# aws/sagemaker-xgboost-container

Hardware: NVIDIA B200
Metric: boosting rounds/sec (higher is better)
Workload: dtype int64

## Files before the change

sagemaker-xgboost-container_b200/csrc/booster.cu:

```cuda
#include "booster.h"
#include <algorithm>
#include <atomic>
#include <cmath>
#include <cstring>
#include <functional>
#include "comm.h"

namespace b200 {

long long g_kernel_launches = 0;

namespace {
struct DeviceCtx {
  cudaStream_t stream = nullptr; int num_sms = 148; bool ok = false; std::string why;
  DeviceCtx() {
    int count = 0;
    cudaError_t e = cudaGetDeviceCount(&count);
    if (e != cudaSuccess || count == 0) { why = std::string("no CUDA device available (") + cudaGetErrorString(e) + ")"; cudaGetLastError(); return; }
    int dev = 0;
    if (const char* lr = getenv("LOCAL_RANK")) { dev = atoi(lr) % count; }
    if (const char* d = getenv("B200XGB_DEVICE")) { dev = atoi(d) % count; }
    if (cudaSetDevice(dev) != cudaSuccess) { why = "cudaSetDevice failed"; return; }
    if (cudaStreamCreateWithFlags(&stream, cudaStreamNonBlocking) != cudaSuccess) { why = "cudaStreamCreate failed"; return; }
    cudaDeviceGetAttribute(&num_sms, cudaDevAttrMultiProcessorCount, dev);
// ... 139 lines not shown

void DMatrix::ensure_binned(int max_bin) {
  if (binned && (binned_max_bin == max_bin || binned_max_bin == -1)) return;
  B200_CHECK(max_bin >= 2, "max_bin must be >= 2");
  cudaStream_t s = engine_stream();
  Comm& comm = Comm::get();
  if (!comm.distributed()) {
    compute_cuts_device(X.p, n, F, weights.empty() ? nullptr : d_weights.p, max_bin, has_missing, &cuts, s);
  } else {
    const int cap = 2048;
    int hm = has_missing ? 1 : 0;
    {
      DevBuf<unsigned> flag; flag.alloc(1); unsigned v = (unsigned)hm;
      CUDA_OK(cudaMemcpyAsync(flag.p, &v, 4, cudaMemcpyHostToDevice, s));
      comm.allreduce_max_u32(flag.p, 1, s);
      CUDA_OK(cudaMemcpyAsync(&v, flag.p, 4, cudaMemcpyDeviceToHost, s)); Comm::get().sync_stream(s);
      has_missing = v != 0;
    }
    std::vector<FeatureSummary> local;
    compute_summaries_device(X.p, n, F, weights.empty() ? nullptr : d_weights.p, cap, &local, s);
    const size_t per_feat = (size_t)(cap + 2);
    const size_t rec = per_feat * (sizeof(float) + sizeof(double)) + sizeof(double);
    std::vector<unsigned char> sendbuf((size_t)F * rec, 0);
    for (int f = 0; f < F; ++f) {
      unsigned char* p = sendbuf.data() + (size_t)f * rec;
      double cntd = (double)local[f].vals.size(); memcpy(p, &cntd, 8);
      memcpy(p + 8, local[f].vals.data(), sizeof(float) * local[f].vals.size());
      memcpy(p + 8 + per_feat * sizeof(float), local[f].weights.data(), sizeof(double) * local[f].weights.size());
    }
    const int W = comm.world();
    DevBuf<unsigned char> dsend, drecv; dsend.alloc(sendbuf.size()); drecv.alloc(sendbuf.size() * W);
    CUDA_OK(cudaMemcpyAsync(dsend.p, sendbuf.data(), sendbuf.size(), cudaMemcpyHostToDevice, s));
    comm.allgather_bytes(dsend.p, drecv.p, sendbuf.size(), s);
    std::vector<unsigned char> all(sendbuf.size() * W);
    CUDA_OK(cudaMemcpyAsync(all.data(), drecv.p, all.size(), cudaMemcpyDeviceToHost, s));
    Comm::get().sync_stream(s);
    std::vector<FeatureSummary> merged(F);
    for (int f = 0; f < F; ++f) {
      std::vector<std::pair<float, double>> pts;
      for (int r = 0; r < W; ++r) {
        const unsigned char* p = all.data() + (size_t)r * sendbuf.size() + (size_t)f * rec;
        double cntd; memcpy(&cntd, p, 8); size_t c = (size_t)cntd;
        const float* v = reinterpret_cast<const float*>(p + 8);
        std::vector<double> w(c); memcpy(w.data(), p + 8 + per_feat * sizeof(float), sizeof(double) * c);
        for (size_t i = 0; i < c; ++i) pts.emplace_back(v[i], w[i]);
      }
      std::stable_sort(pts.begin(), pts.end(), [](const std::pair<float, double>& a, const std::pair<float, double>& b) { return a.first < b.first; });
      for (auto& pw : pts) {
        if (!merged[f].vals.empty() && merged[f].vals.back() == pw.first) merged[f].weights.back() += pw.second;
        else { merged[f].vals.push_back(pw.first); merged[f].weights.push_back(pw.second); }
      }
    }
    cuts_from_summaries(merged, max_bin, has_missing, &cuts);
  }
  binned_max_bin = max_bin;
  bin_with_cuts();
}

__global__ void pack_tree_kernel(TreeArrays t, const int* n_nodes, DevNode* out, int cap) {
  const int nn = *n_nodes;
  for (int i = blockIdx.x * blockDim.x + threadIdx.x; i < cap; i += gridDim.x * blockDim.x) {
    DevNode d;
    if (i < nn) { d.cond = t.split_cond[i]; d.left = t.left[i]; d.right = t.right[i]; d.fidx_dl = (unsigned)t.split_index[i] | ((unsigned)t.default_left[i] << 31); }
    else { d.cond = 0.f; d.left = -1; d.right = -1; d.fidx_dl = 0; }
    out[i] = d;
  }
}

__global__ void snapshot_h_kernel(const GH64* slot, long long* cache, size_t entries) {
  for (size_t e = (size_t)blockIdx.x * blockDim.x + threadIdx.x; e < entries; e += (size_t)gridDim.x * blockDim.x) cache[e] = slot[e].h;
}
__global__ void slot_from_cache_kernel(GH64* slot, const long long* cache, size_t entries) {
  for (size_t e = (size_t)blockIdx.x * blockDim.x + threadIdx.x; e < entries; e += (size_t)gridDim.x * blockDim.x) { GH64 v; v.g = 0; v.h = cache[e]; slot[e] = v; }
}

struct PinnedPool {
  std::vector<std::pair<char*, size_t>> chunks; size_t cur = 0, off = 0;
  ~PinnedPool() { for (auto& c : chunks) cudaFreeHost(c.first); }
  void* take(size_t bytes) {
    bytes = (bytes + 255) & ~(size_t)255;
    while (cur < chunks.size() && off + bytes > chunks[cur].second) { ++cur; off = 0; }
    if (cur >= chunks.size()) { size_t sz = std::max<size_t>(bytes, 4u << 20); char* p = nullptr; CUDA_OK(cudaMallocHost(&p, sz)); chunks.emplace_back(p, sz); off = 0; }
    void* r = chunks[cur].first + off; off += bytes; return r;
  }
  void reset() { cur = 0; off = 0; }
};

struct TreeGraphKey { uint64_t uid, binned_version; const void *margin, *mask, *packed, *bins, *bins_col, *cuts, *mono, *ic_sets, *ic_allowed; int n_ic; int max_depth, max_leaves, lg_iters; float eta, lambda, alpha, gamma, mcw, mds, bynode; unsigned seed; int world, root_mode; int64_t n; };
struct TreeGraph {
  std::vector<cudaGraphExec_t> segs; std::vector<std::function<void()>> colls;
  TreeGraphKey key; long long launches = 0;
  TreeGraph() { memset(&key, 0, sizeof key); }
  void destroy() { for (auto e : segs) if (e) cudaGraphExecDestroy(e); segs.clear(); colls.clear(); }
};

struct GrowerImpl {
  int64_t n = 0; int ngroups = 0, tw = 0, max_depth = 0, max_nodes = 0, cap_nodes = 0, max_level_nodes = 0, region = 0;
  int lg_iters = 0;
  size_t slot_stride = 0;
  int64_t gp_stride = 0;
  int64_t global_n = 0;
  DevBuf<long long> root_h_cache; uint64_t root_h_uid = 0, root_h_version = 0; bool root_h_valid = false;
  GrowState gs{}; TreeArrays ta{};
  DevBuf<unsigned char> state_block;
  DevBuf<unsigned char> tree_block;
  size_t tree_block_bytes = 0;
  DevBuf<GH64> hist_pool; DevBuf<unsigned> ridx0, ridx1, scratch;
  DevBuf<float2> gpair, gp0, gp1; DevBuf<unsigned> tl0, tl1; DevBuf<int> err, tree_index_dev, monotone_dev; DevBuf<unsigned char> feat_mask, ic_path, ic_allowed, ic_sets;
  std::vector<unsigned char> ic_sets_host;
  std::vector<int> monotone_host;
  DevBuf<double> dsum;
  PinnedPool pinned; std::vector<cudaEvent_t> free_events;
  DevBuf<DevNode> packed; std::vector<TreeGraph> graphs; std::vector<char> eager_done;
  TreeGraph* capturing = nullptr;

  void ensure(int64_t n_, int ngroups_, int tw_, int max_depth_, int K, int lg_iters_ = 0) {
    const int64_t stride_ = (n_ + 63) & ~(int64_t)63;
    if (n == n_ && ngroups == ngroups_ && tw == tw_ && max_depth == max_depth_ && lg_iters == lg_iters_ && gpair.n >= (size_t)stride_ * K + 512) return;
    if (lg_iters_ == 0) B200_CHECK(max_depth_ >= 1 && max_depth_ <= kMaxDepth, "max_depth must be in [1, 16] for the B200 depth-wise hist builder");
    n = n_; ngroups = ngroups_; tw = tw_; max_depth = max_depth_; lg_iters = lg_iters_; gp_stride = stride_; root_h_valid = false;
    if (peer_reduce_active()) {
      peer_reduce_close();
      DevBuf<unsigned> bar; bar.alloc(1); bar.zero(engine_stream());
      Comm::get().allreduce_max_u32(bar.p, 1, engine_stream());
      Comm::get().sync_stream(engine_stream());
    }
    for (auto& tg : graphs) tg.destroy();
    size_t pool_slots;
    if (lg_iters > 0) {
      max_nodes = 2 * lg_iters + 1; max_level_nodes = 2; region = 0;
      pool_slots = (size_t)lg_iters + kLgFirstFreeSlot;
    } else {
      max_nodes = (1 << (max_depth + 1)) - 1; max_level_nodes = 1 << (max_depth - 1); region = max_level_nodes;
      pool_slots = 2 * (size_t)region;
    }
    cap_nodes = (max_nodes + 15) & ~15;
    slot_stride = hist_slot_entries(ngroups, tw);
    const size_t pool_bytes = pool_slots * slot_stride * sizeof(GH64);
    size_t free_b = 0, total_b = 0; cudaMemGetInfo(&free_b, &total_b);
    B200_CHECK(pool_bytes < free_b / 2 + hist_pool.n * sizeof(GH64), "histogram pool for this max_depth / max_leaves / feature count does not fit in device memory");
    hist_pool.alloc(pool_slots * slot_stride);
    ridx0.alloc(n); ridx1.alloc(n);
    gpair.alloc((size_t)gp_stride * K + 512); gpair.zero(engine_stream()); gp0.alloc(n); gp1.alloc(n); err.alloc(1); dsum.alloc(4);
    root_h_cache.alloc(slot_stride);
    tl0.alloc(tw == 4 ? n : 0); tl1.alloc(tw == 4 ? n : 0);
    const unsigned max_tiles = (unsigned)((n + kPartTile - 1) / kPartTile) + max_level_nodes + 1;
    scratch.alloc(3 * (size_t)max_level_nodes + 8);
    size_t off = 0; auto take = [&](size_t bytes) { size_t o = off; off += (bytes + 255) & ~(size_t)255; return o; };
    const size_t N = cap_nodes, L = max_level_nodes;
    size_t o_seg_begin = take(4 * N), o_seg_count = take(4 * N), o_slot = take(4 * N), o_sum = take(16 * N), o_rg = take(4 * N), o_w = take(4 * N);
    size_t o_best = take(sizeof(SplitCand) * N), o_bestg = take(sizeof(SplitCand) * N * (ngroups + (tw > 0 ? 1 : 0)));
    size_t o_lnodes = take(4 * (size_t)(kMaxDepth + 1) * L), o_lcount = take(4 * (kMaxDepth + 2));
    size_t o_bnid = take(4 * L), o_bsub = take(4 * L), o_bps = take(4 * L), o_bcount = take(4), o_bprefix = take(4 * (L + 1));
    size_t o_action = take(4 * L), o_tprefix = take(4 * (L + 1)), o_tleft = take(4 * (size_t)max_tiles), o_toff = take(4 * (size_t)max_tiles);
    size_t o_flags = take((size_t)n + 16), o_nleaves = take(4), o_scales = take(16), o_absmax = take(8);
    size_t o_depth = take(4 * N), o_open = take(N), o_nslots = take(4), o_lgdone = take(4), o_lower = take(4 * N), o_upper = take(4 * N);
    state_block.alloc(off); state_block.zero(engine_stream());
    unsigned char* b = state_block.p;
    gs.seg_begin = (unsigned*)(b + o_seg_begin); gs.seg_count = (unsigned*)(b + o_seg_count); gs.hist_slot = (int*)(b + o_slot);
    gs.node_sum = (GH64*)(b + o_sum); gs.root_gain = (float*)(b + o_rg); gs.weight = (float*)(b + o_w);
    gs.best = (SplitCand*)(b + o_best); gs.best_group = (SplitCand*)(b + o_bestg);
    gs.level_nodes = (int*)(b + o_lnodes); gs.level_count = (int*)(b + o_lcount);
    gs.build_nid = (int*)(b + o_bnid); gs.build_sub_nid = (int*)(b + o_bsub); gs.build_parent_slot = (int*)(b + o_bps);
    gs.build_count = (int*)(b + o_bcount); gs.build_prefix = (unsigned*)(b + o_bprefix);
    gs.part_action = (int*)(b + o_action); gs.tile_prefix = (unsigned*)(b + o_tprefix); gs.tile_left = (unsigned*)(b + o_tleft); gs.tile_off = (unsigned*)(b + o_toff);
    gs.lower = (float*)(b + o_lower); gs.upper = (float*)(b + o_upper);
    gs.depth = (int*)(b + o_depth); gs.open = b + o_open; gs.n_slots = (int*)(b + o_nslots); gs.lg_done = (int*)(b + o_lgdone);
    gs.flags = b + o_flags; gs.n_leaves = (int*)(b + o_nleaves); gs.scales = (float*)(b + o_scales); gs.absmax = (unsigned*)(b + o_absmax);
    tree_block_bytes = 64 + 9 * 4 * N + N;
    tree_block.alloc(tree_block_bytes);
    unsigned char* t = tree_block.p;
    gs.n_nodes = (int*)t;
    int* ip = (int*)(t + 64);
    ta.left = ip; ta.right = ip + N; ta.parent = ip + 2 * N; ta.split_index = ip + 3 * N; ta.split_bin = ip + 4 * N;
    float* fp = (float*)(ip + 5 * N);
    ta.split_cond = fp; ta.base_weight = fp + N; ta.loss_chg = fp + 2 * N; ta.sum_hess = fp + 3 * N;
    ta.default_left = (unsigned char*)(fp + 4 * N);
    hist_configure();
    global_n = n;
    if (Comm::get().distributed()) {
      peer_reduce_setup({{hist_pool.p, hist_pool.n * sizeof(GH64)}, {state_block.p, state_block.n}}, engine_stream());
      double v = (double)n;
      CUDA_OK(cudaMemcpyAsync(dsum.p, &v, sizeof v, cudaMemcpyHostToDevice, engine_stream()));
      Comm::get().allreduce_sum_f64(dsum.p, 1, engine_stream());
      CUDA_OK(cudaMemcpyAsync(&v, dsum.p, sizeof v, cudaMemcpyDeviceToHost, engine_stream()));
      Comm::get().sync_stream(engine_stream());
      global_n = (int64_t)v;
    }
  }
};

static int job_grad_bits(int64_t global_n) { return grad_bits_for(global_n); }
static int job_window_rows(int64_t global_n) { return window_rows_for(global_n); }

static int lossguide_iters(const TrainParam& p) {
  if (!p.lossguide) return 0;
  if (p.max_leaves > 0) return std::max(1, p.max_leaves - 1);
  return (1 << p.max_depth) - 1;
}

static TrainParamDev to_dev(const TrainParam& p) {
  TrainParamDev d; d.eta = p.eta; d.lambda = p.lambda; d.alpha = p.alpha; d.gamma = p.gamma; d.min_child_weight = p.min_child_weight;
  d.max_delta_step = p.max_delta_step; d.max_depth = p.max_depth; d.max_leaves = p.max_leaves; return d;
}

static inline uint64_t splitmix64(uint64_t x) {
  x += 0x9E3779B97F4A7C15ULL; x = (x ^ (x >> 30)) * 0xBF58476D1CE4E5B9ULL; x = (x ^ (x >> 27)) * 0x94D049BB133111EBULL; return x ^ (x >> 31);
}
static inline float rng_uniform(uint32_t seed, uint64_t stream, uint64_t idx) {
  uint64_t h = splitmix64(splitmix64(((uint64_t)seed << 32) ^ stream) ^ idx);
  return (float)(h >> 40) * (1.0f / 16777216.0f);
}
std::string subset_mask(const std::string& parent, float frac, unsigned seed, uint64_t stream) {
  if (frac >= 1.0f) return parent;
  const int F = (int)parent.size();
  int cnt = 0; for (int f = 0; f < F; ++f) cnt += parent[f] ? 1 : 0;
  const int keep = std::max(1, (int)std::floor(frac * (float)cnt));
  std::vector<float> u(F);
  for (int f = 0; f < F; ++f) u[f] = rng_uniform(seed, stream, (uint64_t)f);
  std::string m((size_t)F, (char)0);
  for (int f = 0; f < F; ++f) {
    if (!parent[f]) continue;
    int rank = 0;
    for (int g = 0; g < F; ++g) if (parent[g] && (u[g] < u[f] || (u[g] == u[f] && g < f))) ++rank;
    m[f] = rank < keep ? 1 : 0;
  }
  return m;
}
std::string colsample_mask(unsigned seed, int tree_index, int F, float frac) {
  return subset_mask(std::string((size_t)F, (char)1), frac, seed, 0x1000 + (uint64_t)tree_index);
}

Booster::Booster() {}
Booster::~Booster() {
  if (grower_) { for (auto e : grower_->free_events) cudaEventDestroy(e); delete grower_; }
  for (auto& p : pending_) if (p.ready) cudaEventDestroy(p.ready);
}

static const std::map<std::string, int>& objective_table() {
  static const std::map<std::string, int> t = {{"reg:squarederror", kSquaredError}, {"reg:linear", kSquaredError}, {"binary:logistic", kBinaryLogistic},
    {"reg:logistic", kRegLogistic}, {"binary:logitraw", kLogitRaw}, {"multi:softprob", kSoftprob}, {"multi:softmax", kSoftmax},
    {"reg:squaredlogerror", kSquaredLogError}, {"reg:pseudohubererror", kPseudoHuber}, {"count:poisson", kPoisson}, {"reg:gamma", kGamma},
    {"reg:tweedie", kTweedie}, {"binary:hinge", kHinge}};
  return t;
}

void Booster::set_param(const std::string& k, const std::string& v) {
  if (k == "eval_metric") { if (std::find(eval_metrics_.begin(), eval_metrics_.end(), v) == eval_metrics_.end()) eval_metrics_.push_back(v); }
  else raw_params_[k] = v;
  configured_ = false;
}

void Booster::configure() {
  if (configured_) return;
  auto getf = [&](const char* a, const char* b, float def) { auto it = raw_params_.find(a); if (it == raw_params_.end() && b) it = raw_params_.find(b);
    if (it == raw_params_.end()) return def; try { return std::stof(it->second); } catch (...) { throw Error(std::string("Invalid value for parameter ") + a + ": " + it->second); } };
  auto geti = [&](const char* a, int def) { auto it = raw_params_.find(a); if (it == raw_params_.end()) return def;
    try { return (int)std::stod(it->second); } catch (...) { throw Error(std::string("Invalid value for parameter ") + a + ": " + it->second); } };
  TrainParam p;
  auto ito = raw_params_.find("objective");
  if (ito != raw_params_.end()) objective_name_ = ito->second;
  auto ot = objective_table().find(objective_name_);
  B200_CHECK(ot != objective_table().end(), "Unknown objective function: `" + objective_name_ + "` (supported on the B200 hist path: reg:squarederror, reg:linear, reg:logistic, reg:squaredlogerror, reg:pseudohubererror, reg:gamma, reg:tweedie, count:poisson, binary:logistic, binary:logitraw, binary:hinge, multi:softprob, multi:softmax)");
  p.objective = ot->second;
  if (objective_name_ == "reg:linear") objective_name_ = "reg:squarederror";
  p.num_class = (p.objective == kSoftprob || p.objective == kSoftmax) ? geti("num_class", 0) : 1;
  if (p.objective == kSoftprob || p.objective == kSoftmax) B200_CHECK(p.num_class >= 1, "num_class must be set (>= 1) for multi:softprob / multi:softmax");
  p.max_depth = geti("max_depth", 6); p.max_leaves = geti("max_leaves", 0); p.max_bin = geti("max_bin", 256);
  p.eta = getf("eta", "learning_rate", 0.3f); p.lambda = getf("lambda", "reg_lambda", 1.0f); p.alpha = getf("alpha", "reg_alpha", 0.0f);
  p.gamma = getf("gamma", "min_split_loss", 0.0f); p.min_child_weight = getf("min_child_weight", nullptr, 1.0f);
  p.max_delta_step = getf("max_delta_step", nullptr, 0.0f); p.scale_pos_weight = getf("scale_pos_weight", nullptr, 1.0f);
  p.subsample = getf("subsample", nullptr, 1.0f); p.colsample_bytree = getf("colsample_bytree", nullptr, 1.0f);
  p.colsample_bylevel = getf("colsample_bylevel", nullptr, 1.0f); p.colsample_bynode = getf("colsample_bynode", nullptr, 1.0f);
  p.seed = (unsigned)geti("seed", 0);
  p.huber_slope = getf("huber_slope", nullptr, 1.0f); p.tweedie_variance_power = getf("tweedie_variance_power", nullptr, 1.5f);
  B200_CHECK(p.huber_slope != 0.0f, "Check failed: slope != 0.0 (huber_slope)");
  B200_CHECK(p.tweedie_variance_power >= 1.0f && p.tweedie_variance_power < 2.0f, "tweedie_variance_power must be in interval [1, 2)");
  if (p.objective == kPoisson) {
    if (raw_params_.find("max_delta_step") == raw_params_.end()) p.max_delta_step = 0.7f;
    p.poisson_max_delta_step = p.max_delta_step;
    B200_CHECK(p.poisson_max_delta_step >= 0.0f, "max_delta_step must be non-negative for count:poisson");
  }
  B200_CHECK(p.lambda >= 0.0f, "Parameter reg_lambda should be greater equal to 0");
  B200_CHECK(p.subsample > 0.0f && p.subsample <= 1.0f, "Parameter subsample should be in (0, 1]");
  auto tm = raw_params_.find("tree_method");
  if (tm != raw_params_.end()) {
    const std::string& t = tm->second;
    B200_CHECK(t == "hist" || t == "auto" || t == "gpu_hist" || t == "approx" || t == "exact",
               "Unknown tree_method: " + t);
  }
  auto bo = raw_params_.find("booster");
  if (bo != raw_params_.end()) B200_CHECK(bo->second == "gbtree", "Only booster=gbtree is implemented on the B200 hist path (got " + bo->second + ")");
  auto gp = raw_params_.find("grow_policy");
  if (gp != raw_params_.end()) {
    B200_CHECK(gp->second == "depthwise" || gp->second == "lossguide", "Invalid grow_policy: " + gp->second + " (depthwise, lossguide)");
    p.lossguide = gp->second == "lossguide" ? 1 : 0;
  }
  interaction_.clear();
  auto ic = raw_params_.find("interaction_constraints");
  if (ic != raw_params_.end()) {
    int depth = 0; std::string tok; std::vector<int> cur;
    auto flush = [&]() { if (tok.empty()) return; int v = 0; try { v = std::stoi(tok); } catch (...) { throw Error("Invalid interaction_constraints entry: " + tok); }
      B200_CHECK(v >= 0, "interaction_constraints entries must be feature indices (feature names are not supported)"); cur.push_back(v); tok.clear(); };
    for (char ch : ic->second) {
      if (ch == '[' || ch == '(') { ++depth; }
      else if (ch == ']' || ch == ')') { flush(); if (depth == 2 && !cur.empty()) { interaction_.push_back(cur); cur.clear(); } --depth; }
      else if (ch >= '0' && ch <= '9') tok.push_back(ch);
      else { B200_CHECK(ch == ',' || ch == ' ' || ch == '\t' || ch == '\n' || ch == '"' || ch == '\'', std::string("Invalid character in interaction_constraints: ") + ch); flush(); }
    }
    B200_CHECK(depth == 0, "Unbalanced brackets in interaction_constraints");
  }
  monotone_.clear();
  auto mc = raw_params_.find("monotone_constraints");
  if (mc != raw_params_.end()) {
    std::string tok;
    auto flush = [&]() { if (tok.empty()) return; int v = 0; try { v = std::stoi(tok); } catch (...) { throw Error("Invalid monotone_constraints entry: " + tok); }
      B200_CHECK(v >= -1 && v <= 1, "monotone_constraints entries must be -1, 0 or 1"); monotone_.push_back(v); tok.clear(); };
    for (char ch : mc->second) { if (ch == '-' || ch == '+' || (ch >= '0' && ch <= '9')) tok.push_back(ch); else flush(); }
    flush();
    bool any = false; for (int v : monotone_) any |= v != 0;
    if (!any) monotone_.clear();
  }
  if (p.lossguide) {
    B200_CHECK(p.max_depth >= 0 && p.max_depth <= kMaxDepth, "max_depth must be in [0, 16]");
    B200_CHECK(p.max_leaves > 0 || p.max_depth > 0, "grow_policy=lossguide needs max_leaves > 0 or max_depth > 0");
    B200_CHECK(p.max_leaves <= 4096, "max_leaves above 4096 is not supported by the B200 lossguide builder");
    B200_CHECK(p.colsample_bytree >= 1.0f && p.colsample_bylevel >= 1.0f && p.colsample_bynode >= 1.0f, "column sampling (colsample_*) with grow_policy=lossguide is not implemented by the B200 hist builder");
  }
  auto bs = raw_params_.find("base_score");
  if (bs != raw_params_.end() && !bs->second.empty()) {
    base_score_ = std::stof(bs->second); base_score_set_ = true;
// ... 41 lines not shown

void Booster::append_device_tree(int class_id, size_t device_offset, int max_nodes, PendingTree pt) {
  trees_.emplace_back(); tree_info_.push_back(class_id); pending_.push_back(pt); on_device_.push_back(1);
  h_tree_offset.resize(trees_.size() + 1);
  h_tree_offset[trees_.size() - 1] = (int64_t)device_offset;
  h_tree_offset[trees_.size()] = (int64_t)device_offset + max_nodes;
  ++model_version_;
}

void Booster::sync_model() {
  bool any = false;
  for (auto& p : pending_) if (p.staging) { any = true; break; }
  if (!any) return;
  for (size_t t = 0; t < pending_.size(); ++t) {
    PendingTree& p = pending_[t];
    if (!p.staging) continue;
    CUDA_OK(cudaEventSynchronize(p.ready));
    const unsigned char* b = (const unsigned char*)p.staging;
    const int nn = *(const int*)b; const size_t N = p.cap_nodes;
    const int* ip = (const int*)(b + 64); const float* fp = (const float*)(ip + 5 * N); const unsigned char* up = (const unsigned char*)(fp + 4 * N);
    HostTree& h = trees_[t];
    h.left.assign(ip, ip + nn); h.right.assign(ip + N, ip + N + nn); h.parent.assign(ip + 2 * N, ip + 2 * N + nn);
    h.split_index.assign(ip + 3 * N, ip + 3 * N + nn); h.split_bin.assign(ip + 4 * N, ip + 4 * N + nn);
    h.split_cond.assign(fp, fp + nn); h.base_weight.assign(fp + N, fp + N + nn); h.loss_chg.assign(fp + 2 * N, fp + 2 * N + nn); h.sum_hess.assign(fp + 3 * N, fp + 3 * N + nn);
    h.default_left.assign(up, up + nn);
    if (grower_) grower_->free_events.push_back(p.ready); else cudaEventDestroy(p.ready);
    p.ready = nullptr; p.staging = nullptr;
  }
  if (grower_) grower_->pinned.reset();
}

void Booster::upload_model() {
  cudaStream_t s = engine_stream();
  const int nt = (int)trees_.size();
  if ((int)h_tree_offset.size() != nt + 1) h_tree_offset.resize(nt + 1, 0);
  pending_.resize(nt); on_device_.resize(nt, 0);
  for (int t = 0; t < nt; ++t) {
    if (on_device_[t]) continue;
    const HostTree& h = trees_[t];
    const int nn = h.num_nodes();
    std::vector<DevNode> nodes(nn);
    for (int i = 0; i < nn; ++i) { nodes[i].cond = h.split_cond[i]; nodes[i].left = h.left[i]; nodes[i].right = h.right[i]; nodes[i].fidx_dl = (unsigned)h.split_index[i] | ((unsigned)h.default_left[i] << 31);
      if (h.left[i] >= 0 && h.right[i] != h.left[i] + 1) children_adjacent_ = false; }
    if (d_nodes_used + nn > d_nodes.n) {
      size_t cap = std::max<size_t>(d_nodes.n * 2, d_nodes_used + nn + 4096);
      DevBuf<DevNode> nb; nb.alloc(cap);
      if (d_nodes_used) CUDA_OK(cudaMemcpyAsync(nb.p, d_nodes.p, sizeof(DevNode) * d_nodes_used, cudaMemcpyDeviceToDevice, s));
      Comm::get().sync_stream(s);
      std::swap(nb.p, d_nodes.p); std::swap(nb.n, d_nodes.n);
    }
    CUDA_OK(cudaMemcpyAsync(d_nodes.p + d_nodes_used, nodes.data(), sizeof(DevNode) * nn, cudaMemcpyHostToDevice, s));
    Comm::get().sync_stream(s);
    h_tree_offset[t] = (int64_t)d_nodes_used; h_tree_offset[t + 1] = (int64_t)d_nodes_used + nn;
    d_nodes_used += nn; on_device_[t] = 1; d_trees_uploaded = 0;
  }
  if (d_trees_uploaded != nt || d_tree_offset.n < (size_t)nt + 1) {
    d_tree_offset.ensure(std::max<size_t>(nt + 1, 64)); d_tree_info.ensure(std::max<size_t>(nt, 64));
    CUDA_OK(cudaMemcpyAsync(d_tree_offset.p, h_tree_offset.data(), sizeof(int64_t) * (nt + 1), cudaMemcpyHostToDevice, s));
    if (nt) CUDA_OK(cudaMemcpyAsync(d_tree_info.p, tree_info_.data(), sizeof(int) * nt, cudaMemcpyHostToDevice, s));
    Comm::get().sync_stream(s);
    d_trees_uploaded = nt;
  }
}

PredCache& Booster::cache_for(DMatrix* dm) {
  PredCache& c = caches_[dm->uid];
  const int K = param_.num_class;
  if (c.n != dm->n || c.margin.n != (size_t)dm->n * K) {
    c.n = dm->n; c.margin.alloc((size_t)dm->n * K); c.trees_applied = -1;
  }
  return c;
}

void Booster::bring_cache_up_to_date(DMatrix* dm, PredCache& c) {
  cudaStream_t s = engine_stream();
  const int K = param_.num_class;
  const int nt = (int)trees_.size();
  if (c.trees_applied < 0) {
    if (!dm->base_margin.empty()) {
      B200_CHECK(dm->base_margin.size() == (size_t)dm->n * K, "base_margin size does not match rows x groups");
      CUDA_OK(cudaMemcpyAsync(c.margin.p, dm->d_base_margin.p, sizeof(float) * dm->n * K, cudaMemcpyDeviceToDevice, s));
    } else launch_fill(c.margin.p, dm->n * K, base_margin(), s);
    c.trees_applied = 0;
  }
  if (c.trees_applied < nt) {
    upload_model();
    PredictArgs pa{}; pa.X = dm->X.p; pa.n = dm->n; pa.F = dm->F; pa.nodes = d_nodes.p; pa.tree_offset = d_tree_offset.p; pa.tree_info = d_tree_info.p;
    pa.tree_begin = c.trees_applied; pa.tree_end = nt; pa.K = K; pa.margin = c.margin.p; pa.leaf = nullptr;
    pa.h_tree_offset = h_tree_offset.data(); pa.has_nan = dm->has_missing ? 1 : 0; pa.children_adjacent = children_adjacent_ ? 1 : 0;
    launch_predict(pa, s);
    c.trees_applied = nt;
  }
}

static void check_labels(const DMatrix* dm) {
  B200_CHECK(dm->labels.size() == (size_t)dm->n, "Check failed: preds.size() == info.labels_.size() (" + std::to_string(dm->n) + " vs. " +
             std::to_string(dm->labels.size()) + ") : labels are not correctly provided");
}

void Booster::update_one_iter(int iter, DMatrix* dtrain) {
  configure();
  (void)iter;
  cudaStream_t s = engine_stream();
  check_labels(dtrain);
  if (num_feature_ == 0) num_feature_ = dtrain->F;
  B200_CHECK(num_feature_ == dtrain->F, "Check failed: learner_model_param_.num_feature == p_fmat->Info().num_col_ (" + std::to_string(num_feature_) +
             " vs. " + std::to_string(dtrain->F) + ") : Number of columns does not match number of features in booster.");
  B200_CHECK(dtrain->n > 0 || Comm::get().distributed(), "Empty dataset at worker: 0");
  dtrain->ensure_binned(param_.max_bin);
  const int K = param_.num_class;
  if (!grower_) grower_ = new GrowerImpl();
  GrowerImpl& g = *grower_;
  g.ensure(dtrain->n, dtrain->ngroups, dtrain->tw, param_.max_depth, K, lossguide_iters(param_));
  if (!labels_checked_) {
    const std::vector<float>& y = dtrain->labels;
    if (param_.objective == kBinaryLogistic || param_.objective == kRegLogistic || param_.objective == kLogitRaw)
      for (float v : y) B200_CHECK(v >= 0.0f && v <= 1.0f, "Check failed: label must be in [0,1] for logistic regression");
    if (param_.objective == kSoftprob || param_.objective == kSoftmax)
      for (float v : y) B200_CHECK(v >= 0.0f && (int)v < K, "SoftmaxMultiClassObj: label must be in [0, num_class).");
    if (param_.objective == kSquaredLogError) for (float v : y) B200_CHECK(v > -1.0f, "Check failed: label must be greater than -1 for rmsle so that log(label + 1) can be valid.");
    if (param_.objective == kPoisson) for (float v : y) B200_CHECK(v >= 0.0f, "PoissonRegression: label must be nonnegative");
    if (param_.objective == kGamma) for (float v : y) B200_CHECK(v > 0.0f, "GammaRegression: label must be positive.");
    if (param_.objective == kTweedie) for (float v : y) B200_CHECK(v >= 0.0f, "TweedieRegression: label must be nonnegative");
    labels_checked_ = true;
  }
  estimate_base_score(dtrain);
  PredCache& cache = cache_for(dtrain);
  bring_cache_up_to_date(dtrain, cache);

  const int round = (int)trees_.size() / K;
  CUDA_OK(cudaMemsetAsync(g.gs.absmax, 0, 8, s));
  GradArgs ga{}; ga.margin = cache.margin.p; ga.label = dtrain->d_labels.p; ga.weight = dtrain->weights.empty() ? nullptr : dtrain->d_weights.p;
  ga.gpair = g.gpair.p; ga.gp_stride = g.gp_stride; ga.absmax = g.gs.absmax; ga.err = g.err.p; ga.n = dtrain->n; ga.row_offset = 0; ga.K = K; ga.objective = param_.objective;
  ga.scale_pos_weight = param_.scale_pos_weight; ga.subsample = param_.subsample; ga.seed = param_.seed; ga.iter = (unsigned long long)round;
  ga.row_offset = (int64_t)Comm::get().rank() << 40; ga.aux = objective_aux(param_);
  launch_gradient(ga, s);
  Comm::get().allreduce_max_u32(g.gs.absmax, 2, s);
  launch_scales(g.gs, job_grad_bits(g.global_n), s);

  for (int k = 0; k < K; ++k) grow_one_tree(dtrain, cache, k, round * K + k);
}


void Booster::enqueue_tree(DMatrix* dtrain, float* margin, int k, const unsigned char* mask, DevNode* packed_out, int root_mode) {
  cudaStream_t s = engine_stream();
  GrowerImpl& g = *grower_;
  Comm& comm = Comm::get();
  const int K = param_.num_class;
  const int D = param_.max_depth;
  const TrainParamDev pd = to_dev(param_);
  const BinnedMatrix bm = dtrain->binned_view();
  const int num_sms = engine_num_sms();
  const unsigned max_tiles = (unsigned)((dtrain->n + kPartTile - 1) / kPartTile) + g.max_level_nodes + 1;

  launch_init_tree(g.gs, g.ta, (unsigned)dtrain->n, 0, g.max_level_nodes, s);
  if (root_mode == 2) { slot_from_cache_kernel<<<148, 256, 0, s>>>(g.hist_pool.p, g.root_h_cache.p, g.slot_stride); ++g_kernel_launches; CUDA_OK(cudaGetLastError()); }
  else CUDA_OK(cudaMemsetAsync(g.hist_pool.p, 0, g.slot_stride * sizeof(GH64), s));

  HistArgs ha{}; ha.bins = bm.bins; ha.bins_tail = bm.bins_tail; ha.n = bm.n; ha.row_stride = bm.ngroups * kSlots; ha.tw = bm.tw;
  ha.bins_gather = bm.bins_gather; ha.gather_stride = bm.gather_stride;
  ha.gpair = g.gpair.p + (size_t)k * g.gp_stride; ha.ridx = nullptr;
  ha.build_count = g.gs.build_count; ha.build_nid = g.gs.build_nid; ha.build_prefix = g.gs.build_prefix; ha.seg_begin = g.gs.seg_begin;
  ha.hist_slot = g.gs.hist_slot; ha.scales = g.gs.scales; ha.hist_pool = g.hist_pool.p; ha.node_sum = g.gs.node_sum; ha.ngroups = bm.ngroups;
  ha.accumulate_sum = 1; ha.g_only = root_mode == 2 ? 1 : 0; ha.window_rows = job_window_rows(g.global_n);
  ha.rows_counter = profile_ ? prof_rows_.p : nullptr;
  prof_begin(0);
  launch_hist_build(ha, num_sms, s);
  prof_end();
  if (root_mode == 1) { snapshot_h_kernel<<<148, 256, 0, s>>>(g.hist_pool.p, g.root_h_cache.p, g.slot_stride); ++g_kernel_launches; CUDA_OK(cudaGetLastError()); }
  ha.g_only = 0;
  auto collective = [&](std::function<void()> f) {
    if (!comm.distributed()) return;
    if (!g.capturing) { f(); return; }
    cudaGraph_t graph = nullptr;
    CUDA_OK(cudaStreamEndCapture(s, &graph));
    cudaGraphExec_t exec = nullptr;
    cudaError_t e = cudaGraphInstantiate(&exec, graph, 0);
    cudaGraphDestroy(graph);
    CUDA_OK(e);
    g.capturing->segs.push_back(exec); g.capturing->colls.push_back(f);
    CUDA_OK(cudaStreamBeginCapture(s, cudaStreamCaptureModeThreadLocal));
  };
  auto allreduce_hist = [&](GH64* p, size_t cnt) {
    if (!comm.distributed()) return;
    if (peer_allreduce_i64(reinterpret_cast<long long*>(p), cnt, s)) return;
    collective([p, cnt, s]() { Comm::get().allreduce_sum_i64(p, cnt, s); });
  };
  allreduce_hist(g.hist_pool.p, g.slot_stride * 2);
  allreduce_hist(g.gs.node_sum, 2);
  const int* mono_dev = nullptr;
  if (!monotone_.empty()) {
    B200_CHECK((int)monotone_.size() <= bm.F, "monotone_constraints has more entries than the data has features");
    mono_dev = g.monotone_dev.p;
  }
  const bool ic_on = !interaction_.empty();
  if (ic_on) {
    CUDA_OK(cudaMemsetAsync(g.ic_path.p, 0, (size_t)bm.F, s));
    CUDA_OK(cudaMemsetAsync(g.ic_allowed.p, 1, (size_t)bm.F, s));
  }
  EvalArgs ea{}; ea.hist_pool = g.hist_pool.p; ea.gs = g.gs; ea.cut_ptrs = dtrain->d_cut_ptrs.p; ea.feat_mask = mask; ea.p = pd; ea.F = bm.F;
  ea.ngroups = bm.ngroups; ea.tw = bm.tw; ea.ntail = bm.ntail; ea.has_missing = bm.has_missing; ea.level = 0; ea.max_level_nodes = g.max_level_nodes;
  ea.colsample_bynode = mask ? param_.colsample_bynode : 1.0f; ea.seed = param_.seed; ea.tree_index = g.tree_index_dev.p; ea.monotone = mono_dev; ea.node_allowed = ic_on ? g.ic_allowed.p : nullptr;
  launch_eval(ea, 1, s);

  const int lg_iters = lossguide_iters(param_);
  for (int it = 0; it < lg_iters; ++it) {
    ApplyArgs aa{}; aa.gs = g.gs; aa.tree = g.ta; aa.cut_ptrs = dtrain->d_cut_ptrs.p; aa.cut_vals = dtrain->d_cut_vals.p; aa.min_vals = dtrain->d_min_vals.p;
    aa.p = pd; aa.scratch = g.scratch.p; aa.ngroups = bm.ngroups + (bm.tw > 0 ? 1 : 0); aa.level = 0; aa.max_level_nodes = g.max_level_nodes; aa.monotone = mono_dev;
    if (ic_on) { aa.node_path = g.ic_path.p; aa.node_allowed = g.ic_allowed.p; aa.ic_sets = g.ic_sets.p; aa.n_ic_sets = (int)interaction_.size(); aa.F = bm.F; }
    launch_apply_lossguide(aa, it, s);
    const bool carry_tail = bm.tw == 4;
    PartArgs pa{}; pa.gs = g.gs; pa.tree = g.ta; pa.bins_col = bm.bins_col; pa.n = bm.n;
    pa.ridx_cur = it == 0 ? nullptr : g.ridx0.p; pa.ridx_next = g.ridx1.p;
    pa.gp_cur = it == 0 ? g.gpair.p + (size_t)k * g.gp_stride : g.gp0.p; pa.gp_next = g.gp1.p;
    pa.tl_cur = !carry_tail ? nullptr : (it == 0 ? reinterpret_cast<const unsigned*>(bm.bins_tail) : g.tl0.p); pa.tl_next = !carry_tail ? nullptr : g.tl1.p;
    pa.has_missing = bm.has_missing; pa.level = 0; pa.max_level_nodes = g.max_level_nodes;
    launch_partition(pa, max_tiles, 1, s);
    launch_lg_copy_back(pa, g.ridx0.p, g.gp0.p, g.tl0.p, max_tiles, s);
    launch_zero_build_slots(g.gs, g.hist_pool.p, g.slot_stride, 1, s);
    ha.ridx = g.ridx0.p; ha.gpair = g.gp0.p; ha.tail_pos = carry_tail ? g.tl0.p : nullptr; ha.accumulate_sum = 0;
    ha.rows_counter = profile_ ? prof_rows_.p + 1 : nullptr;
    prof_begin(1);
    launch_hist_build(ha, num_sms, s);
    prof_end();
    if (comm.distributed()) {
      launch_lg_stage(g.gs, g.hist_pool.p, g.slot_stride, 1, s);
      allreduce_hist(g.hist_pool.p + (size_t)kLgStageSlot * g.slot_stride, g.slot_stride * 2);
      launch_lg_stage(g.gs, g.hist_pool.p, g.slot_stride, 0, s);
    }
    launch_subtract(g.gs, g.hist_pool.p, g.slot_stride, 1, s);
    ea.level = 1; ea.feat_mask = nullptr;
    launch_eval(ea, 2, s);
  }

  for (int L = 0; L < D && lg_iters == 0; ++L) {
    const bool final_level = (L == D - 1);
    const int next_base = ((L + 1) & 1) * g.region, next_half = 1 << L;
    ApplyArgs aa{}; aa.gs = g.gs; aa.tree = g.ta; aa.cut_ptrs = dtrain->d_cut_ptrs.p; aa.cut_vals = dtrain->d_cut_vals.p; aa.min_vals = dtrain->d_min_vals.p;
    aa.p = pd; aa.scratch = g.scratch.p; aa.ngroups = bm.ngroups + (bm.tw > 0 ? 1 : 0); aa.level = L; aa.max_level_nodes = g.max_level_nodes; aa.next_base = next_base; aa.next_half = next_half; aa.monotone = mono_dev;
    if (ic_on) { aa.node_path = g.ic_path.p; aa.node_allowed = g.ic_allowed.p; aa.ic_sets = g.ic_sets.p; aa.n_ic_sets = (int)interaction_.size(); aa.F = bm.F; }
    launch_apply(aa, s);
    if (final_level) break;
    PartArgs pa{}; pa.gs = g.gs; pa.tree = g.ta; pa.bins_col = bm.bins_col; pa.n = bm.n;
    pa.ridx_cur = L == 0 ? nullptr : ((L & 1) ? g.ridx0.p : g.ridx1.p);
    pa.ridx_next = (L & 1) ? g.ridx1.p : g.ridx0.p;
    pa.gp_cur = L == 0 ? g.gpair.p + (size_t)k * g.gp_stride : ((L & 1) ? g.gp0.p : g.gp1.p);
    pa.gp_next = (L & 1) ? g.gp1.p : g.gp0.p;
    const bool carry_tail = bm.tw == 4;
    pa.tl_cur = !carry_tail ? nullptr : (L == 0 ? reinterpret_cast<const unsigned*>(bm.bins_tail) : ((L & 1) ? g.tl0.p : g.tl1.p));
    pa.tl_next = !carry_tail ? nullptr : ((L & 1) ? g.tl1.p : g.tl0.p);
    pa.has_missing = bm.has_missing; pa.level = L; pa.max_level_nodes = g.max_level_nodes;
    launch_partition(pa, max_tiles, 1 << L, s);
    CUDA_OK(cudaMemsetAsync(g.hist_pool.p + (size_t)next_base * g.slot_stride, 0, (size_t)next_half * g.slot_stride * sizeof(GH64), s));
    ha.ridx = pa.ridx_next; ha.gpair = pa.gp_next; ha.tail_pos = pa.tl_next; ha.accumulate_sum = 0;
    ha.rows_counter = profile_ ? prof_rows_.p + 1 : nullptr;
    prof_begin(L + 1);
    launch_hist_build(ha, num_sms, s);
    prof_end();
    allreduce_hist(g.hist_pool.p + (size_t)next_base * g.slot_stride, (size_t)next_half * g.slot_stride * 2);
    launch_subtract(g.gs, g.hist_pool.p, g.slot_stride, next_half, s);
    ea.level = L + 1;
    ea.feat_mask = mask ? mask + (size_t)(L + 1) * bm.F : nullptr;
    launch_eval(ea, 1 << (L + 1), s);
  }

  launch_update_margin(g.ta, g.gs.n_nodes, bm.bins_col, bm.n, bm.has_missing, margin, K, k, s);

  pack_tree_kernel<<<(g.cap_nodes + 255) / 256, 256, 0, s>>>(g.ta, g.gs.n_nodes, packed_out, g.cap_nodes); ++g_kernel_launches;
  CUDA_OK(cudaGetLastError());
}

void Booster::grow_one_tree(DMatrix* dtrain, PredCache& cache, int k, int tree_index) {
  cudaStream_t s = engine_stream();
  GrowerImpl& g = *grower_;
  const unsigned char* mask = nullptr;
  const bool sampling = param_.colsample_bytree < 1.0f || param_.colsample_bylevel < 1.0f || param_.colsample_bynode < 1.0f;
  if (sampling) {
    const std::string tm = colsample_mask(param_.seed, tree_index, dtrain->F, param_.colsample_bytree);
    std::string all;
    for (int d = 0; d < param_.max_depth; ++d) all += subset_mask(tm, param_.colsample_bylevel, param_.seed, 0x300000ull + 64ull * (uint64_t)tree_index + (uint64_t)d);
    g.feat_mask.ensure(all.size()); g.tree_index_dev.ensure(1);
    CUDA_OK(cudaMemcpyAsync(g.feat_mask.p, all.data(), all.size(), cudaMemcpyHostToDevice, s));
    CUDA_OK(cudaMemcpyAsync(g.tree_index_dev.p, &tree_index, sizeof(int), cudaMemcpyHostToDevice, s));
    Comm::get().sync_stream(s);
    mask = g.feat_mask.p;
  }
  if (!monotone_.empty()) {
    std::vector<int> mh(monotone_); mh.resize((size_t)std::max<int>(dtrain->F, (int)mh.size()), 0);
    if (mh != g.monotone_host || g.monotone_dev.n < mh.size()) {
      g.monotone_dev.ensure(mh.size());
      CUDA_OK(cudaMemcpyAsync(g.monotone_dev.p, mh.data(), sizeof(int) * mh.size(), cudaMemcpyHostToDevice, s));
      Comm::get().sync_stream(s);
      g.monotone_host = mh;
    }
  }
  if (!interaction_.empty()) {
    const size_t F = (size_t)dtrain->F;
    std::vector<unsigned char> sets(interaction_.size() * F, 0);
    for (size_t si = 0; si < interaction_.size(); ++si)
      for (int f : interaction_[si]) { B200_CHECK((size_t)f < F, "interaction_constraints names feature " + std::to_string(f) + " but the data has " + std::to_string(F) + " features"); sets[si * F + f] = 1; }
    g.ic_path.ensure((size_t)g.cap_nodes * F); g.ic_allowed.ensure((size_t)g.cap_nodes * F);
    if (sets != g.ic_sets_host || g.ic_sets.n < sets.size()) {
      g.ic_sets.ensure(sets.size());
      CUDA_OK(cudaMemcpyAsync(g.ic_sets.p, sets.data(), sets.size(), cudaMemcpyHostToDevice, s));
      Comm::get().sync_stream(s);
      g.ic_sets_host = sets;
    }
  }
  g.packed.ensure((size_t)g.cap_nodes);
  static const bool no_graph = getenv("B200XGB_NO_GRAPH") != nullptr;
  static const bool no_graph_multi = getenv("B200XGB_NO_GRAPH_MULTI") != nullptr;
  const bool dist = Comm::get().distributed();
  if ((int)g.eager_done.size() <= k) g.eager_done.resize(k + 1, 0);
  const bool eager_first = dist && !g.eager_done[k];
  static const bool no_consth = getenv("B200XGB_NO_CONSTH") != nullptr;
  const bool consth = !no_consth && param_.objective == kSquaredError && param_.num_class == 1 && dtrain->weights.empty() &&
                      param_.subsample >= 1.0f && param_.scale_pos_weight == 1.0f;
  int root_mode = 0;
  if (consth) {
    if (g.root_h_valid && g.root_h_uid == dtrain->uid && g.root_h_version == dtrain->binned_version) root_mode = 2;
    else root_mode = 1;
  }
  if (profile_ || no_graph || (dist && no_graph_multi) || eager_first || root_mode == 1) {
    g.eager_done[k] = 1;
    enqueue_tree(dtrain, cache.margin.p, k, mask, g.packed.p, root_mode);
    if (root_mode == 1) { g.root_h_valid = true; g.root_h_uid = dtrain->uid; g.root_h_version = dtrain->binned_version; }
  } else {
    if ((int)g.graphs.size() <= k) g.graphs.resize(k + 1);
    TreeGraph& tg = g.graphs[k];
    TreeGraphKey key; memset(&key, 0, sizeof key);
    key.uid = dtrain->uid; key.binned_version = dtrain->binned_version; key.root_mode = root_mode;
    key.margin = cache.margin.p; key.mask = mask; key.packed = g.packed.p; key.max_depth = param_.max_depth;
    key.bins = dtrain->bins.p; key.bins_col = dtrain->bins_col.p; key.cuts = dtrain->d_cut_vals.p;
    key.max_leaves = param_.max_leaves; key.lg_iters = lossguide_iters(param_); key.eta = param_.eta; key.lambda = param_.lambda; key.alpha = param_.alpha; key.gamma = param_.gamma;
    key.mcw = param_.min_child_weight; key.mds = param_.max_delta_step; key.world = Comm::get().world(); key.n = dtrain->n;
    key.bynode = param_.colsample_bynode; key.seed = param_.seed; key.mono = monotone_.empty() ? nullptr : g.monotone_dev.p;
    key.ic_sets = interaction_.empty() ? nullptr : g.ic_sets.p; key.ic_allowed = interaction_.empty() ? nullptr : g.ic_allowed.p; key.n_ic = (int)interaction_.size();
    if (tg.segs.empty() || memcmp(&tg.key, &key, sizeof key) != 0) {
      tg.destroy();
      const long long launches_before = g_kernel_launches;
      CUDA_OK(cudaStreamBeginCapture(s, cudaStreamCaptureModeThreadLocal));
      g.capturing = &tg;
      cudaGraph_t graph = nullptr;
      try { enqueue_tree(dtrain, cache.margin.p, k, mask, g.packed.p, root_mode); }
      catch (...) { g.capturing = nullptr; cudaStreamEndCapture(s, &graph); if (graph) cudaGraphDestroy(graph); tg.destroy(); throw; }
      g.capturing = nullptr;
      CUDA_OK(cudaStreamEndCapture(s, &graph));
      cudaGraphExec_t exec = nullptr;
      cudaError_t e = cudaGraphInstantiate(&exec, graph, 0);
      cudaGraphDestroy(graph);
      if (e != cudaSuccess) { tg.destroy(); CUDA_OK(e); }
      tg.segs.push_back(exec);
      tg.key = key; tg.launches = g_kernel_launches - launches_before;
      g_kernel_launches = launches_before;
    }
    for (size_t i = 0; i < tg.segs.size(); ++i) {
      CUDA_OK(cudaGraphLaunch(tg.segs[i], s));
      if (i < tg.colls.size()) tg.colls[i]();
    }
    g_kernel_launches += tg.launches;
  }

  const size_t need = d_nodes_used + (size_t)g.cap_nodes;
  if (need > d_nodes.n) {
    size_t cap = std::max<size_t>(d_nodes.n * 2, need + 64 * (size_t)g.cap_nodes);
    DevBuf<DevNode> nb; nb.alloc(cap);
    if (d_nodes_used) CUDA_OK(cudaMemcpyAsync(nb.p, d_nodes.p, sizeof(DevNode) * d_nodes_used, cudaMemcpyDeviceToDevice, s));
    Comm::get().sync_stream(s);
    std::swap(nb.p, d_nodes.p); std::swap(nb.n, d_nodes.n);
  }
  CUDA_OK(cudaMemcpyAsync(d_nodes.p + d_nodes_used, g.packed.p, sizeof(DevNode) * (size_t)g.cap_nodes, cudaMemcpyDeviceToDevice, s));
  if (pending_.size() - (size_t)std::count_if(pending_.begin(), pending_.end(), [](const PendingTree& p) { return p.staging == nullptr; }) >= 512) sync_model();
  PendingTree pt; pt.cap_nodes = (size_t)g.cap_nodes;
  pt.staging = g.pinned.take(g.tree_block_bytes);
  if (!g.free_events.empty()) { pt.ready = g.free_events.back(); g.free_events.pop_back(); }
  else CUDA_OK(cudaEventCreateWithFlags(&pt.ready, cudaEventDisableTiming));
  CUDA_OK(cudaMemcpyAsync(pt.staging, g.tree_block.p, g.tree_block_bytes, cudaMemcpyDeviceToHost, s));
  CUDA_OK(cudaEventRecord(pt.ready, s));
  append_device_tree(k, d_nodes_used, g.cap_nodes, pt);
  d_nodes_used += (size_t)g.cap_nodes;
  d_trees_uploaded = 0;
  cache.trees_applied = (int)trees_.size();
}

void Booster::boost_one_iter(DMatrix*, const float*, const float*, size_t) {
  throw Error("custom objective (BoostOneIter) is not implemented on the B200 hist path");
}

int Booster::boosted_rounds() { configure(); return (int)trees_.size() / std::max(1, param_.num_class); }

static std::string default_metric(const TrainParam& p) {
  switch (p.objective) {
    case kSquaredError: case kRegLogistic: return "rmse";
    case kBinaryLogistic: case kLogitRaw: return "logloss";
    case kSquaredLogError: return "rmsle";
    case kPseudoHuber: return "mphe";
    case kPoisson: return "poisson-nloglik";
    case kGamma: return "gamma-nloglik";
    case kTweedie: { char buf[64]; snprintf(buf, sizeof buf, "tweedie-nloglik@%g", (double)p.tweedie_variance_power); return buf; }
    case kHinge: return "error";
    default: return "mlogloss";
  }
}

std::string Booster::eval_one_iter(int iter, const std::vector<DMatrix*>& dms, const std::vector<std::string>& names) {
  configure();
  cudaStream_t s = engine_stream();
  std::vector<std::string> metrics = eval_metrics_;
  if (metrics.empty()) metrics.push_back(default_metric(param_));
  if (!grower_) grower_ = new GrowerImpl();
  grower_->dsum.ensure(4);
  std::string out = "[" + std::to_string(iter) + "]";
  for (size_t i = 0; i < dms.size(); ++i) {
    DMatrix* dm = dms[i];
    check_labels(dm);
    PredCache& c = cache_for(dm);
    bring_cache_up_to_date(dm, c);
    for (const std::string& mname : metrics) {
      MetricArgs ma{}; ma.margin = c.margin.p; ma.label = dm->d_labels.p; ma.weight = dm->weights.empty() ? nullptr : dm->d_weights.p;
      ma.out = grower_->dsum.p; ma.n = dm->n; ma.K = param_.num_class; ma.threshold = 0.5f;
      ma.is_logistic = (param_.objective == kBinaryLogistic || param_.objective == kRegLogistic) ? 1 : 0;
      ma.transform = objective_transform(param_.objective); ma.aux = 0.0f;
      std::string base = mname;
      if (mname.rfind("tweedie-nloglik@", 0) == 0) { base = "tweedie-nloglik"; ma.aux = std::stof(mname.substr(16)); B200_CHECK(ma.aux >= 1.0f && ma.aux < 2.0f, "tweedie variance power must be in interval [1, 2)"); }
      if (mname.rfind("error@", 0) == 0) { base = "error"; ma.threshold = std::stof(mname.substr(6)); }
      if (base == "auc") {
        B200_CHECK(param_.num_class <= 1, "auc is implemented for binary / regression-style predictions only");
        const int logistic = (param_.objective == kBinaryLogistic || param_.objective == kRegLogistic) ? 1 : 0;
        compute_auc_device(c.margin.p, dm->d_labels.p, dm->weights.empty() ? nullptr : dm->d_weights.p, dm->n, logistic, grower_->dsum.p, s);
        double h3[3];
        CUDA_OK(cudaMemcpyAsync(h3, grower_->dsum.p, 3 * sizeof(double), cudaMemcpyDeviceToHost, s));
        Comm::get().sync_stream(s);
        double pair[2] = {h3[0], h3[1] * h3[2]};
        if (Comm::get().distributed()) {
          CUDA_OK(cudaMemcpyAsync(grower_->dsum.p, pair, 2 * sizeof(double), cudaMemcpyHostToDevice, s));
          Comm::get().allreduce_sum_f64(grower_->dsum.p, 2, s);
          CUDA_OK(cudaMemcpyAsync(pair, grower_->dsum.p, 2 * sizeof(double), cudaMemcpyDeviceToHost, s));
          Comm::get().sync_stream(s);
        }
        B200_CHECK(pair[1] > 0.0, "Check failed: !auc_error AUC: the dataset only contains pos or neg samples");
        char buf[64]; snprintf(buf, sizeof buf, "%.17g", pair[0] / pair[1]);
        out += "\t" + names[i] + "-" + mname + ":" + buf;
        continue;
      }
      if (base == "rmse") ma.metric = kMetricRmse; else if (base == "mse") ma.metric = kMetricRmse; else if (base == "mae") ma.metric = kMetricMae;
      else if (base == "logloss") ma.metric = kMetricLogloss; else if (base == "error") ma.metric = kMetricError;
      else if (base == "merror") ma.metric = kMetricMerror; else if (base == "mlogloss") ma.metric = kMetricMlogloss;
      else if (base == "rmsle") ma.metric = kMetricRmsle; else if (base == "mape") ma.metric = kMetricMape;
      else if (base == "mphe") { ma.metric = kMetricMphe; ma.aux = param_.huber_slope; }
      else if (base == "poisson-nloglik") ma.metric = kMetricPoissonNll; else if (base == "gamma-nloglik") ma.metric = kMetricGammaNll;
      else if (base == "gamma-deviance") ma.metric = kMetricGammaDeviance;
      else if (base == "tweedie-nloglik") { ma.metric = kMetricTweedieNll; if (ma.aux == 0.0f) throw Error("tweedie-nloglik needs its variance power: tweedie-nloglik@rho"); }
      else throw Error("Unknown metric function " + mname + " (B200 hist path implements rmse, mse, rmsle, mae, mape, mphe, logloss, error, error@t, merror, mlogloss, auc, poisson-nloglik, gamma-nloglik, gamma-deviance, tweedie-nloglik@rho)");
      if (param_.objective == kLogitRaw && (ma.metric == kMetricLogloss || ma.metric == kMetricError)) ma.is_logistic = 1;
      if ((ma.metric == kMetricMerror || ma.metric == kMetricMlogloss)) B200_CHECK(param_.num_class > 1, "Check failed: preds.size() == info.labels_.size() : label and prediction size not match, hint: use merror or mlogloss for multi-class classification");
      CUDA_OK(cudaMemsetAsync(grower_->dsum.p, 0, 2 * sizeof(double), s));
      launch_metric(ma, s);
      Comm::get().allreduce_sum_f64(grower_->dsum.p, 2, s);
      double h[2];
      CUDA_OK(cudaMemcpyAsync(h, grower_->dsum.p, 2 * sizeof(double), cudaMemcpyDeviceToHost, s));
      Comm::get().sync_stream(s);
      double v = h[1] == 0.0 ? h[0] : h[0] / h[1];
      if (mname == "rmse" || mname == "rmsle") v = std::sqrt(v);
      if (mname == "gamma-deviance") v *= 2.0;
      char buf[64]; snprintf(buf, sizeof buf, "%.17g", v);
      out += "\t" + names[i] + "-" + mname + ":" + buf;
    }
  }
  return out;
}

void Booster::predict(DMatrix* dm, int type, bool training, int iter_begin, int iter_end, bool strict_shape,
                      std::vector<float>* out, std::vector<uint64_t>* shape) {
  configure();
  (void)training;
  cudaStream_t s = engine_stream();
  const int K = param_.num_class;
  const int rounds = (int)trees_.size() / K;
  if (iter_end == 0) iter_end = rounds;
  B200_CHECK(iter_begin >= 0 && iter_begin <= iter_end && iter_end <= rounds, "Invalid iteration range: [" + std::to_string(iter_begin) + ", " + std::to_string(iter_end) + ") for a model with " + std::to_string(rounds) + " rounds");
  if (num_feature_ > 0 && !trees_.empty())
    B200_CHECK(dm->F <= num_feature_ || true, "feature count mismatch");
  B200_CHECK(type == 0 || type == 1 || type == 2 || type == 6, "predict type " + std::to_string(type) + " (approximate contributions / interactions) is not implemented on the B200 path");
  if (type == 2) { predict_contribs(dm, iter_begin * K, iter_end * K, out, shape); return; }
  upload_model();
  const int tb = iter_begin * K, te = iter_end * K;
  const int64_t n = dm->n;
  PredictArgs pa{}; pa.X = dm->X.p; pa.n = n; pa.F = dm->F; pa.nodes = d_nodes.p; pa.tree_offset = d_tree_offset.p; pa.tree_info = d_tree_info.p;
  pa.tree_begin = tb; pa.tree_end = te; pa.K = K;
  pa.h_tree_offset = h_tree_offset.data(); pa.has_nan = dm->has_missing ? 1 : 0; pa.children_adjacent = children_adjacent_ ? 1 : 0;
  if (type == 6) {
    const int nt = te - tb;
    DevBuf<int>& leaf = pred_leaf_; leaf.ensure((size_t)n * std::max(nt, 1));
    pa.margin = nullptr; pa.leaf = leaf.p;
    launch_predict(pa, s);
    std::vector<int> h((size_t)n * nt);
    if (!h.empty()) CUDA_OK(cudaMemcpyAsync(h.data(), leaf.p, sizeof(int) * h.size(), cudaMemcpyDeviceToHost, s));
    Comm::get().sync_stream(s);
    out->resize(h.size());
    for (size_t i = 0; i < h.size(); ++i) (*out)[i] = (float)h[i];
    shape->assign({(uint64_t)n, (uint64_t)nt});
    return;
  }
  DevBuf<float>& margin = pred_margin_; margin.ensure((size_t)n * K);
  if (!dm->base_margin.empty()) {
    B200_CHECK(dm->base_margin.size() == (size_t)n * K, "base_margin size does not match rows x groups");
    CUDA_OK(cudaMemcpyAsync(margin.p, dm->d_base_margin.p, sizeof(float) * n * K, cudaMemcpyDeviceToDevice, s));
  } else launch_fill(margin.p, n * K, base_margin(), s);
  pa.margin = margin.p; pa.leaf = nullptr;
  launch_predict(pa, s);
  int out_cols = K;
  DevBuf<float>& cls = pred_cls_;
  if (type == 0) {
    if (param_.objective == kSoftmax) { cls.ensure(n); launch_transform(margin.p, n, K, param_.objective, cls.p, s); out_cols = 1; }
    else launch_transform(margin.p, n, K, param_.objective, nullptr, s);
  }
  out->resize((size_t)n * out_cols);
  if (!out->empty()) CUDA_OK(cudaMemcpyAsync(out->data(), (type == 0 && param_.objective == kSoftmax) ? cls.p : margin.p, sizeof(float) * out->size(), cudaMemcpyDeviceToHost, s));
  Comm::get().sync_stream(s);
  if (out_cols == 1 && !strict_shape) shape->assign({(uint64_t)n});
  else shape->assign({(uint64_t)n, (uint64_t)out_cols});
}

__global__ void gather_u32_kernel(const unsigned* src, const unsigned* idx, unsigned* dst, int64_t n) {
  const int64_t i = (int64_t)blockIdx.x * blockDim.x + threadIdx.x;
  if (i < n) dst[i] = src[idx[i]];
}

void Booster::debug_build_root_hist(DMatrix* dm, const float* gpair_host, std::vector<long long>* hist_out, float* scales_out,
                                    int repeats, float* ms_out, int mode, const unsigned* row_ids, int64_t n_ids) {
  configure();
  cudaStream_t s = engine_stream();
  dm->ensure_binned(param_.max_bin);
  if (!grower_) grower_ = new GrowerImpl();
  GrowerImpl& g = *grower_;
  g.ensure(dm->n, dm->ngroups, dm->tw, param_.max_depth, param_.num_class, lossguide_iters(param_));
  hist_configure();
  const int64_t rows = row_ids ? n_ids : dm->n;
  B200_CHECK(rows <= dm->n, "debug_build_root_hist: more row ids than rows");
  CUDA_OK(cudaMemcpyAsync(g.gpair.p, gpair_host, sizeof(float2) * rows, cudaMemcpyHostToDevice, s));
  if (row_ids) CUDA_OK(cudaMemcpyAsync(g.ridx0.p, row_ids, sizeof(unsigned) * rows, cudaMemcpyHostToDevice, s));
  float mg = 0.f, mh = 0.f;
  for (int64_t i = 0; i < rows; ++i) { mg = std::max(mg, std::fabs(gpair_host[2 * i])); mh = std::max(mh, gpair_host[2 * i + 1]); }
  unsigned am[2]; memcpy(&am[0], &mg, 4); memcpy(&am[1], &mh, 4);
  CUDA_OK(cudaMemcpyAsync(g.gs.absmax, am, 8, cudaMemcpyHostToDevice, s));
  launch_scales(g.gs, job_grad_bits(g.global_n), s);
  const BinnedMatrix bm = dm->binned_view();
  HistArgs ha{}; ha.bins = bm.bins; ha.bins_tail = bm.bins_tail; ha.n = bm.n; ha.row_stride = bm.ngroups * kSlots; ha.tw = bm.tw; ha.gpair = g.gpair.p;
  ha.bins_gather = bm.bins_gather; ha.gather_stride = bm.gather_stride;
  ha.ridx = row_ids ? g.ridx0.p : nullptr;
  ha.build_count = g.gs.build_count; ha.build_nid = g.gs.build_nid; ha.build_prefix = g.gs.build_prefix; ha.seg_begin = g.gs.seg_begin;
  ha.hist_slot = g.gs.hist_slot; ha.scales = g.gs.scales; ha.hist_pool = g.hist_pool.p; ha.node_sum = g.gs.node_sum; ha.ngroups = bm.ngroups; ha.accumulate_sum = 1;
  ha.force_gather = (mode & 3) == 1 ? 1 : 0; ha.g_only = (mode & 3) == 2 ? 1 : 0; ha.window_rows = job_window_rows(g.global_n);
  if ((mode & 4) && row_ids && bm.tw == 4) {
    gather_u32_kernel<<<(unsigned)((rows + 255) / 256), 256, 0, s>>>(reinterpret_cast<const unsigned*>(bm.bins_tail), g.ridx0.p, g.tl0.p, rows); ++g_kernel_launches;
    CUDA_OK(cudaGetLastError());
    ha.tail_pos = g.tl0.p;
  }
  g.root_h_valid = false;
  cudaEvent_t e0, e1; CUDA_OK(cudaEventCreate(&e0)); CUDA_OK(cudaEventCreate(&e1));
  float total = 0.f;
  for (int r = 0; r < std::max(1, repeats); ++r) {
    launch_init_tree(g.gs, g.ta, (unsigned)rows, 0, g.max_level_nodes, s);
    CUDA_OK(cudaMemsetAsync(g.hist_pool.p, 0, g.slot_stride * sizeof(GH64), s));
    CUDA_OK(cudaEventRecord(e0, s));
    launch_hist_build(ha, engine_num_sms(), s);
    CUDA_OK(cudaEventRecord(e1, s));
    CUDA_OK(cudaEventSynchronize(e1));
    float ms = 0; CUDA_OK(cudaEventElapsedTime(&ms, e0, e1)); total += ms;
  }
  if (ms_out) *ms_out = total / std::max(1, repeats);
  hist_out->resize(g.slot_stride * 2);
  CUDA_OK(cudaMemcpyAsync(hist_out->data(), g.hist_pool.p, sizeof(GH64) * g.slot_stride, cudaMemcpyDeviceToHost, s));
  CUDA_OK(cudaMemcpyAsync(scales_out, g.gs.scales, 4 * sizeof(float), cudaMemcpyDeviceToHost, s));
  Comm::get().sync_stream(s);
  cudaEventDestroy(e0); cudaEventDestroy(e1);
}

void Booster::predict_contribs(DMatrix* dm, int tb, int te, std::vector<float>* out, std::vector<uint64_t>* shape) {
  cudaStream_t s = engine_stream();
  sync_model();
  const int K = param_.num_class;
  const int64_t n = dm->n;
  const int F = std::max(dm->F, num_feature_);
  B200_CHECK(dm->F == F, "pred_contribs: the data has " + std::to_string(dm->F) + " columns, the model uses " + std::to_string(F));
  std::vector<ShapNode> nodes; std::vector<int64_t> offs; std::vector<int> info;
  int max_depth = 0;
  for (int t = tb; t < te; ++t) {
    const HostTree& h = trees_[t];
    const int nn = h.num_nodes();
    const size_t base = nodes.size();
    offs.push_back((int64_t)base); info.push_back(tree_info_[t]);
    nodes.resize(base + nn);
    std::vector<int> depth(nn, 0);
    for (int i = 0; i < nn; ++i) {
      ShapNode& d = nodes[base + i];
      d.cond = h.split_cond[i]; d.left = h.left[i]; d.right = h.right[i]; d.fidx_dl = (unsigned)h.split_index[i] | ((unsigned)h.default_left[i] << 31);
      d.sum_hess = h.sum_hess[i]; d.mean = 0.0f;
      if (h.left[i] >= 0) { B200_CHECK(h.left[i] > i && h.right[i] > i, "pred_contribs: children must follow their parent in the node array"); depth[h.left[i]] = depth[h.right[i]] = depth[i] + 1; }
      max_depth = std::max(max_depth, depth[i]);
    }
    for (int i = nn - 1; i >= 0; --i) {
      ShapNode& d = nodes[base + i];
      if (d.left < 0) d.mean = d.cond;
      else { float r = nodes[base + d.left].mean * nodes[base + d.left].sum_hess; r += nodes[base + d.right].mean * nodes[base + d.right].sum_hess; d.mean = r / d.sum_hess; }
    }
  }
  DevBuf<ShapNode> d_sn; DevBuf<int64_t> d_off; DevBuf<int> d_info; DevBuf<float> d_out;
  d_sn.alloc(std::max<size_t>(nodes.size(), 1)); d_off.alloc(std::max<size_t>(offs.size(), 1)); d_info.alloc(std::max<size_t>(info.size(), 1));
  const size_t total = (size_t)n * K * (F + 1);
  d_out.alloc(std::max<size_t>(total, 1));
  if (!nodes.empty()) {
    CUDA_OK(cudaMemcpyAsync(d_sn.p, nodes.data(), sizeof(ShapNode) * nodes.size(), cudaMemcpyHostToDevice, s));
    CUDA_OK(cudaMemcpyAsync(d_off.p, offs.data(), sizeof(int64_t) * offs.size(), cudaMemcpyHostToDevice, s));
    CUDA_OK(cudaMemcpyAsync(d_info.p, info.data(), sizeof(int) * info.size(), cudaMemcpyHostToDevice, s));
  }
  CUDA_OK(cudaMemsetAsync(d_out.p, 0, sizeof(float) * std::max<size_t>(total, 1), s));
  ShapArgs sa{}; sa.X = dm->X.p; sa.n = n; sa.F = F; sa.nodes = d_sn.p; sa.tree_offset = d_off.p; sa.tree_info = d_info.p; sa.tree_begin = tb; sa.tree_end = te; sa.K = K;
  sa.out = d_out.p; sa.base_margin = base_margin();
  if (!dm->base_margin.empty()) { B200_CHECK(dm->base_margin.size() == (size_t)n * K, "base_margin size does not match rows x groups"); sa.base_margin_rows = dm->d_base_margin.p; }
  launch_shap(sa, max_depth, s);
  out->resize(total);
  if (total) CUDA_OK(cudaMemcpyAsync(out->data(), d_out.p, sizeof(float) * total, cudaMemcpyDeviceToHost, s));
  Comm::get().sync_stream(s);
  if (K > 1) shape->assign({(uint64_t)n, (uint64_t)K, (uint64_t)(F + 1)}); else shape->assign({(uint64_t)n, (uint64_t)(F + 1)});
}

float Booster::debug_predict_kernel_ms(DMatrix* dm, int repeats) {
  configure();
  cudaStream_t s = engine_stream();
  upload_model();
  const int K = param_.num_class;
  pred_margin_.ensure((size_t)dm->n * K);
  PredictArgs pa{}; pa.X = dm->X.p; pa.n = dm->n; pa.F = dm->F; pa.nodes = d_nodes.p; pa.tree_offset = d_tree_offset.p; pa.tree_info = d_tree_info.p;
  pa.tree_begin = 0; pa.tree_end = (int)trees_.size(); pa.K = K; pa.margin = pred_margin_.p; pa.leaf = nullptr;
  pa.h_tree_offset = h_tree_offset.data(); pa.has_nan = dm->has_missing ? 1 : 0; pa.children_adjacent = children_adjacent_ ? 1 : 0;
  cudaEvent_t e0, e1; CUDA_OK(cudaEventCreate(&e0)); CUDA_OK(cudaEventCreate(&e1));
  float total = 0.f;
  for (int r = 0; r < std::max(1, repeats); ++r) {
    launch_fill(pred_margin_.p, dm->n * K, base_margin(), s);
    CUDA_OK(cudaEventRecord(e0, s));
    launch_predict(pa, s);
    CUDA_OK(cudaEventRecord(e1, s));
    CUDA_OK(cudaEventSynchronize(e1));
    float ms = 0; CUDA_OK(cudaEventElapsedTime(&ms, e0, e1)); total += ms;
  }
  cudaEventDestroy(e0); cudaEventDestroy(e1);
  return total / std::max(1, repeats);
}

void Booster::cached_margin(DMatrix* dm, std::vector<float>* out) {
  configure();
  cudaStream_t s = engine_stream();
  PredCache& c = cache_for(dm);
  bring_cache_up_to_date(dm, c);
  out->resize((size_t)dm->n * param_.num_class);
  if (!out->empty()) CUDA_OK(cudaMemcpyAsync(out->data(), c.margin.p, sizeof(float) * out->size(), cudaMemcpyDeviceToHost, s));
  Comm::get().sync_stream(s);
}

void Booster::set_profile(bool on) {
  profile_ = on;
  if (on) { prof_rows_.alloc(2); prof_rows_.zero(engine_stream()); prof_launches_ = 0; }
  for (auto& e : prof_events_) { cudaEventDestroy(e.a); cudaEventDestroy(e.b); }
  prof_events_.clear();
}
void Booster::prof_begin(int level) {
  if (!profile_) return;
  ProfEvent e; e.level = level;
  CUDA_OK(cudaEventCreate(&e.a)); CUDA_OK(cudaEventCreate(&e.b));
  CUDA_OK(cudaEventRecord(e.a, engine_stream()));
  prof_events_.push_back(e);
}
void Booster::prof_end() {
  if (!profile_) return;
  CUDA_OK(cudaEventRecord(prof_events_.back().b, engine_stream()));
}
std::string Booster::get_profile() {
  cudaStream_t s = engine_stream();
  Comm::get().sync_stream(s);
  double root_ms = 0, deep_ms = 0; long long root_n = 0, deep_n = 0;
  for (auto& e : prof_events_) { float ms = 0; CUDA_OK(cudaEventElapsedTime(&ms, e.a, e.b)); if (e.level == 0) { root_ms += ms; ++root_n; } else { deep_ms += ms; ++deep_n; } }
  unsigned long long rows[2] = {0, 0};
  if (prof_rows_.p) CUDA_OK(cudaMemcpy(rows, prof_rows_.p, sizeof rows, cudaMemcpyDeviceToHost));
  char buf[512];
  snprintf(buf, sizeof buf, "{\"root_hist_ms\":%.6f,\"root_hist_launches\":%lld,\"root_hist_rows\":%llu,\"deep_hist_ms\":%.6f,\"deep_hist_launches\":%lld,\"deep_hist_rows\":%llu}",
           root_ms, root_n, rows[0], deep_ms, deep_n, rows[1]);
  return buf;
}

}
```

sagemaker-xgboost-container_b200/csrc/booster.h:

```cpp
#pragma once
#include <map>
#include <memory>
#include <string>
#include <vector>
#include "engine.h"
#include "json.h"
#include "misc.h"
#include "tree.h"

namespace b200 {

cudaStream_t engine_stream();
int engine_num_sms();

class DMatrix {
 public:
  int64_t n = 0; int F = 0;
  bool has_missing = false;
  DevBuf<float> X;
  std::vector<float> labels, weights, base_margin;
  DevBuf<float> d_labels, d_weights, d_base_margin;
  std::vector<std::string> feature_names, feature_types;
  bool binned = false; int binned_max_bin = 0;
  HostCuts cuts; DevBuf<int> d_cut_ptrs; DevBuf<float> d_cut_vals, d_min_vals;
  DevBuf<uint8_t> bins, bins_tail, bins_col, bins_gather; int ngroups = 0, tw = 0, ntail = 0, gather_stride = 0;
  uint64_t binned_version = 0;
  uint64_t uid;

  DMatrix();
  static std::unique_ptr<DMatrix> from_dense(const float* data, int64_t nrow, int ncol, float missing);
  static std::unique_ptr<DMatrix> from_device(const float* dptr, int64_t nrow, int ncol, float missing);
  static std::unique_ptr<DMatrix> from_csv_text(const char* text, int64_t len, char delim, int* status);
  static std::unique_ptr<DMatrix> from_libsvm_text(const char* text, int64_t len, int whitespace_mode, float absent, int* status);
  static std::unique_ptr<DMatrix> from_csv_text_labeled(const char* text, int64_t len, char delim, int label_col, int weight_col, int* status);
  static std::unique_ptr<DMatrix> from_columns(const void* const* cols, const int* types, int ncols, int64_t nrow, int label_col, int weight_col);
  static std::unique_ptr<DMatrix> from_csr(const size_t* indptr, const unsigned* indices, const float* data, size_t nindptr, size_t nelem, size_t ncol);
  std::unique_ptr<DMatrix> slice(const int* idx, int64_t len) const;
  void set_float_info(const std::string& field, const float* v, size_t len);
  const std::vector<float>& get_float_info(const std::string& field) const;
  void ensure_binned(int max_bin);
  void set_cuts(const HostCuts& c);
  BinnedMatrix binned_view() const { BinnedMatrix b; b.bins = bins.p; b.bins_tail = tw ? bins_tail.p : nullptr; b.bins_col = bins_col.p; b.n = n; b.F = F;
    b.bins_gather = bins_gather.p ? bins_gather.p : bins.p; b.gather_stride = gather_stride;
    b.ngroups = ngroups; b.tw = tw; b.ntail = ntail; b.has_missing = has_missing; return b; }
  void finish_upload(float missing);
 private:
  void bin_with_cuts();
};

struct HostTree {
  std::vector<int> left, right, parent, split_index, split_bin;
  std::vector<uint8_t> default_left;
  std::vector<float> split_cond, base_weight, loss_chg, sum_hess;
  int num_nodes() const { return (int)left.size(); }
};

struct PendingTree {
  void* staging = nullptr; size_t cap_nodes = 0; cudaEvent_t ready = nullptr;
};

struct PredCache { DevBuf<float> margin; int trees_applied = 0; int64_t n = 0; uint64_t model_version = 0; };

bool looks_like_legacy_binary(const char* buf, size_t len);
JPtr legacy_binary_to_doc(const char* buf, size_t len);
std::pair<const char*, size_t> legacy_serialized_model_section(const char* buf, size_t len);

class Booster {
 public:
  Booster();
  ~Booster();
  void set_param(const std::string& k, const std::string& v);
  std::string save_config();
  void load_config(const std::string& json);
  void update_one_iter(int iter, DMatrix* dtrain);
  void boost_one_iter(DMatrix* dtrain, const float* grad, const float* hess, size_t len);
  std::string eval_one_iter(int iter, const std::vector<DMatrix*>& dms, const std::vector<std::string>& names);
  void predict(DMatrix* dm, int type, bool training, int iter_begin, int iter_end, bool strict_shape,
               std::vector<float>* out, std::vector<uint64_t>* shape);
  void predict_contribs(DMatrix* dm, int tree_begin, int tree_end, std::vector<float>* out, std::vector<uint64_t>* shape);
  std::string save_model_buffer(const std::string& format);
  void load_model_buffer(const char* buf, size_t len);
  std::string serialize();
  void unserialize(const char* buf, size_t len);
  std::unique_ptr<Booster> slice(int begin, int end, int step);
  int boosted_rounds();
  int num_features() const { return num_feature_; }
  std::map<std::string, std::string> attrs;
  std::vector<std::string> feature_names, feature_types;

  void sync_model();
  void cached_margin(DMatrix* dm, std::vector<float>* out);
  float debug_predict_kernel_ms(DMatrix* dm, int repeats);
  const std::vector<HostTree>& trees() { sync_model(); return trees_; }
  const std::vector<int>& tree_info() const { return tree_info_; }
  float base_score() const { return base_score_; }
  int num_class() const { return param_.num_class; }
  const TrainParam& param() { configure(); return param_; }
  void set_profile(bool on);
  std::string get_profile();
  void debug_build_root_hist(DMatrix* dm, const float* gpair_host, std::vector<long long>* hist_out, float* scales_out,
                             int repeats, float* ms_out, int mode = 0, const unsigned* row_ids = nullptr, int64_t n_ids = 0);

 private:
  friend struct GrowerImpl;
  std::map<std::string, std::string> raw_params_;
  std::vector<std::string> eval_metrics_;
  std::vector<int> monotone_;
  std::vector<std::vector<int>> interaction_;
  bool configured_ = false;
  TrainParam param_;
  std::string objective_name_ = "reg:squarederror";
  bool base_score_set_ = false; float base_score_ = 0.5f; bool base_score_estimated_ = false;
  int num_feature_ = 0;
  std::vector<HostTree> trees_; std::vector<int> tree_info_;
  std::vector<PendingTree> pending_;
  std::vector<char> on_device_;
  uint64_t model_version_ = 0;
  DevBuf<DevNode> d_nodes; std::vector<int64_t> h_tree_offset; DevBuf<int64_t> d_tree_offset; DevBuf<int> d_tree_info;
  size_t d_nodes_used = 0; int d_trees_uploaded = 0;
  std::map<uint64_t, PredCache> caches_;
  struct GrowerImpl* grower_ = nullptr;
  bool labels_checked_ = false;
  DevBuf<float> pred_margin_, pred_cls_; DevBuf<int> pred_leaf_;
  bool children_adjacent_ = true;
  bool profile_ = false;
  struct ProfEvent { cudaEvent_t a, b; int level; };
  std::vector<ProfEvent> prof_events_;
  DevBuf<unsigned long long> prof_rows_;
  long long prof_launches_ = 0;

  void configure();
  float base_margin() const;
  void estimate_base_score(DMatrix* dtrain);
  void upload_model();
  PredCache& cache_for(DMatrix* dm);
  void bring_cache_up_to_date(DMatrix* dm, PredCache& c);
  void append_device_tree(int class_id, size_t device_offset, int max_nodes, PendingTree pt);
  void grow_one_tree(DMatrix* dtrain, PredCache& cache, int k, int tree_index);
  void enqueue_tree(DMatrix* dtrain, float* margin, int k, const unsigned char* mask, DevNode* packed_out, int root_mode);
  void prof_begin(int level);
  void prof_end();
  JPtr model_to_json();
  void model_from_json(const JValue& doc);
  JPtr config_to_json();
  void config_from_json(const JValue& doc);
  void reset_model();
};

std::string colsample_mask(unsigned seed, int tree_index, int F, float frac);
std::string subset_mask(const std::string& parent, float frac, unsigned seed, uint64_t stream);

}
```

sagemaker-xgboost-container_b200/csrc/engine.h:

```cpp
#pragma once
#include <cuda_runtime.h>
#include <cstdint>
#include <cstdio>
#include <stdexcept>
#include <string>
#include <vector>

namespace b200 {

struct Error : std::runtime_error { using std::runtime_error::runtime_error; };
#define B200_CHECK(cond, msg) do { if (!(cond)) throw ::b200::Error(std::string(msg)); } while (0)
#define CUDA_OK(expr) do { cudaError_t e_ = (expr); if (e_ != cudaSuccess) throw ::b200::Error( \
    std::string("CUDA error: ") + cudaGetErrorString(e_) + " at " + __FILE__ + ":" + std::to_string(__LINE__)); } while (0)

extern long long g_kernel_launches;

template <typename T> struct DevBuf {
  T* p = nullptr; size_t n = 0;
  DevBuf() = default;
  DevBuf(const DevBuf&) = delete; DevBuf& operator=(const DevBuf&) = delete;
  ~DevBuf() { release(); }
  void release() { if (p) cudaFree(p); p = nullptr; n = 0; }
  void alloc(size_t count) { if (count == n && p) return; release(); if (count) { CUDA_OK(cudaMalloc(&p, count * sizeof(T))); } n = count; }
  void ensure(size_t count) { if (count > n) alloc(count); }
  void zero(cudaStream_t s) { if (n) CUDA_OK(cudaMemsetAsync(p, 0, n * sizeof(T), s)); }
};

constexpr int kSlots = 32;
constexpr int kBins = 256;
constexpr int kGroupEntries = kBins * kSlots;
constexpr int kMissingBin = 255;
constexpr int kGradBits = 18, kWindowRows = 8064;
constexpr int kGradBitsSmall = 21, kWindowRowsSmall = 1008;
constexpr int64_t kSmallMatrixRows = 1 << 20;
inline int grad_bits_for(int64_t n) { return n <= kSmallMatrixRows ? kGradBitsSmall : kGradBits; }
inline int window_rows_for(int64_t n) { return n <= kSmallMatrixRows ? kWindowRowsSmall : kWindowRows; }
constexpr int kMaxDepth = 16;

struct GH64 { long long g, h; };

struct BinnedMatrix {
  const uint8_t* bins = nullptr;
  const uint8_t* bins_tail = nullptr;
  const uint8_t* bins_col = nullptr;
  const uint8_t* bins_gather = nullptr;
  int gather_stride = 0;
  int64_t n = 0;
  int F = 0, ngroups = 0, tw = 0, ntail = 0;
  int has_missing = 0;
};

inline void feature_layout(int F, int* ngroups, int* tw, int* ntail) {
  const int a = F / 32, L = F % 32;
  if (a >= 1 && L >= 1 && L <= 8) { *ngroups = a; *ntail = L; *tw = L <= 4 ? 4 : 8; }
  else { *ngroups = a + (L > 0 ? 1 : 0); if (*ngroups == 0) *ngroups = 1; *ntail = 0; *tw = 0; }
}
inline size_t hist_slot_entries(int ngroups, int tw) { return (size_t)ngroups * 256 * 32 + (size_t)256 * tw; }

enum Objective : int { kSquaredError = 0, kBinaryLogistic = 1, kRegLogistic = 2, kLogitRaw = 3, kSoftprob = 4, kSoftmax = 5,
                       kSquaredLogError = 6, kPseudoHuber = 7, kPoisson = 8, kGamma = 9, kTweedie = 10, kHinge = 11 };
enum Transform : int { kTransformNone = 0, kTransformSigmoid = 1, kTransformExp = 2, kTransformHinge = 3 };
inline bool objective_is_logistic(int o) { return o == kBinaryLogistic || o == kRegLogistic || o == kLogitRaw; }
inline bool objective_is_log_link(int o) { return o == kPoisson || o == kGamma || o == kTweedie; }
inline int objective_transform(int o) {
  if (o == kBinaryLogistic || o == kRegLogistic) return kTransformSigmoid;
  if (objective_is_log_link(o)) return kTransformExp;
  return o == kHinge ? kTransformHinge : kTransformNone;
}

struct TrainParam {
  int objective = kSquaredError;
  int num_class = 1;
  int max_depth = 6, max_leaves = 0, max_bin = 256;
  int lossguide = 0;
  float eta = 0.3f, lambda = 1.0f, alpha = 0.0f, gamma = 0.0f, min_child_weight = 1.0f, max_delta_step = 0.0f;
  float scale_pos_weight = 1.0f, subsample = 1.0f, colsample_bytree = 1.0f, colsample_bylevel = 1.0f, colsample_bynode = 1.0f;
  unsigned seed = 0;
  float huber_slope = 1.0f, tweedie_variance_power = 1.5f, poisson_max_delta_step = 0.7f;
};

struct SplitCand {
  float loss_chg; int feature; int bin; int dleft; int ord;
  long long GL, HL;
};

struct TreeArrays {
  int *left, *right, *parent, *split_index, *split_bin;
  unsigned char* default_left;
  float *split_cond, *base_weight, *loss_chg, *sum_hess;
};

struct GrowState {
  unsigned* seg_begin; unsigned* seg_count;
  int* hist_slot;
  GH64* node_sum;
  float* root_gain; float* weight;
  SplitCand* best;
  SplitCand* best_group;
  int* level_nodes;
  int* level_count;
  int* build_nid; int* build_sub_nid; int* build_parent_slot; int* build_count;
  unsigned* build_prefix;
  int* part_action;
  unsigned* tile_prefix;
  unsigned* tile_left; unsigned* tile_off;
  unsigned char* flags;
  int* n_nodes; int* n_leaves;
  int* depth; unsigned char* open; int* n_slots; int* lg_done;
  float* lower; float* upper;
  float* scales;
  unsigned* absmax;
};

}
```

sagemaker-xgboost-container_b200/csrc/hist.cu:

```cuda
#include <cuda.h>
#include <cstdlib>
#include <cstring>
#include <map>
#include <mutex>
#include <tuple>
#include <type_traits>
#include "engine.h"
#include "tree.h"

namespace b200 {

constexpr int kSuperRows = 32;
constexpr int kMinRowsPerCta = 4096;
constexpr int kSpillThreshold = 1 << 24;
constexpr int kPlaneBytes = kGroupEntries * 4;
constexpr int kMaxSmem = 232448;
constexpr int kTeamWarps = 4, kTeams = 6, kRootRows = 16 * kTeamWarps;
constexpr int kRootConsumerWarps = kTeamWarps * kTeams;
constexpr int kRootProducerWarps = 3;
constexpr int kRootThreads = (kRootConsumerWarps + kRootProducerWarps) * 32;

template <int K, int N, typename F> __device__ __forceinline__ void static_for(F&& f) {
  if constexpr (K < N) { f(std::integral_constant<int, K>{}); static_for<K + 1, N>(f); }
}
// ... 240 lines not shown

template <bool GONLY, int G>
__device__ __forceinline__ void root_unit(const LaneConst& lc, const unsigned (&ldsoff)[4], unsigned rowaddr, int gq, unsigned hq) {
  constexpr int PL = GONLY ? 1 : 2;
  unsigned ww[4];
#pragma unroll
  for (int j = 0; j < 4; ++j) ww[j] = lds_u32(rowaddr + (unsigned)(G * 32) + ldsoff[j]);
  accumulate16<GONLY, G * PL * kPlaneBytes>(lc, ww, gq, hq);
}

template <bool GONLY>
__global__ void __launch_bounds__(kRootThreads, 1)
hist_root_kernel(const __grid_constant__ CUtensorMap tm, HistArgs a, RootCfg c) {
  constexpr int PL = GONLY ? 1 : 2;
  constexpr int NCW = kRootConsumerWarps, R = kRootRows;
  extern __shared__ __align__(128) unsigned char smem_raw[];
  const int nb = *a.build_count;
  if (nb <= 0) return;
  const unsigned T = a.build_prefix[nb];
  if (T == 0) return;
  const int lane = threadIdx.x & 31, warp = threadIdx.x >> 5;
  const int g0 = blockIdx.y * a.ng_chunk;
  const int ng_here = min(a.ng_chunk, a.ngroups - g0);
  const bool has_tail = a.tw > 0 && blockIdx.y == gridDim.y - 1;
  if (a.rows_counter && blockIdx.x == 0 && blockIdx.y == 0 && threadIdx.x == 0) atomicAdd(a.rows_counter, (unsigned long long)T);

  const unsigned smem_base = (unsigned)__cvta_generic_to_shared(smem_raw);
  const unsigned ring = (smem_base + c.ring_off + 127u) & ~127u;
  const unsigned bars = ring + (unsigned)c.S * c.stage_bytes;
  const unsigned row_bytes = 32u * (unsigned)c.box_groups;
  const unsigned main_tile_bytes = (unsigned)R * row_bytes;
  const unsigned gp_off = main_tile_bytes, tail_tile_off = main_tile_bytes + (unsigned)R * 8u;
  const unsigned ntiles = (T + R - 1) / R;
  const unsigned my_ntiles = ntiles > blockIdx.x ? (ntiles - blockIdx.x + gridDim.x - 1) / gridDim.x : 0u;

  {
    const int main4 = ng_here * PL * kPlaneBytes / 16;
    int4* z = reinterpret_cast<int4*>(smem_raw);
    for (int i = threadIdx.x; i < main4; i += blockDim.x) z[i] = make_int4(0, 0, 0, 0);
    if (has_tail) {
      const int tail4 = PL * 256 * a.tw * c.trep * 4 / 16;
      int4* zt = reinterpret_cast<int4*>(smem_raw + c.tail_off);
      for (int i = threadIdx.x; i < tail4; i += blockDim.x) zt[i] = make_int4(0, 0, 0, 0);
    }
    if (threadIdx.x == 0) {
      for (int s = 0; s < c.S; ++s) { mbar_init(bars + 8u * s, 1); mbar_init(bars + 8u * (c.S + s), kTeamWarps); }
      asm volatile("fence.mbarrier_init.release.cluster;" ::: "memory");
    }
  }
  __syncthreads();

  const int nid = a.build_nid[0];
  const size_t slot_entries = (size_t)a.ngroups * kGroupEntries + (size_t)256 * a.tw;
  GH64* out_slot = a.hist_pool + (size_t)a.hist_slot[nid] * slot_entries;
  GH64* out_main = out_slot + (size_t)g0 * kGroupEntries;
  GH64* out_tail = out_slot + (size_t)a.ngroups * kGroupEntries;

  if (warp >= NCW) {
    if (lane == 0) {
      const unsigned P = (c.flags & 8) ? 1u : (unsigned)kRootProducerWarps, pw = (unsigned)(warp - NCW);
      if (pw < P) {
        const unsigned tx = main_tile_bytes + (unsigned)R * 8u + (has_tail ? (unsigned)R * (unsigned)a.tw : 0u);
        unsigned s = pw % (unsigned)c.S, round = pw / (unsigned)c.S;
        for (unsigned i = pw; i < my_ntiles; i += P) {
          if (round > 0) mbar_wait(bars + 8u * (c.S + s), (round - 1u) & 1u);
          const unsigned full = bars + 8u * s, dst = ring + s * c.stage_bytes;
          const unsigned t = blockIdx.x + i * gridDim.x;
          const unsigned row0 = t * (unsigned)R;
          mbar_expect_tx(full, tx);
          if ((c.flags & 1) && gridDim.y == 1) bulk_load_1d(dst, a.bins + (size_t)row0 * a.row_stride, main_tile_bytes, full);
          else tma_load_2d(dst, &tm, g0 * 32, (int)row0, full);
          bulk_load_1d(dst + gp_off, a.gpair + row0, (unsigned)R * 8u, full);
          if (has_tail) bulk_load_1d(dst + tail_tile_off, a.bins_tail + (size_t)row0 * a.tw, (unsigned)R * (unsigned)a.tw, full);
          const unsigned tp = t + 8u * gridDim.x;
          if (tp < ntiles && !(c.flags & 4)) tma_prefetch_2d(&tm, g0 * 32, (int)(tp * (unsigned)R));
          s += P; if (s >= (unsigned)c.S) { s -= (unsigned)c.S; ++round; }
        }
      }
    }
    return;
  }

  const int team = warp / kTeamWarps, wit = warp % kTeamWarps;
  const float sg = a.scales[0], sh = a.scales[1];
  const LaneConst lc = make_lane_const(lane, smem_base);
  unsigned ldsoff[4];
#pragma unroll
  for (int j = 0; j < 4; ++j) { ldsoff[j] = 16u * (unsigned)(lane & 1) + 4u * (unsigned)((j + lc.qw) & 3); asm volatile("" : "+r"(ldsoff[j])); }
  TailConst tc;
  tc.tw = a.tw; tc.base_g = smem_base + c.tail_off; tc.hplane_bytes = 256u * (unsigned)a.tw * (unsigned)c.trep * 4u;
  tc.bin_stride = (unsigned)a.tw * (unsigned)c.trep * 4u;
  tc.rep_off = has_tail ? (unsigned)((lane / a.tw) % c.trep) * (unsigned)a.tw * 4u : 0u;
  const unsigned rowl = (unsigned)(wit << 4) + (unsigned)(lane >> 1);
  const unsigned tiles_per_window = (unsigned)a.window_rows / R;
  long long accG = 0, accH = 0;
  unsigned i = (unsigned)team, s = (unsigned)team, ph = 0;
  for (unsigned wstart = 0;; wstart += tiles_per_window) {
    const unsigned wend = wstart + tiles_per_window < my_ntiles ? wstart + tiles_per_window : my_ntiles;
    while (i < wend) {
      mbar_wait(bars + 8u * s, ph);
      const unsigned tile = ring + s * c.stage_bytes;
      const unsigned row0 = (blockIdx.x + i * gridDim.x) * (unsigned)R;
      if (!(c.flags & 2)) {
        const uint2 ghb = lds_v2(tile + gp_off + rowl * 8u);
        int gq = 0; unsigned hq = 0;
        if (row0 + rowl < T) { gq = __float2int_rn(__uint_as_float(ghb.x) * sg); hq = (unsigned)__float2int_rn(__uint_as_float(ghb.y) * sh); }
        if ((lane & 1) == 0) { accG += gq; accH += hq; }
        const unsigned rowaddr = tile + rowl * row_bytes;
        root_unit<GONLY, 0>(lc, ldsoff, rowaddr, gq, hq);
        if (ng_here > 1) root_unit<GONLY, 1>(lc, ldsoff, rowaddr, gq, hq);
        if (ng_here > 2) root_unit<GONLY, 2>(lc, ldsoff, rowaddr, gq, hq);
        if (has_tail) {
          const unsigned tu = ((unsigned)wit + i) & (unsigned)(kTeamWarps - 1);
          if (tu < (unsigned)(R >> 5)) {
            const unsigned trow = (tu << 5) + (unsigned)lane;
            unsigned w0, w1 = 0;
            if (a.tw == 4) w0 = lds_u32(tile + tail_tile_off + trow * 4u);
            else { const uint2 ww = lds_v2(tile + tail_tile_off + trow * 8u); w0 = ww.x; w1 = ww.y; }
            const uint2 gt = lds_v2(tile + gp_off + trow * 8u);
            int gqt = 0; unsigned hqt = 0;
            if (row0 + trow < T) { gqt = __float2int_rn(__uint_as_float(gt.x) * sg); hqt = (unsigned)__float2int_rn(__uint_as_float(gt.y) * sh); }
            else { w0 = 0; w1 = 0; }
            tail_accumulate<GONLY>(tc, lane, w0, w1, gqt, hqt);
          }
        }
      }
      __syncwarp();
      if (lane == 0) mbar_arrive(bars + 8u * (c.S + s));
      i += kTeams; s += kTeams;
      if (s >= (unsigned)c.S) { s -= (unsigned)c.S; ph ^= 1u; }
    }
    if (wend == my_ntiles) break;
    named_bar_sync(1, NCW * 32);
    spill_main<PL>(reinterpret_cast<int*>(smem_raw), ng_here, out_main, false, threadIdx.x, NCW * 32);
    if (has_tail) spill_tail<PL>(reinterpret_cast<int*>(smem_raw + c.tail_off), a.tw, c.trep, out_tail, false, threadIdx.x, NCW * 32);
    named_bar_sync(1, NCW * 32);
  }
  named_bar_sync(1, NCW * 32);
  spill_main<PL>(reinterpret_cast<int*>(smem_raw), ng_here, out_main, true, threadIdx.x, NCW * 32);
  if (has_tail) spill_tail<PL>(reinterpret_cast<int*>(smem_raw + c.tail_off), a.tw, c.trep, out_tail, true, threadIdx.x, NCW * 32);
  if (a.accumulate_sum && blockIdx.y == 0) {
#pragma unroll
    for (int o = 16; o > 0; o >>= 1) { accG += __shfl_xor_sync(0xffffffffu, accG, o); accH += __shfl_xor_sync(0xffffffffu, accH, o); }
    if (lane == 0 && (accG != 0 || accH != 0)) { red_global_s64(&a.node_sum[nid].g, accG); red_global_s64(&a.node_sum[nid].h, accH); }
  }
}

template <int TW> struct Stage { unsigned id; float2 gh; unsigned t0; };
template <> struct Stage<8> { unsigned id; float2 gh; unsigned t0, t1; };

__host__ __device__ constexpr int gather_tail_replicas(int ng) { return ng >= 3 ? 4 : 8; }
__host__ __device__ constexpr int gather_tail_bytes(int ng) { return ng >= 3 ? 32768 : 65536; }

template <int NG, int TW, int NTHREADS>
__global__ void __launch_bounds__(NTHREADS, NG == 1 ? (TW ? 1 : 3) : 1) hist_gather_kernel(HistArgs a) {
  constexpr bool TAIL = TW != 0;
  constexpr int NWARPS = NTHREADS / 32;
  constexpr int LPR = 2 * NG, RPI = 32 / LPR, U = 2 * NG;
  constexpr int SUP = RPI * U;
  static_assert(kWindowRowsSmall / (SUP * NWARPS) >= 1, "window too small");
  const unsigned iters_per_window = (unsigned)a.window_rows / (SUP * NWARPS);
  extern __shared__ __align__(16) int smem[];
  const int nb = *a.build_count;
  if (nb <= 0) return;
  const unsigned T = a.build_prefix[nb];
  if (T == 0) return;
  if (a.rows_counter && blockIdx.x == 0 && blockIdx.y == 0 && threadIdx.x == 0) atomicAdd(a.rows_counter, (unsigned long long)T);
  const unsigned C = gridDim.x;
  unsigned ceff = (T + kMinRowsPerCta - 1) / kMinRowsPerCta;
  ceff = ceff < 1 ? 1 : (ceff > C ? C : ceff);
  if (blockIdx.x >= ceff) return;
  unsigned chunk = (T + ceff - 1) / ceff;
  chunk = (chunk + SUP - 1) / SUP * SUP;
  unsigned long long r0l = (unsigned long long)blockIdx.x * chunk;
  if (r0l >= T) return;
  unsigned r0 = (unsigned)r0l;
  unsigned r1 = (unsigned long long)r0 + chunk > T ? T : r0 + chunk;
  const int g0 = blockIdx.y * a.ng_chunk;
  const int ng_here = min(min(a.ng_chunk, NG), a.ngroups - g0);
  const bool has_tail = TAIL && a.tw > 0 && blockIdx.y == gridDim.y - 1;
  const float sg = a.scales[0], sh = a.scales[1];
  const unsigned smem_g = (unsigned)__cvta_generic_to_shared(smem);
  const bool aligned = a.ridx != nullptr && a.bins_gather != nullptr;
  const int64_t row_stride = aligned ? (int64_t)a.gather_stride : (int64_t)a.row_stride;
  const int lane = threadIdx.x & 31, warp = threadIdx.x >> 5;
  const int q = lane / LPR, c = lane - q * LPR;
  const bool lane_on = q < RPI && (c >> 1) < ng_here;
  const int rot = q < RPI ? NG * q + (c >> 1) : 15;
  const LaneConst lc = make_lane_const_rot(rot, c & 1, smem_g + (unsigned)((q < RPI ? (c >> 1) : 0) * 2 * kPlaneBytes));
  const int rot_qw = rot >> 2, rot_qb8 = (rot & 3) * 8;
  const uint8_t* gbins = (aligned ? a.bins_gather : a.bins) + (int64_t)g0 * kSlots + c * 16;
  constexpr int TWC = TAIL ? TW : 4;
  constexpr int trep = gather_tail_replicas(NG) < gather_tail_bytes(NG) / (2 * 256 * 4 * TWC) ? gather_tail_replicas(NG) : gather_tail_bytes(NG) / (2 * 256 * 4 * TWC);
  const unsigned tail_base_rep = smem_g + (unsigned)(NG * 2 * kPlaneBytes) + (unsigned)((lane / TWC) % trep) * (unsigned)TWC * 4u;

  {
    const int words4 = (NG * 2 * kPlaneBytes + (TAIL ? 2 * 256 * TWC * trep * 4 : 0)) / 16;
    for (int i = threadIdx.x; i < words4; i += NTHREADS) reinterpret_cast<int4*>(smem)[i] = make_int4(0, 0, 0, 0);
  }
  __syncthreads();

  int b = 0;
  { int lo = 0, hi = nb; while (lo < hi) { int mid = (lo + hi) >> 1; if (a.build_prefix[mid + 1] > r0) hi = mid; else lo = mid + 1; } b = lo; }

  const size_t slot_entries = (size_t)a.ngroups * kGroupEntries + (size_t)256 * a.tw;
  typedef Stage<TW> StageT;
  while (r0 < r1) {
    const unsigned nbeg = a.build_prefix[b], nend_node = a.build_prefix[b + 1];
    const unsigned nend = nend_node < r1 ? nend_node : r1;
    const int nid = a.build_nid[b];
    const unsigned seg = a.seg_begin[nid];
    GH64* out_slot = a.hist_pool + (size_t)a.hist_slot[nid] * slot_entries;
    GH64* out_main = out_slot + (size_t)g0 * kGroupEntries;
    GH64* out_tail = out_slot + (size_t)a.ngroups * kGroupEntries;
    int accG = 0; unsigned accH = 0;
    const unsigned pa = seg + (r0 - nbeg), pb = seg + (nend - nbeg);
    const unsigned nsuper = (pb - pa + SUP - 1) / SUP;
    const unsigned iters = (nsuper + NWARPS - 1) / NWARPS;

    auto load_ids = [&](unsigned st) -> StageT {
      StageT s_; s_.id = 0xffffffffu; s_.gh = make_float2(0.f, 0.f); s_.t0 = 0u;
      if constexpr (TW == 8) s_.t1 = 0u;
      unsigned p = pa + st * SUP + lane;
      if (lane < SUP && st < nsuper && p < pb) {
        s_.id = a.ridx ? __ldg(a.ridx + p) : p; s_.gh = ldg_nc_f2(a.gpair + p);
        if (TAIL && has_tail) {
          if constexpr (TW == 8) { const uint2 v = ldg_nc_v2(a.bins_tail + (int64_t)s_.id * 8); s_.t0 = v.x; s_.t1 = v.y; }
          else if (a.tail_pos) s_.t0 = ldg_nc_u32(a.tail_pos + p);
          else s_.t0 = ldg_nc_u32(a.bins_tail + (int64_t)s_.id * 4);
        }
      }
      return s_;
    };
    auto load_unit = [&](unsigned ids, int k) -> uint4 {
      const unsigned rid = __shfl_sync(0xffffffffu, ids, q < RPI ? k * RPI + q : 0);
      return (lane_on && rid != 0xffffffffu) ? ldg_nc_v4(gbins + (int64_t)rid * row_stride) : make_uint4(0, 0, 0, 0);
    };
    StageT cur = load_ids(warp);
    StageT nxt = load_ids(warp + NWARPS);
    uint4 w[U];
#pragma unroll
    for (int k = 0; k < U; ++k) w[k] = load_unit(cur.id, k);
    for (unsigned it = 0; it < iters; ++it) {
      const unsigned s = warp + it * NWARPS;
      StageT nn = load_ids(s + 2 * NWARPS);
      const bool active = s < nsuper;
      const int gq_l = __float2int_rn(cur.gh.x * sg);
      const unsigned hq_l = (unsigned)__float2int_rn(cur.gh.y * sh);
      accG += gq_l; accH += hq_l;
#pragma unroll
      for (int k = 0; k < U; ++k) {
        if (active) {
          int gq = __shfl_sync(0xffffffffu, gq_l, q < RPI ? k * RPI + q : 0);
          unsigned hq = __shfl_sync(0xffffffffu, hq_l, q < RPI ? k * RPI + q : 0);
          if (!lane_on) { gq = 0; hq = 0; }
          unsigned ww[4];
          rotate_words_bytes(rot_qw, rot_qb8, w[k], ww);
          accumulate16_pairs_prerotated<0>(lc.A, ww, gq, hq);
        }
        w[k] = load_unit(nxt.id, k);
      }
      if constexpr (TAIL) { if (active && has_tail) { unsigned t1 = 0; if constexpr (TW == 8) t1 = cur.t1; tail_accumulate_ct<TWC, trep>(tail_base_rep, lane, cur.t0, t1, gq_l, hq_l); } }
      cur = nxt; nxt = nn;
      if ((it + 1) % iters_per_window == 0 && it + 1 < iters) {
        if (a.accumulate_sum && blockIdx.y == 0) { flush_node_sum(a.node_sum + nid, accG, accH, lane); accG = 0; accH = 0; }
        __syncthreads();
        spill_main<2>(smem, ng_here, out_main, false, threadIdx.x, NTHREADS);
        if (has_tail) spill_tail<2>(smem + NG * 2 * kGroupEntries, TWC, trep, out_tail, false, threadIdx.x, NTHREADS);
        __syncthreads();
      }
    }
    __syncthreads();
    spill_main<2>(smem, ng_here, out_main, true, threadIdx.x, NTHREADS);
    if (has_tail) spill_tail<2>(smem + NG * 2 * kGroupEntries, TWC, trep, out_tail, true, threadIdx.x, NTHREADS);
    __syncthreads();
    if (a.accumulate_sum && blockIdx.y == 0) flush_node_sum(a.node_sum + nid, accG, accH, lane);
    r0 = nend; ++b;
  }
}

static thread_local const char* g_last_kernel = "none";
const char* hist_last_kernel() { return g_last_kernel; }

static int chunks_for(int ngroups) { return (ngroups + 2) / 3; }
static int groups_per_chunk(int ngroups) { const int nc = chunks_for(ngroups); return (ngroups + nc - 1) / nc; }

static bool root_plan(int ngc, int tw, bool gonly, RootCfg* c) {
  const int PL = gonly ? 1 : 2;
  const unsigned main_b = (unsigned)ngc * PL * kPlaneBytes;
  const unsigned avail = kMaxSmem - 128  - 2 * 8 * 16 ;
  const unsigned stage = (unsigned)kRootRows * (32u * ngc + 8u + tw);
  int trep = tw ? 32 / tw : 0;
  unsigned tail_b = (unsigned)PL * 256u * tw * trep * 4u;
  if (tw && main_b + tail_b + kTeams * stage > avail) { trep = 1; tail_b = (unsigned)PL * 256u * tw * 4u; }
  if (main_b + tail_b + kTeams * stage > avail) return false;
  int S = (int)((avail - main_b - tail_b) / stage);
  int smax = 16;
  if (const char* e = getenv("B200XGB_ROOT_S")) smax = atoi(e);
  if (S > smax) S = smax;
  constexpr int kStageQuantum = kTeams % kRootProducerWarps == 0 ? kTeams : kTeams * kRootProducerWarps;
  S -= S % kStageQuantum;
  if (S < kTeams) return false;
  c->S = S; c->trep = trep; c->box_groups = ngc; c->tail_off = main_b; c->ring_off = main_b + tail_b; c->stage_bytes = stage;
  c->total = main_b + tail_b + 128 + (unsigned)S * stage + 2 * 8 * (unsigned)S;
  c->flags = 0;
  if (const char* f = getenv("B200XGB_ROOT_FLAGS")) c->flags = atoi(f);
  return true;
}

typedef CUresult (*EncodeTiledFn)(CUtensorMap*, CUtensorMapDataType, cuuint32_t, void*, const cuuint64_t*, const cuuint64_t*, const cuuint32_t*,
                                  const cuuint32_t*, CUtensorMapInterleave, CUtensorMapSwizzle, CUtensorMapL2promotion, CUtensorMapFloatOOBfill);
static EncodeTiledFn encode_fn() {
  static EncodeTiledFn fn = [] {
    void* p = nullptr; cudaDriverEntryPointQueryResult q;
    if (cudaGetDriverEntryPoint("cuTensorMapEncodeTiled", &p, cudaEnableDefault, &q) != cudaSuccess || q != cudaDriverEntryPointSuccess) { cudaGetLastError(); p = nullptr; }
    return reinterpret_cast<EncodeTiledFn>(p);
  }();
  return fn;
}

static bool get_tensor_map(const uint8_t* bins, int64_t n, int row_stride, int box_groups, int R, CUtensorMap* out) {
  typedef std::tuple<const void*, int64_t, int, int, int> Key;
  static std::map<Key, CUtensorMap> cache; static std::mutex mu;
  std::lock_guard<std::mutex> lk(mu);
  const Key key(bins, n, row_stride, box_groups, R);
  auto it = cache.find(key);
  if (it != cache.end()) { *out = it->second; return true; }
  EncodeTiledFn fn = encode_fn();
  if (!fn) return false;
  CUtensorMap tm;
  const cuuint64_t dims[2] = {(cuuint64_t)row_stride, (cuuint64_t)n};
  const cuuint64_t strides[1] = {(cuuint64_t)row_stride};
  const cuuint32_t box[2] = {(cuuint32_t)(32 * box_groups), (cuuint32_t)R};
  const cuuint32_t estr[2] = {1, 1};
  CUresult r = fn(&tm, CU_TENSOR_MAP_DATA_TYPE_UINT8, 2, const_cast<uint8_t*>(bins), dims, strides, box, estr, CU_TENSOR_MAP_INTERLEAVE_NONE,
                  CU_TENSOR_MAP_SWIZZLE_NONE, CU_TENSOR_MAP_L2_PROMOTION_L2_128B, CU_TENSOR_MAP_FLOAT_OOB_FILL_NONE);
  if (r != CUDA_SUCCESS) return false;
  if (cache.size() > 64) cache.clear();
  cache[key] = tm; *out = tm;
  return true;
}

template <int NG, int TW, int NT> static void set_gather_attr() {
  CUDA_OK(cudaFuncSetAttribute(hist_gather_kernel<NG, TW, NT>, cudaFuncAttributeMaxDynamicSharedMemorySize, NG * 2 * kPlaneBytes + (TW ? gather_tail_bytes(NG) : 0)));
}

void hist_configure() {
  static bool configured = false;
  if (configured) return;
  set_gather_attr<1, 0, 256>(); set_gather_attr<1, 4, 256>(); set_gather_attr<1, 8, 256>();
  set_gather_attr<2, 0, 768>(); set_gather_attr<2, 4, 768>(); set_gather_attr<2, 8, 768>();
  set_gather_attr<3, 0, 768>(); set_gather_attr<3, 4, 768>(); set_gather_attr<3, 8, 768>();
  CUDA_OK(cudaFuncSetAttribute(hist_root_kernel<false>, cudaFuncAttributeMaxDynamicSharedMemorySize, kMaxSmem));
  CUDA_OK(cudaFuncSetAttribute(hist_root_kernel<true>, cudaFuncAttributeMaxDynamicSharedMemorySize, kMaxSmem));
  configured = true;
}

template <int NG, int NT>
static void launch_gather(const HistArgs& a, int gx, int nchunks, cudaStream_t stream) {
  const int smem = NG * 2 * kPlaneBytes + (a.tw ? gather_tail_bytes(NG) : 0);
  if (a.tw == 0) hist_gather_kernel<NG, 0, NT><<<dim3(gx, nchunks), NT, smem, stream>>>(a);
  else if (a.tw == 4) hist_gather_kernel<NG, 4, NT><<<dim3(gx, nchunks), NT, smem, stream>>>(a);
  else hist_gather_kernel<NG, 8, NT><<<dim3(gx, nchunks), NT, smem, stream>>>(a);
}

void launch_hist_build(const HistArgs& a_in, int num_sms, cudaStream_t stream) {
  HistArgs a = a_in;
  const int nchunks = chunks_for(a.ngroups);
  a.ng_chunk = groups_per_chunk(a.ngroups);
  static const bool no_tma = getenv("B200XGB_NO_TMA") != nullptr;
  if (a.ridx == nullptr && !no_tma && !a.force_gather) {
    RootCfg c; CUtensorMap tm;
    const bool gonly = a.g_only != 0;
    if (root_plan(a.ng_chunk, a.tw, gonly, &c) && get_tensor_map(a.bins, a.n, a.row_stride, c.box_groups, kRootRows, &tm)) {
      const int gx = num_sms / nchunks > 0 ? num_sms / nchunks : 1;
      if (gonly) hist_root_kernel<true><<<dim3(gx, nchunks), kRootThreads, c.total, stream>>>(tm, a, c);
      else hist_root_kernel<false><<<dim3(gx, nchunks), kRootThreads, c.total, stream>>>(tm, a, c);
      g_last_kernel = gonly ? "hist_root_kernel<GONLY>" : "hist_root_kernel<GH>";
      ++g_kernel_launches;
      CUDA_OK(cudaGetLastError());
      return;
    }
  }
  B200_CHECK(!a.g_only || a.ridx == nullptr, "hist: G-only accumulation is a root-pass mode");
  B200_CHECK(!a.g_only, "hist: the G-only root pass needs the TMA kernel (tensor-map creation failed or B200XGB_NO_TMA is set)");
  const bool tail = a.tw > 0;
  const int ng = a.ng_chunk;
  if (ng == 1) {
    const int per_sm = tail ? 1 : 3;
    const int gx = (num_sms * per_sm + nchunks - 1) / nchunks;
    launch_gather<1, 256>(a, gx, nchunks, stream);
  } else {
    const int gx = (num_sms + nchunks - 1) / nchunks;
    if (ng == 2) launch_gather<2, 768>(a, gx, nchunks, stream); else launch_gather<3, 768>(a, gx, nchunks, stream);
  }
  g_last_kernel = "hist_gather_kernel";
  ++g_kernel_launches;
  CUDA_OK(cudaGetLastError());
}

}
```

sagemaker-xgboost-container_b200/csrc/tree.cu:

```cuda
#include "engine.h"
#include "tree.h"

namespace b200 {

__device__ __forceinline__ double threshold_l1(double w, double alpha) {
  if (w > +alpha) return w - alpha;
  if (w < -alpha) return w + alpha;
  return 0.0;
}
__device__ __forceinline__ float calc_weight(const TrainParamDev& p, double G, double H) {
  if (H < p.min_child_weight || H <= 0.0) return 0.0f;
  double dw = -threshold_l1(G, p.alpha) / (H + p.lambda);
  if (p.max_delta_step != 0.0f && fabs(dw) > p.max_delta_step) dw = copysign((double)p.max_delta_step, dw);
  return (float)dw;
}
__device__ __forceinline__ float calc_gain_given_weight(const TrainParamDev& p, double G, double H, float w) {
  if (H <= 0.0) return 0.0f;
  if (p.max_delta_step == 0.0f) { double t = threshold_l1(G, p.alpha); return (float)(t * t / (H + p.lambda)); }
  float g = (float)G, h = (float)H;
  return -(2.0f * g * w + (h + p.lambda) * w * w);
}
__device__ __forceinline__ float calc_gain(const TrainParamDev& p, double G, double H) {
  return calc_gain_given_weight(p, G, H, calc_weight(p, G, H));
}
__device__ __forceinline__ float calc_split_gain(const TrainParamDev& p, double GL, double HL, double GR, double HR) {
  float wl = calc_weight(p, GL, HL), wr = calc_weight(p, GR, HR);
  return calc_gain_given_weight(p, GL, HL, wl) + calc_gain_given_weight(p, GR, HR, wr);
}

__device__ __forceinline__ void interaction_children(const ApplyArgs& a, int nid, int f, int Lc, int Rc) {
  if (a.node_allowed == nullptr) return;
  const size_t F = (size_t)a.F;
  unsigned char* pl = a.node_path + (size_t)Lc * F; unsigned char* pr = a.node_path + (size_t)Rc * F;
  unsigned char* al = a.node_allowed + (size_t)Lc * F; unsigned char* ar = a.node_allowed + (size_t)Rc * F;
  const unsigned char* pp = a.node_path + (size_t)nid * F;
  for (int j = 0; j < a.F; ++j) { const unsigned char v = (pp[j] || j == f) ? 1 : 0; pl[j] = v; pr[j] = v; al[j] = v; ar[j] = v; }
  for (int s = 0; s < a.n_ic_sets; ++s) {
    const unsigned char* set = a.ic_sets + (size_t)s * F;
    bool relevant = true;
    for (int j = 0; j < a.F && relevant; ++j) if (pl[j] && !set[j]) relevant = false;
    if (relevant) for (int j = 0; j < a.F; ++j) if (set[j]) { al[j] = 1; ar[j] = 1; }
  }
}

__device__ __forceinline__ float clamp_weight(float w, float lo, float hi) { return w < lo ? lo : (w > hi ? hi : w); }
__device__ __forceinline__ float gain_at_weight(const TrainParamDev& p, double G, double H, float w) {
  if (H <= 0.0) return 0.0f;
  const float g = (float)G, h = (float)H;
  return -(2.0f * g * w + (h + p.lambda) * w * w);
}
__device__ __forceinline__ bool constrained_split_gain(const TrainParamDev& p, double GL, double HL, double GR, double HR, float lo, float hi, int c, float* gain) {
  const float wl = clamp_weight(calc_weight(p, GL, HL), lo, hi), wr = clamp_weight(calc_weight(p, GR, HR), lo, hi);
  *gain = gain_at_weight(p, GL, HL, wl) + gain_at_weight(p, GR, HR, wr);
  return c == 0 || (c > 0 ? wl <= wr : wl >= wr);
}

__device__ __forceinline__ unsigned long long splitmix64_tree(unsigned long long x) {
  x += 0x9E3779B97F4A7C15ULL; x = (x ^ (x >> 30)) * 0xBF58476D1CE4E5B9ULL;
  x = (x ^ (x >> 27)) * 0x94D049BB133111EBULL; return x ^ (x >> 31);
}
__device__ __forceinline__ float rng_uniform_tree(unsigned seed, unsigned long long stream, unsigned long long idx) {
  unsigned long long h = splitmix64_tree(splitmix64_tree(((unsigned long long)seed << 32) ^ stream) ^ idx);
  return (float)(h >> 40) * (1.0f / 16777216.0f);
}

__device__ __forceinline__ unsigned long long cand_key(float loss, int f, int ord) {
  if (!(loss > 0.0f) || isinf(loss)) return 0ull;
  return ((unsigned long long)__float_as_uint(loss) << 32) | ((unsigned long long)(0xFFFFu - (unsigned)f) << 16) |
         (unsigned long long)(0xFFFFu - (unsigned)ord);
}

__global__ void init_tree_kernel(GrowState gs, TreeArrays t, unsigned n, int root_slot, int max_level_nodes) {
  if (threadIdx.x != 0 || blockIdx.x != 0) return;
  *gs.n_nodes = 1; *gs.n_leaves = 1;
  *gs.n_slots = kLgFirstFreeSlot; *gs.lg_done = 0; gs.depth[0] = 0; gs.open[0] = 0;
  gs.lower[0] = -INFINITY; gs.upper[0] = INFINITY;
  for (int d = 0; d < kMaxDepth + 2; ++d) gs.level_count[d] = 0;
  gs.level_count[0] = 1; gs.level_nodes[0] = 0;
  gs.seg_begin[0] = 0; gs.seg_count[0] = n; gs.hist_slot[0] = root_slot;
  gs.node_sum[0].g = 0; gs.node_sum[0].h = 0;
  *gs.build_count = 1; gs.build_nid[0] = 0; gs.build_sub_nid[0] = -1; gs.build_parent_slot[0] = -1;
  gs.build_prefix[0] = 0; gs.build_prefix[1] = n;
  t.left[0] = -1; t.right[0] = -1; t.parent[0] = 2147483647; t.split_index[0] = 0; t.split_bin[0] = -1;
  t.default_left[0] = 0; t.split_cond[0] = 0.f; t.base_weight[0] = 0.f; t.loss_chg[0] = 0.f; t.sum_hess[0] = 0.f;
  (void)max_level_nodes;
}

__global__ void scales_kernel(GrowState gs, int grad_bits) {
  if (threadIdx.x != 0 || blockIdx.x != 0) return;
  float mg = __uint_as_float(gs.absmax[0]), mh = __uint_as_float(gs.absmax[1]);
  int eg = 0, eh = 0;
  if (mg > 0.f && isfinite(mg)) frexpf(mg, &eg);
  if (mh > 0.f && isfinite(mh)) frexpf(mh, &eh);
  float sg = ldexpf(1.0f, grad_bits - eg), sh = ldexpf(1.0f, grad_bits + 1 - eh);
  gs.scales[0] = sg; gs.scales[1] = sh; gs.scales[2] = 1.0f / sg; gs.scales[3] = 1.0f / sh;
}

constexpr int kEvalSegs = 32, kEvalBinsPerSeg = kBins / kEvalSegs;
__global__ void __launch_bounds__(32 * kEvalSegs) eval_kernel(EvalArgs a) {
  const int li = blockIdx.x;
  if (li >= a.gs.level_count[a.level]) return;
  const int nid = a.gs.level_nodes[(size_t)a.level * a.max_level_nodes + li];
  const int group = blockIdx.y;
  const bool is_tail = group == a.ngroups;
  const int nblocks = a.ngroups + (a.tw > 0 ? 1 : 0);
  const int64_t slot_entries = (int64_t)a.ngroups * kGroupEntries + 256 * a.tw;
  const GH64* hist = a.hist_pool + (int64_t)a.gs.hist_slot[nid] * slot_entries + (int64_t)group * kGroupEntries;
  const int stride = is_tail ? a.tw : kSlots;
  const int slot = threadIdx.x & 31, seg = threadIdx.x >> 5;
  const int f = group * kSlots + slot;
  bool active = slot < stride && f < a.F && (a.feat_mask == nullptr || a.feat_mask[f] != 0);
  if (active && a.node_allowed != nullptr) active = a.node_allowed[(size_t)nid * a.F + f] != 0;
  if (a.feat_mask != nullptr && a.colsample_bynode < 1.0f) {
    __shared__ int s_rank[32], s_cnt;
    if (threadIdx.x < 32) s_rank[threadIdx.x] = 0;
    if (threadIdx.x == 0) s_cnt = 0;
    __syncthreads();
    const unsigned long long stream = 0x80000000ull + ((unsigned long long)(unsigned)*a.tree_index << 20) + (unsigned long long)nid;
    const float uf = rng_uniform_tree(a.seed, stream, (unsigned long long)f);
    int rank = 0, cnt = 0;
    for (int g = seg; g < a.F; g += kEvalSegs) {
      if (a.feat_mask[g]) { ++cnt; const float ug = rng_uniform_tree(a.seed, stream, (unsigned long long)g); rank += (ug < uf || (ug == uf && g < f)) ? 1 : 0; }
    }
    if (rank) atomicAdd(&s_rank[slot], rank);
    if (slot == 0 && cnt) atomicAdd(&s_cnt, cnt);
    __syncthreads();
    const int keep = max(1, (int)floorf(a.colsample_bynode * (float)s_cnt));
    active = active && s_rank[slot] < keep;
  }
  const int nbf = active ? a.cut_ptrs[f + 1] - a.cut_ptrs[f] : 0;
  const double isg = (double)a.gs.scales[2], ish = (double)a.gs.scales[3];
  const GH64 tot = a.gs.node_sum[nid];
  const double G = (double)tot.g * isg, H = (double)tot.h * ish;
  const bool mono = a.monotone != nullptr;
  const float w_lo = mono ? a.gs.lower[nid] : 0.f, w_hi = mono ? a.gs.upper[nid] : 0.f;
  const int mono_c = (mono && active) ? a.monotone[f] : 0;
  const float node_w = mono ? clamp_weight(calc_weight(a.p, G, H), w_lo, w_hi) : calc_weight(a.p, G, H);
  const float root_gain = mono ? gain_at_weight(a.p, G, H, node_w) : calc_gain(a.p, G, H);
  if (threadIdx.x == 0 && group == 0) { a.gs.root_gain[nid] = root_gain; a.gs.weight[nid] = node_w; }

  __shared__ long long segG[kEvalSegs][32], segH[kEvalSegs][32];
  __shared__ unsigned long long wkey[kEvalSegs];
  const int b0 = seg * kEvalBinsPerSeg;
  GH64 vals[kEvalBinsPerSeg];
  long long sG = 0, sH = 0;
#pragma unroll
  for (int i = 0; i < kEvalBinsPerSeg; ++i) { int b = b0 + i; GH64 v; v.g = 0; v.h = 0; if (b < nbf) v = hist[b * stride + slot]; vals[i] = v; sG += v.g; sH += v.h; }
  segG[seg][slot] = sG; segH[seg][slot] = sH;
  __syncthreads();
  long long pG = 0, pH = 0, tG = 0, tH = 0;
#pragma unroll 8
  for (int s = 0; s < kEvalSegs; ++s) { long long x = segG[s][slot], y = segH[s][slot]; if (s < seg) { pG += x; pH += y; } tG += x; tH += y; }
  const bool fmiss = a.has_missing && (tG != tot.g || tH != tot.h);

  SplitCand best; best.loss_chg = 0.f; best.feature = 0; best.bin = -1; best.dleft = 0; best.ord = 0; best.GL = 0; best.HL = 0;
  unsigned long long bkey = 0ull;
  const double mcw = (double)a.p.min_child_weight;
  long long cG = pG, cH = pH;
#pragma unroll
  for (int i = 0; i < kEvalBinsPerSeg; ++i) {
    int b = b0 + i;
    if (b < nbf) {
      GH64 v = vals[i]; cG += v.g; cH += v.h;
      double GL = (double)cG * isg, HL = (double)cH * ish;
      double GR = (double)(tot.g - cG) * isg, HR = (double)(tot.h - cH) * ish;
      if (HL >= mcw && HR >= mcw) {
        float lc;
        if (mono) { float gsum; lc = constrained_split_gain(a.p, GL, HL, GR, HR, w_lo, w_hi, mono_c, &gsum) ? gsum - root_gain : 0.0f; }
        else lc = calc_split_gain(a.p, GL, HL, GR, HR) - root_gain;
        unsigned long long k = cand_key(lc, f, b);
        if (k > bkey) { bkey = k; best.loss_chg = lc; best.feature = f; best.bin = b; best.dleft = 0; best.ord = b; best.GL = cG; best.HL = cH; }
      }
    }
  }
  if (fmiss) {
    long long rG = tG - pG, rH = tH - pH;
#pragma unroll
    for (int i = 0; i < kEvalBinsPerSeg; ++i) {
      int b = b0 + i;
      if (b < nbf) {
        long long lG = tot.g - rG, lH = tot.h - rH;
        double GL = (double)lG * isg, HL = (double)lH * ish, GR = (double)rG * isg, HR = (double)rH * ish;
        if (HR >= mcw && HL >= mcw) {
          float lc;
          if (mono) { float gsum; lc = constrained_split_gain(a.p, GL, HL, GR, HR, w_lo, w_hi, mono_c, &gsum) ? gsum - root_gain : 0.0f; }
          else lc = calc_split_gain(a.p, GL, HL, GR, HR) - root_gain;
          int ord = 256 + (255 - b);
          unsigned long long k = cand_key(lc, f, ord);
          if (k > bkey) { bkey = k; best.loss_chg = lc; best.feature = f; best.bin = b - 1; best.dleft = 1; best.ord = ord; best.GL = lG; best.HL = lH; }
        }
        GH64 v = vals[i]; rG -= v.g; rH -= v.h;
      }
    }
  }
  unsigned long long k = bkey;
#pragma unroll
  for (int o = 16; o > 0; o >>= 1) { unsigned long long x = __shfl_xor_sync(0xffffffffu, k, o); k = x > k ? x : k; }
  if ((threadIdx.x & 31) == 0) wkey[seg] = k;
  __syncthreads();
  unsigned long long m = 0ull;
#pragma unroll 8
  for (int s = 0; s < kEvalSegs; ++s) m = wkey[s] > m ? wkey[s] : m;
  SplitCand* out = a.gs.best_group + (size_t)nid * nblocks + group;
  if (m == 0ull) { if (threadIdx.x == 0) { SplitCand z; z.loss_chg = 0.f; z.feature = 0; z.bin = -1; z.dleft = 0; z.ord = 0; z.GL = 0; z.HL = 0; *out = z; } }
  else if (bkey == m) *out = best;
}

__device__ unsigned block_exclusive_scan(const unsigned* in, unsigned* out, int n, unsigned* s_tmp ) {
  unsigned carry = 0;
  const int lane = threadIdx.x & 31, warp = threadIdx.x >> 5, nw = blockDim.x >> 5;
  for (int base = 0; base < n; base += blockDim.x) {
    int i = base + threadIdx.x;
    unsigned v = i < n ? in[i] : 0u, x = v;
#pragma unroll
    for (int o = 1; o < 32; o <<= 1) { unsigned y = __shfl_up_sync(0xffffffffu, x, o); if (lane >= o) x += y; }
    if (lane == 31) s_tmp[warp] = x;
    __syncthreads();
    if (warp == 0) {
      unsigned w = lane < nw ? s_tmp[lane] : 0u, z = w;
#pragma unroll
      for (int o = 1; o < 32; o <<= 1) { unsigned y = __shfl_up_sync(0xffffffffu, z, o); if (lane >= o) z += y; }
      s_tmp[lane] = z - w;
      if (lane == 31) s_tmp[32] = z;
    }
    __syncthreads();
    if (i < n) out[i] = carry + s_tmp[warp] + x - v;
    carry += s_tmp[32];
    __syncthreads();
  }
  return carry;
}

__global__ void __launch_bounds__(256) apply_kernel(ApplyArgs a) {
  __shared__ unsigned s_tmp[33];
  GrowState& gs = a.gs; TreeArrays& t = a.tree;
  const int L = a.level;
  const int cnt = gs.level_count[L];
  const int* nodes = gs.level_nodes + (size_t)L * a.max_level_nodes;
  unsigned* valid = a.scratch;
  unsigned* rank = a.scratch + a.max_level_nodes;
  unsigned* tiles = a.scratch + 2 * (size_t)a.max_level_nodes;
  const double isg = (double)gs.scales[2], ish = (double)gs.scales[3];
  if (L == 0 && threadIdx.x == 0 && cnt > 0) {
    t.base_weight[0] = gs.weight[0]; t.sum_hess[0] = (float)((double)gs.node_sum[0].h * ish);
    t.split_cond[0] = a.p.eta * gs.weight[0];
  }
  for (int i = threadIdx.x; i < cnt; i += blockDim.x) {
    const int nid = nodes[i];
    SplitCand best = gs.best_group[(size_t)nid * a.ngroups];
    unsigned long long bk = cand_key(best.loss_chg, best.feature, best.ord);
    for (int g = 1; g < a.ngroups; ++g) {
      SplitCand c = gs.best_group[(size_t)nid * a.ngroups + g];
      unsigned long long k = cand_key(c.loss_chg, c.feature, c.ord);
      if (k > bk) { bk = k; best = c; }
    }
    gs.best[nid] = best;
    const GH64 tot = gs.node_sum[nid];
    bool ok = best.loss_chg > 1e-6f;
    if (ok && (best.HL == 0 || tot.h - best.HL == 0)) ok = false;
    if (ok && best.loss_chg < a.p.gamma) ok = false;
    if (ok && a.p.max_depth > 0 && L >= a.p.max_depth) ok = false;
    valid[i] = ok ? 1u : 0u;
  }
  __syncthreads();
  if (a.p.max_leaves > 0 && threadIdx.x == 0) {
    int leaves = *gs.n_leaves;
    for (int i = 0; i < cnt; ++i) { if (valid[i]) { if (leaves >= a.p.max_leaves) valid[i] = 0; else ++leaves; } }
  }
  __syncthreads();
  const unsigned nvalid = block_exclusive_scan(valid, rank, cnt, s_tmp);
  const int n0 = *gs.n_nodes;
  const bool children_evaluated = (L + 1 < a.p.max_depth) || a.p.max_depth == 0;
  for (int i = threadIdx.x; i < cnt; i += blockDim.x) {
    const int nid = nodes[i];
    tiles[i] = (gs.seg_count[nid] + kPartTile - 1) / kPartTile;
    gs.part_action[i] = (int)valid[i];
    if (!valid[i]) continue;
    const SplitCand best = gs.best[nid];
    const GH64 tot = gs.node_sum[nid];
    const int r = (int)rank[i];
    const int Lc = n0 + 2 * r, Rc = Lc + 1;
    const long long GLq = best.GL, HLq = best.HL, GRq = tot.g - best.GL, HRq = tot.h - best.HL;
    const double GL = (double)GLq * isg, HL = (double)HLq * ish, GR = (double)GRq * isg, HR = (double)HRq * ish;
    float wl = calc_weight(a.p, GL, HL), wr = calc_weight(a.p, GR, HR);
    if (a.monotone) {
      const float lo = gs.lower[nid], hi = gs.upper[nid];
      wl = clamp_weight(wl, lo, hi); wr = clamp_weight(wr, lo, hi);
      const float mid = (wl + wr) / 2.0f; const int mc = a.monotone[best.feature];
      gs.lower[Lc] = lo; gs.upper[Lc] = hi; gs.lower[Rc] = lo; gs.upper[Rc] = hi;
      if (mc < 0) { gs.lower[Lc] = mid; gs.upper[Rc] = mid; } else if (mc > 0) { gs.upper[Lc] = mid; gs.lower[Rc] = mid; }
    }
    interaction_children(a, nid, best.feature, Lc, Rc);
    const int cb = a.cut_ptrs[best.feature];
    float thr = best.dleft ? (best.bin < 0 ? a.min_vals[best.feature] : a.cut_vals[cb + best.bin]) : a.cut_vals[cb + best.bin];
    t.left[nid] = Lc; t.right[nid] = Rc; t.split_index[nid] = best.feature; t.split_cond[nid] = thr;
    t.split_bin[nid] = best.bin; t.default_left[nid] = (unsigned char)best.dleft;
    t.base_weight[nid] = gs.weight[nid]; t.loss_chg[nid] = best.loss_chg; t.sum_hess[nid] = (float)((double)tot.h * ish);
    const int ch[2] = {Lc, Rc}; const float cw[2] = {wl, wr}; const double chh[2] = {HL, HR};
    for (int s = 0; s < 2; ++s) {
      int c = ch[s];
      t.left[c] = -1; t.right[c] = -1; t.parent[c] = nid; t.split_index[c] = 0; t.split_bin[c] = -1; t.default_left[c] = 0;
      t.split_cond[c] = a.p.eta * cw[s]; t.base_weight[c] = a.p.eta * cw[s]; t.loss_chg[c] = 0.f; t.sum_hess[c] = (float)chh[s];
    }
    gs.node_sum[Lc].g = GLq; gs.node_sum[Lc].h = HLq; gs.node_sum[Rc].g = GRq; gs.node_sum[Rc].h = HRq;
    gs.seg_begin[Lc] = 0; gs.seg_count[Lc] = 0; gs.seg_begin[Rc] = 0; gs.seg_count[Rc] = 0;
    if (children_evaluated) {
      int* nxt = gs.level_nodes + (size_t)(L + 1) * a.max_level_nodes;
      nxt[2 * r] = Lc; nxt[2 * r + 1] = Rc;
      const bool fewer_right = HRq < HLq;
      const int bld = fewer_right ? Rc : Lc, sub = fewer_right ? Lc : Rc;
      gs.hist_slot[bld] = a.next_base + r; gs.hist_slot[sub] = a.next_base + a.next_half + r;
      gs.build_nid[r] = bld; gs.build_sub_nid[r] = sub; gs.build_parent_slot[r] = gs.hist_slot[nid];
    }
  }
  __syncthreads();
  const unsigned total_tiles = block_exclusive_scan(tiles, gs.tile_prefix, cnt, s_tmp);
  if (threadIdx.x == 0) {
    gs.tile_prefix[cnt] = total_tiles;
    *gs.n_nodes = n0 + 2 * (int)nvalid;
    *gs.n_leaves += (int)nvalid;
    gs.level_count[L + 1] = children_evaluated ? 2 * (int)nvalid : 0;
    *gs.build_count = children_evaluated ? (int)nvalid : 0;
  }
}

__global__ void __launch_bounds__(256) apply_lossguide_kernel(ApplyArgs a, int iter) {
  __shared__ unsigned long long s_key[8];
  GrowState& gs = a.gs; TreeArrays& t = a.tree;
  const double isg = (double)gs.scales[2], ish = (double)gs.scales[3];
  const int src = iter == 0 ? 0 : 1;
  const int cnt = gs.level_count[src];
  const int* nodes = gs.level_nodes + (size_t)src * a.max_level_nodes;
  if (iter == 0 && threadIdx.x == 0 && cnt > 0) {
    t.base_weight[0] = gs.weight[0]; t.sum_hess[0] = (float)((double)gs.node_sum[0].h * ish); t.split_cond[0] = a.p.eta * gs.weight[0];
  }
  for (int i = threadIdx.x; i < cnt; i += blockDim.x) {
    const int nid = nodes[i];
    SplitCand best = gs.best_group[(size_t)nid * a.ngroups];
    unsigned long long bk = cand_key(best.loss_chg, best.feature, best.ord);
    for (int g = 1; g < a.ngroups; ++g) {
      SplitCand c = gs.best_group[(size_t)nid * a.ngroups + g];
      unsigned long long k = cand_key(c.loss_chg, c.feature, c.ord);
      if (k > bk) { bk = k; best = c; }
    }
    gs.best[nid] = best;
    gs.open[nid] = best.loss_chg > 1e-6f ? 1 : 0;
  }
  __syncthreads();
  const int n0 = *gs.n_nodes;
  unsigned long long key = 0ull;
  for (int nid = threadIdx.x; nid < n0; nid += blockDim.x)
    if (gs.open[nid]) { unsigned long long k = ((unsigned long long)__float_as_uint(gs.best[nid].loss_chg) << 32) | (unsigned long long)(0xffffffffu - (unsigned)nid); key = k > key ? k : key; }
#pragma unroll
  for (int o = 16; o > 0; o >>= 1) { unsigned long long x = __shfl_xor_sync(0xffffffffu, key, o); key = x > key ? x : key; }
  if ((threadIdx.x & 31) == 0) s_key[threadIdx.x >> 5] = key;
  __syncthreads();
  if (threadIdx.x != 0) return;
  for (int w = 1; w < 8; ++w) key = s_key[w] > key ? s_key[w] : key;
  bool stop = *gs.lg_done != 0 || key == 0ull;
  int nid = 0; SplitCand best{}; GH64 tot{};
  if (!stop) {
    nid = (int)(0xffffffffu - (unsigned)(key & 0xffffffffull));
    best = gs.best[nid]; tot = gs.node_sum[nid];
    bool ok = best.loss_chg > 1e-6f;
    if (ok && (best.HL == 0 || tot.h - best.HL == 0)) ok = false;
    if (ok && best.loss_chg < a.p.gamma) ok = false;
    if (ok && a.p.max_depth > 0 && gs.depth[nid] == a.p.max_depth) ok = false;
    if (ok && a.p.max_leaves > 0 && *gs.n_leaves == a.p.max_leaves) ok = false;
    stop = !ok;
  }
  if (stop) {
    *gs.lg_done = 1;
    gs.level_count[0] = 0; gs.level_count[1] = 0; *gs.build_count = 0; gs.part_action[0] = 0; gs.tile_prefix[0] = 0; gs.tile_prefix[1] = 0;
    return;
  }
  gs.open[nid] = 0;
  const int Lc = n0, Rc = n0 + 1, d = gs.depth[nid];
  const long long GLq = best.GL, HLq = best.HL, GRq = tot.g - best.GL, HRq = tot.h - best.HL;
  const double GL = (double)GLq * isg, HL = (double)HLq * ish, GR = (double)GRq * isg, HR = (double)HRq * ish;
  float wl = calc_weight(a.p, GL, HL), wr = calc_weight(a.p, GR, HR);
  if (a.monotone) {
    const float lo = gs.lower[nid], hi = gs.upper[nid];
    wl = clamp_weight(wl, lo, hi); wr = clamp_weight(wr, lo, hi);
    const float mid = (wl + wr) / 2.0f; const int mc = a.monotone[best.feature];
    gs.lower[Lc] = lo; gs.upper[Lc] = hi; gs.lower[Rc] = lo; gs.upper[Rc] = hi;
    if (mc < 0) { gs.lower[Lc] = mid; gs.upper[Rc] = mid; } else if (mc > 0) { gs.upper[Lc] = mid; gs.lower[Rc] = mid; }
  }
  interaction_children(a, nid, best.feature, Lc, Rc);
  const int cb = a.cut_ptrs[best.feature];
  const float thr = best.dleft ? (best.bin < 0 ? a.min_vals[best.feature] : a.cut_vals[cb + best.bin]) : a.cut_vals[cb + best.bin];
  t.left[nid] = Lc; t.right[nid] = Rc; t.split_index[nid] = best.feature; t.split_cond[nid] = thr;
  t.split_bin[nid] = best.bin; t.default_left[nid] = (unsigned char)best.dleft;
  t.base_weight[nid] = gs.weight[nid]; t.loss_chg[nid] = best.loss_chg; t.sum_hess[nid] = (float)((double)tot.h * ish);
  const int ch[2] = {Lc, Rc}; const float cw[2] = {wl, wr}; const double chh[2] = {HL, HR};
  for (int s = 0; s < 2; ++s) {
    const int c = ch[s];
    t.left[c] = -1; t.right[c] = -1; t.parent[c] = nid; t.split_index[c] = 0; t.split_bin[c] = -1; t.default_left[c] = 0;
    t.split_cond[c] = a.p.eta * cw[s]; t.base_weight[c] = a.p.eta * cw[s]; t.loss_chg[c] = 0.f; t.sum_hess[c] = (float)chh[s];
    gs.depth[c] = d + 1; gs.open[c] = 0;
  }
  gs.node_sum[Lc].g = GLq; gs.node_sum[Lc].h = HLq; gs.node_sum[Rc].g = GRq; gs.node_sum[Rc].h = HRq;
  gs.seg_begin[Lc] = 0; gs.seg_count[Lc] = 0; gs.seg_begin[Rc] = 0; gs.seg_count[Rc] = 0;
  *gs.n_nodes = n0 + 2;
  const int leaves = *gs.n_leaves + 1;
  *gs.n_leaves = leaves;
  const bool children_evaluated = !(a.p.max_depth > 0 && d + 1 >= a.p.max_depth) && !(a.p.max_leaves > 0 && leaves >= a.p.max_leaves);
  gs.level_nodes[0] = nid; gs.level_count[0] = 1;
  gs.part_action[0] = children_evaluated ? 1 : 0;
  gs.tile_prefix[0] = 0; gs.tile_prefix[1] = children_evaluated ? (gs.seg_count[nid] + kPartTile - 1) / kPartTile : 0u;
  if (children_evaluated) {
    int* nxt = gs.level_nodes + (size_t)a.max_level_nodes;
    nxt[0] = Lc; nxt[1] = Rc; gs.level_count[1] = 2;
    const bool fewer_right = HRq < HLq;
    const int bld = fewer_right ? Rc : Lc, sub = fewer_right ? Lc : Rc;
    const int slot = (*gs.n_slots)++;
    gs.hist_slot[bld] = slot; gs.hist_slot[sub] = gs.hist_slot[nid];
    gs.build_nid[0] = bld; gs.build_sub_nid[0] = sub; gs.build_parent_slot[0] = gs.hist_slot[nid];
    *gs.build_count = 1;
  } else { gs.level_count[1] = 0; *gs.build_count = 0; }
}

__global__ void __launch_bounds__(256) lg_copy_back_kernel(PartArgs a, unsigned* ridx_dst, float2* gp_dst, unsigned* tl_dst) {
  const GrowState& gs = a.gs;
  if (gs.level_count[0] <= 0 || !gs.part_action[0]) return;
  const int nid = gs.level_nodes[0];
  const unsigned b = gs.seg_begin[nid], c = gs.seg_count[nid];
  for (unsigned p = b + blockIdx.x * blockDim.x + threadIdx.x; p < b + c; p += gridDim.x * blockDim.x) {
    ridx_dst[p] = a.ridx_next[p]; gp_dst[p] = a.gp_next[p];
    if (a.tl_next) tl_dst[p] = a.tl_next[p];
  }
}

__global__ void __launch_bounds__(256) zero_build_slots_kernel(GrowState gs, GH64* pool, size_t stride) {
  const int r = blockIdx.x;
  if (r >= *gs.build_count) return;
  GH64* h = pool + (size_t)gs.hist_slot[gs.build_nid[r]] * stride;
  GH64 z; z.g = 0; z.h = 0;
  for (size_t e = (size_t)blockIdx.y * blockDim.x + threadIdx.x; e < stride; e += (size_t)gridDim.y * blockDim.x) h[e] = z;
}

__global__ void __launch_bounds__(256) lg_stage_kernel(GrowState gs, GH64* pool, size_t stride, int to_stage) {
  if (*gs.build_count <= 0) return;
  GH64* slot = pool + (size_t)gs.hist_slot[gs.build_nid[0]] * stride;
  GH64* stage = pool + (size_t)kLgStageSlot * stride;
  for (size_t e = (size_t)blockIdx.x * blockDim.x + threadIdx.x; e < stride; e += (size_t)gridDim.x * blockDim.x) {
    if (to_stage) stage[e] = slot[e]; else slot[e] = stage[e];
  }
}

__device__ __forceinline__ int find_node_of_tile(const unsigned* tile_prefix, int cnt, unsigned tile) {
  int lo = 0, hi = cnt;
  while (hi - lo > 1) { int mid = (lo + hi) >> 1; if (tile_prefix[mid] <= tile) lo = mid; else hi = mid; }
  return lo;
}

__global__ void __launch_bounds__(256) part_count_kernel(PartArgs a) {
  const GrowState& gs = a.gs;
  const int cnt = gs.level_count[a.level];
  if (cnt <= 0) return;
  const unsigned tile = blockIdx.x;
  if (tile >= gs.tile_prefix[cnt]) return;
  const int i = find_node_of_tile(gs.tile_prefix, cnt, tile);
  if (!gs.part_action[i]) return;
  const int nid = gs.level_nodes[(size_t)a.level * a.max_level_nodes + i];
  const unsigned lt = tile - gs.tile_prefix[i];
  const unsigned b = gs.seg_begin[nid], c = gs.seg_count[nid];
  const unsigned p0 = b + lt * kPartTile, p1 = (b + c < p0 + kPartTile) ? b + c : p0 + kPartTile;
  const int f = a.tree.split_index[nid];
  const int sb = a.tree.split_bin[nid], dl = a.tree.default_left[nid];
  const uint8_t* col = a.bins_col + (int64_t)f * a.n;
  unsigned nleft = 0;
  const unsigned pt = p0 + threadIdx.x * 8;
#pragma unroll
  for (int j = 0; j < 8; ++j) {
    unsigned p = pt + j;
    if (p < p1) {
      unsigned r = a.ridx_cur ? a.ridx_cur[p] : p;
      int byte = col[r];
      bool left = (a.has_missing && byte == kMissingBin) ? (dl != 0) : (byte <= sb);
      gs.flags[p] = left ? 1 : 0; nleft += left ? 1u : 0u;
    }
  }
  __shared__ unsigned s_cnt[8];
#pragma unroll
  for (int o = 16; o > 0; o >>= 1) nleft += __shfl_xor_sync(0xffffffffu, nleft, o);
  if ((threadIdx.x & 31) == 0) s_cnt[threadIdx.x >> 5] = nleft;
  __syncthreads();
  if (threadIdx.x == 0) { unsigned tsum = 0; for (int w = 0; w < 8; ++w) tsum += s_cnt[w]; gs.tile_left[tile] = tsum; }
}

struct PackedNode { unsigned short feat_dl; unsigned short bin_plus1; unsigned short left, right; };
constexpr int kPackedNodesSmem = 2048;

__global__ void __launch_bounds__(256) update_margin_kernel(TreeArrays t, const int* n_nodes, const uint8_t* bins_col, int64_t n, int has_missing,
                                                            float* margin, int K, int k) {
  __shared__ PackedNode s_nodes[kPackedNodesSmem];
  __shared__ float s_leaf[kPackedNodesSmem];
  const int nn = *n_nodes;
  const bool packed = nn <= kPackedNodesSmem && nn < 0xffff;
  if (packed) {
    for (int i = threadIdx.x; i < nn; i += blockDim.x) {
      PackedNode p; p.feat_dl = (unsigned short)(t.split_index[i] | (t.default_left[i] ? 0x8000 : 0)); p.bin_plus1 = (unsigned short)(t.split_bin[i] + 1);
      const int l = t.left[i]; p.left = l < 0 ? 0xffff : (unsigned short)l; p.right = l < 0 ? 0xffff : (unsigned short)t.right[i];
      s_nodes[i] = p; s_leaf[i] = t.split_cond[i];
    }
    __syncthreads();
  }
  const int64_t base = (int64_t)blockIdx.x * 1024 + threadIdx.x;
  int nid[4]; bool done[4];
  const bool root_leaf = packed ? (s_nodes[0].left == 0xffff) : (t.left[0] == -1);
#pragma unroll
  for (int j = 0; j < 4; ++j) { nid[j] = 0; done[j] = (base + j * 256 >= n) || root_leaf; }
  bool any = !(done[0] && done[1] && done[2] && done[3]);
  while (any) {
    int byte[4];
#pragma unroll
    for (int j = 0; j < 4; ++j) {
      const int f = packed ? (int)(s_nodes[nid[j]].feat_dl & 0x7fff) : t.split_index[nid[j]];
      byte[j] = done[j] ? 0 : bins_col[(int64_t)f * n + base + j * 256];
    }
    any = false;
#pragma unroll
    for (int j = 0; j < 4; ++j) {
      if (done[j]) continue;
      const int nd = nid[j];
      if (packed) {
        const PackedNode p = s_nodes[nd];
        const bool left = (has_missing && byte[j] == kMissingBin) ? ((p.feat_dl & 0x8000) != 0) : (byte[j] < (int)p.bin_plus1);
        nid[j] = left ? p.left : p.right;
        done[j] = s_nodes[nid[j]].left == 0xffff;
      } else {
        const bool left = (has_missing && byte[j] == kMissingBin) ? (t.default_left[nd] != 0) : (byte[j] <= t.split_bin[nd]);
        nid[j] = left ? t.left[nd] : t.right[nd];
        done[j] = t.left[nid[j]] == -1;
      }
      any |= !done[j];
    }
  }
#pragma unroll
  for (int j = 0; j < 4; ++j) { const int64_t r = base + j * 256; if (r < n) margin[r * K + k] += packed ? s_leaf[nid[j]] : t.split_cond[nid[j]]; }
}

__global__ void __launch_bounds__(1024) part_scan_kernel(PartArgs a) {
  __shared__ unsigned s_tmp[33];
  const GrowState& gs = a.gs;
  const int cnt = gs.level_count[a.level];
  const int i = blockIdx.x;
  if (i >= cnt || !gs.part_action[i]) return;
  const int nid = gs.level_nodes[(size_t)a.level * a.max_level_nodes + i];
  const unsigned t0 = gs.tile_prefix[i], t1 = gs.tile_prefix[i + 1];
  const unsigned nl = block_exclusive_scan(gs.tile_left + t0, gs.tile_off + t0, (int)(t1 - t0), s_tmp);
  if (threadIdx.x == 0) {
    const unsigned b = gs.seg_begin[nid], c = gs.seg_count[nid];
    const int Lc = a.tree.left[nid], Rc = a.tree.right[nid];
    gs.seg_begin[Lc] = b; gs.seg_count[Lc] = nl; gs.seg_begin[Rc] = b + nl; gs.seg_count[Rc] = c - nl;
  }
}

__global__ void __launch_bounds__(256) part_scatter_kernel(PartArgs a) {
  const GrowState& gs = a.gs;
  const int cnt = gs.level_count[a.level];
  if (cnt <= 0) return;
  const unsigned tile = blockIdx.x;
  if (tile >= gs.tile_prefix[cnt]) return;
  const int i = find_node_of_tile(gs.tile_prefix, cnt, tile);
  if (!gs.part_action[i]) return;
  const int nid = gs.level_nodes[(size_t)a.level * a.max_level_nodes + i];
  const unsigned lt = tile - gs.tile_prefix[i];
  const unsigned b = gs.seg_begin[nid], c = gs.seg_count[nid];
  const unsigned p0 = b + lt * kPartTile, p1 = (b + c < p0 + kPartTile) ? b + c : p0 + kPartTile;
  const unsigned nrows = p1 - p0;
  const unsigned nl = gs.seg_count[a.tree.left[nid]];
  const unsigned toff = gs.tile_off[tile];
  const unsigned pt = p0 + threadIdx.x * 8;
  __shared__ unsigned s_rid[kPartTile];
  __shared__ float2 s_gp[kPartTile];
  __shared__ unsigned s_tl[kPartTile];
  __shared__ unsigned s_w[8];
  const bool has_tl = a.tl_cur != nullptr;
  unsigned rows[8]; float2 gp[8]; unsigned tl[8]; unsigned char fl[8]; unsigned mine = 0;
#pragma unroll
  for (int j = 0; j < 8; ++j) {
    unsigned p = pt + j;
    if (p < p1) { rows[j] = a.ridx_cur ? a.ridx_cur[p] : p; gp[j] = a.gp_cur[p]; tl[j] = has_tl ? a.tl_cur[p] : 0u; fl[j] = gs.flags[p]; mine += fl[j]; }
    else { rows[j] = 0; gp[j] = make_float2(0.f, 0.f); tl[j] = 0u; fl[j] = 2; }
  }
  const int lane = threadIdx.x & 31, warp = threadIdx.x >> 5;
  unsigned x = mine;
#pragma unroll
  for (int o = 1; o < 32; o <<= 1) { unsigned y = __shfl_up_sync(0xffffffffu, x, o); if (lane >= o) x += y; }
  if (lane == 31) s_w[warp] = x;
  __syncthreads();
  unsigned woff = 0, tile_left = 0;
  for (int w = 0; w < 8; ++w) { if (w < warp) woff += s_w[w]; tile_left += s_w[w]; }
  unsigned lbefore = woff + x - mine;
#pragma unroll
  for (int j = 0; j < 8; ++j) {
    if (fl[j] == 2) continue;
    unsigned jj = threadIdx.x * 8 + j;
    unsigned slot = fl[j] ? lbefore++ : tile_left + (jj - lbefore);
    s_rid[slot] = rows[j]; s_gp[slot] = gp[j]; if (has_tl) s_tl[slot] = tl[j];
  }
  __syncthreads();
  const unsigned dl = b + toff, dr = b + nl + (lt * kPartTile - toff);
  for (unsigned k = threadIdx.x; k < nrows; k += blockDim.x) {
    unsigned dest = k < tile_left ? dl + k : dr + (k - tile_left);
    a.ridx_next[dest] = s_rid[k];
    a.gp_next[dest] = s_gp[k];
    if (has_tl) a.tl_next[dest] = s_tl[k];
  }
}

__global__ void __launch_bounds__(256) build_prefix_kernel(GrowState gs) {
  __shared__ unsigned s_tmp[33];
  const int nb = *gs.build_count;
  if (nb <= 0) { if (threadIdx.x == 0) gs.build_prefix[0] = 0; return; }
  unsigned* tmp = gs.tile_left;
  for (int i = threadIdx.x; i < nb; i += blockDim.x) tmp[i] = gs.seg_count[gs.build_nid[i]];
  __syncthreads();
  unsigned total = block_exclusive_scan(tmp, gs.build_prefix, nb, s_tmp);
  if (threadIdx.x == 0) gs.build_prefix[nb] = total;
}

__global__ void __launch_bounds__(256) subtract_kernel(GrowState gs, GH64* pool, size_t stride) {
  const int r = blockIdx.x;
  if (r >= *gs.build_count) return;
  const int bld = gs.build_nid[r], sub = gs.build_sub_nid[r];
  const GH64* hb = pool + (size_t)gs.hist_slot[bld] * stride;
  const GH64* hp = pool + (size_t)gs.build_parent_slot[r] * stride;
  GH64* hs = pool + (size_t)gs.hist_slot[sub] * stride;
  for (size_t e = (size_t)blockIdx.y * blockDim.x + threadIdx.x; e < stride; e += (size_t)gridDim.y * blockDim.x) {
    GH64 p = hp[e], b = hb[e]; GH64 o; o.g = p.g - b.g; o.h = p.h - b.h; hs[e] = o;
  }
}

void launch_init_tree(const GrowState& gs, const TreeArrays& t, unsigned n, int root_slot, int max_level_nodes, cudaStream_t s) {
  init_tree_kernel<<<1, 32, 0, s>>>(gs, t, n, root_slot, max_level_nodes); ++g_kernel_launches; CUDA_OK(cudaGetLastError());
}
void launch_scales(const GrowState& gs, int grad_bits, cudaStream_t s) { scales_kernel<<<1, 32, 0, s>>>(gs, grad_bits); ++g_kernel_launches; CUDA_OK(cudaGetLastError()); }
void launch_eval(const EvalArgs& a, int max_nodes_level, cudaStream_t s) {
  dim3 grid(max_nodes_level, a.ngroups + (a.tw > 0 ? 1 : 0)); eval_kernel<<<grid, 32 * kEvalSegs, 0, s>>>(a); ++g_kernel_launches; CUDA_OK(cudaGetLastError());
}
void launch_apply_lossguide(const ApplyArgs& a, int iter, cudaStream_t s) { apply_lossguide_kernel<<<1, 256, 0, s>>>(a, iter); ++g_kernel_launches; CUDA_OK(cudaGetLastError()); }
void launch_lg_copy_back(const PartArgs& a, unsigned* ridx_dst, float2* gp_dst, unsigned* tl_dst, unsigned max_tiles, cudaStream_t s) {
  lg_copy_back_kernel<<<max_tiles < 1184u ? max_tiles : 1184u, 256, 0, s>>>(a, ridx_dst, gp_dst, tl_dst); ++g_kernel_launches; CUDA_OK(cudaGetLastError());
}
void launch_zero_build_slots(const GrowState& gs, GH64* pool, size_t slot_entries, int max_build, cudaStream_t s) {
  dim3 grid(max_build, (unsigned)((slot_entries + 1023) / 1024)); zero_build_slots_kernel<<<grid, 256, 0, s>>>(gs, pool, slot_entries); ++g_kernel_launches; CUDA_OK(cudaGetLastError());
}
void launch_lg_stage(const GrowState& gs, GH64* pool, size_t slot_entries, int to_stage, cudaStream_t s) {
  lg_stage_kernel<<<(unsigned)((slot_entries + 1023) / 1024), 256, 0, s>>>(gs, pool, slot_entries, to_stage); ++g_kernel_launches; CUDA_OK(cudaGetLastError());
}
void launch_apply(const ApplyArgs& a, cudaStream_t s) { apply_kernel<<<1, 256, 0, s>>>(a); ++g_kernel_launches; CUDA_OK(cudaGetLastError()); }
void launch_partition(const PartArgs& a, unsigned max_tiles, int max_nodes_level, cudaStream_t s) {
  part_count_kernel<<<max_tiles, 256, 0, s>>>(a); ++g_kernel_launches; CUDA_OK(cudaGetLastError());
  part_scan_kernel<<<max_nodes_level, 1024, 0, s>>>(a); ++g_kernel_launches; CUDA_OK(cudaGetLastError());
  part_scatter_kernel<<<max_tiles, 256, 0, s>>>(a); ++g_kernel_launches; CUDA_OK(cudaGetLastError());
  build_prefix_kernel<<<1, 256, 0, s>>>(a.gs); ++g_kernel_launches; CUDA_OK(cudaGetLastError());
}
void launch_update_margin(const TreeArrays& t, const int* n_nodes, const uint8_t* bins_col, int64_t n, int has_missing, float* margin, int K, int k, cudaStream_t s) {
  if (n == 0) return;
  update_margin_kernel<<<(unsigned)((n + 1023) / 1024), 256, 0, s>>>(t, n_nodes, bins_col, n, has_missing, margin, K, k); ++g_kernel_launches; CUDA_OK(cudaGetLastError());
}
void launch_subtract(const GrowState& gs, GH64* pool, size_t slot_entries, int max_build, cudaStream_t s) {
  dim3 grid(max_build, (unsigned)((slot_entries + 1023) / 1024)); subtract_kernel<<<grid, 256, 0, s>>>(gs, pool, slot_entries); ++g_kernel_launches; CUDA_OK(cudaGetLastError());
}

}
```

sagemaker-xgboost-container_b200/csrc/tree.h:

```cpp
#pragma once
#include "engine.h"

namespace b200 {

constexpr unsigned kPartTile = 2048;

struct TrainParamDev {
  float eta, lambda, alpha, gamma, min_child_weight, max_delta_step;
  int max_depth, max_leaves;
};

struct EvalArgs {
  const GH64* hist_pool; GrowState gs; const int* cut_ptrs; const unsigned char* feat_mask;
  TrainParamDev p; int F, ngroups, tw, ntail, has_missing, level, max_level_nodes;
  const int* monotone;
  const unsigned char* node_allowed;
  float colsample_bynode; unsigned seed; const int* tree_index;
};

struct ApplyArgs {
  GrowState gs; TreeArrays tree; const int* cut_ptrs; const float* cut_vals; const float* min_vals;
  TrainParamDev p; unsigned* scratch; int ngroups , level, max_level_nodes, next_base, next_half;
  const int* monotone;
  unsigned char* node_path; unsigned char* node_allowed; const unsigned char* ic_sets; int n_ic_sets, F;
};

struct PartArgs {
  GrowState gs; TreeArrays tree; const uint8_t* bins_col; int64_t n; const unsigned* ridx_cur; unsigned* ridx_next;
  const float2* gp_cur; float2* gp_next;
  const unsigned* tl_cur; unsigned* tl_next;
  int has_missing, level, max_level_nodes;
};

struct HistArgs {
  const uint8_t* bins;
  const uint8_t* bins_tail;
  const unsigned* tail_pos;
  int64_t n;
  int row_stride;
  const uint8_t* bins_gather;
  int gather_stride;
  int tw;
  const float2* gpair;
  const unsigned* ridx;
  const int* build_count;
  const int* build_nid;
  const unsigned* build_prefix;
  const unsigned* seg_begin;
  const int* hist_slot;
  const float* scales;
  GH64* hist_pool;
  GH64* node_sum;
  int ngroups;
  int ng_chunk;
  int accumulate_sum;
  int g_only;
  int window_rows;
  int force_gather;
  unsigned long long* rows_counter;
};

constexpr int kLgRootSlot = 0, kLgStageSlot = 1, kLgFirstFreeSlot = 2;
void launch_apply_lossguide(const ApplyArgs& a, int iter, cudaStream_t s);
void launch_lg_copy_back(const PartArgs& a, unsigned* ridx_dst, float2* gp_dst, unsigned* tl_dst, unsigned max_tiles, cudaStream_t s);
void launch_zero_build_slots(const GrowState& gs, GH64* pool, size_t slot_entries, int max_build, cudaStream_t s);
void launch_lg_stage(const GrowState& gs, GH64* pool, size_t slot_entries, int to_stage, cudaStream_t s);
void launch_hist_build(const HistArgs& a, int num_sms, cudaStream_t stream);
void hist_configure();
const char* hist_last_kernel();
void launch_init_tree(const GrowState& gs, const TreeArrays& t, unsigned n, int root_slot, int max_level_nodes, cudaStream_t s);
void launch_scales(const GrowState& gs, int grad_bits, cudaStream_t s);
void launch_eval(const EvalArgs& a, int max_nodes_level, cudaStream_t s);
void launch_apply(const ApplyArgs& a, cudaStream_t s);
void launch_partition(const PartArgs& a, unsigned max_tiles, int max_nodes_level, cudaStream_t s);
void launch_update_margin(const TreeArrays& t, const int* n_nodes, const uint8_t* bins_col, int64_t n, int has_missing, float* margin, int K, int k, cudaStream_t s);
void launch_subtract(const GrowState& gs, GH64* pool, size_t slot_entries, int max_build, cudaStream_t s);

}
```

Baseline: 113.8.

## Fuse partition into single persistent kernel and carry G-only payload when hessian constant

Replaces the four-launch partition sequence (count, scan, scatter, build-prefix) with one persistent partition kernel sized by occupancy. Tiles coordinate through a part_sync array, which looks like a decoupled look-back, instead of separate flag, tile_left and tile_off buffers. When the hessian is constant, it moves only the gradient float rather than a float2 pair and feeds that to the histogram kernels. This is meant to cut launch overhead and partition memory traffic, at the cost of added cross-block synchronization complexity. It also adds per-level partition profiling and a microbenchmark script.

```diff
diff --git a/microbench/partition_levels.py b/microbench/partition_levels.py
--- /dev/null
+++ b/microbench/partition_levels.py
@@ -0,0 +1,77 @@
+#!/usr/bin/env python
+import argparse
+import json
+import os
+import subprocess
+import sys
+
+ROOT = os.path.dirname(os.path.dirname(os.path.abspath(__file__)))
+sys.path.insert(0, ROOT)
+
+
+def bytes_per_row(level, gonly, tail4):
+    pay = 4 if gonly else 8
+    rd = (0 if level == 0 else 4) + 1 + (8 if level == 0 else pay) + (4 if tail4 else 0)
+    wr = 4 + pay + (4 if tail4 else 0)
+    return rd + wr
+
+
+def card():
+    try:
+        q = subprocess.run(["nvidia-smi", "--query-gpu=name,power.limit", "--format=csv,noheader"], capture_output=True, text=True, timeout=60)
+        return q.stdout.strip().splitlines()[0]
+    except (OSError, IndexError, subprocess.SubprocessError):
+        return "unknown"
+
+
+def main():
+    ap = argparse.ArgumentParser()
+    ap.add_argument("--rows", type=int, default=50_000_000)
+    ap.add_argument("--cols", type=int, default=100)
+    ap.add_argument("--depth", type=int, default=6)
+    ap.add_argument("--warmup", type=int, default=3)
+    ap.add_argument("--rounds", type=int, default=5)
+    ap.add_argument("--out", default="")
+    a = ap.parse_args()
+    import torch
+    import bench
+    import sagemaker_xgboost_container_b200 as xgb
+    be = xgb.get_backend()
+    dev = torch.device("cuda", 0)
+    ba = argparse.Namespace(rows=a.rows, cols=a.cols, seed=43, objective="reg:squarederror", num_class=0)
+    X, y = bench.gen_shard(ba, 0, a.rows, dev)
+    d = xgb.DMatrix(X, label=y.cpu().numpy())
+    del X
+    torch.cuda.empty_cache()
+    bst = xgb.Booster(dict(objective="reg:squarederror", tree_method="hist", max_depth=a.depth, eta=0.3, max_bin=256), [d])
+    it = 0
+    for _ in range(a.warmup):
+        bst.update(d, it); it += 1
+    be.booster_set_profile(bst.handle, True)
+    for _ in range(a.rounds):
+        bst.update(d, it); it += 1
+    prof = be.booster_get_profile(bst.handle)
+    be.booster_set_profile(bst.handle, False)
+    peak, peak_src = bench.hbm_peak()
+    gonly = "B200XGB_NO_CONSTH" not in os.environ
+    tail4 = 1 <= a.cols % 32 <= 4 and a.cols >= 32
+    levels = []
+    for L, (ms, rows) in enumerate(zip(prof["part_level_ms"], prof["part_level_rows"])):
+        nb = bytes_per_row(L, gonly, tail4)
+        ms_round = ms / a.rounds
+        gbs = rows * nb / (ms * 1e-3) / 1e9 if ms > 0 else 0.0
+        levels.append(dict(level=L, ms_per_round=ms_round, rows_per_round=rows // a.rounds, bytes_per_row=nb, gbs=gbs, frac_of_peak=gbs / peak))
+        print("level %d  %8.3f ms  %10d rows  %2d B/row  %7.1f GB/s  (%.2f of %s %.0f GB/s)" % (L, ms_round, rows // a.rounds, nb, gbs, gbs / peak, peak_src, peak))
+    total = prof["part_ms"] / a.rounds
+    print("partition per round: %.3f ms in %d launches; payload %s" % (total, prof["part_launches"] // a.rounds, "g" if gonly else "(g,h)"))
+    res = dict(workload="synthetic %dx%d reg:squarederror depth %d" % (a.rows, a.cols, a.depth), card=card(), payload="g" if gonly else "gh",
+               part_ms_per_round=total, launches_per_round=prof["part_launches"] / a.rounds, levels=levels, peak_gbs=peak, peak_source=peak_src,
+               timing="CUDA events around each partition launch, %d profiled rounds after %d warm-up rounds (direct launches)" % (a.rounds, a.warmup))
+    print(json.dumps(res))
+    if a.out:
+        os.makedirs(os.path.dirname(os.path.abspath(a.out)), exist_ok=True)
+        json.dump(res, open(a.out, "w"), indent=1)
+
+
+if __name__ == "__main__":
+    main()
diff --git a/sagemaker-xgboost-container_b200/csrc/booster.cu b/sagemaker-xgboost-container_b200/csrc/booster.cu
--- a/sagemaker-xgboost-container_b200/csrc/booster.cu
+++ b/sagemaker-xgboost-container_b200/csrc/booster.cu
@@ -315,8 +315,8 @@
     size_t o_best = take(sizeof(SplitCand) * N), o_bestg = take(sizeof(SplitCand) * N * (ngroups + (tw > 0 ? 1 : 0)));
     size_t o_lnodes = take(4 * (size_t)(kMaxDepth + 1) * L), o_lcount = take(4 * (kMaxDepth + 2));
     size_t o_bnid = take(4 * L), o_bsub = take(4 * L), o_bps = take(4 * L), o_bcount = take(4), o_bprefix = take(4 * (L + 1));
-    size_t o_action = take(4 * L), o_tprefix = take(4 * (L + 1)), o_tleft = take(4 * (size_t)max_tiles), o_toff = take(4 * (size_t)max_tiles);
-    size_t o_flags = take((size_t)n + 16), o_nleaves = take(4), o_scales = take(16), o_absmax = take(8);
+    size_t o_action = take(4 * L), o_tprefix = take(4 * (L + 1)), o_psync = take(8 * (2 + (size_t)max_tiles));
+    size_t o_nleaves = take(4), o_scales = take(16), o_absmax = take(8);
     size_t o_depth = take(4 * N), o_open = take(N), o_nslots = take(4), o_lgdone = take(4), o_lower = take(4 * N), o_upper = take(4 * N);
     state_block.alloc(off); state_block.zero(engine_stream());
     unsigned char* b = state_block.p;
@@ -326,10 +326,10 @@
     gs.level_nodes = (int*)(b + o_lnodes); gs.level_count = (int*)(b + o_lcount);
     gs.build_nid = (int*)(b + o_bnid); gs.build_sub_nid = (int*)(b + o_bsub); gs.build_parent_slot = (int*)(b + o_bps);
     gs.build_count = (int*)(b + o_bcount); gs.build_prefix = (unsigned*)(b + o_bprefix);
-    gs.part_action = (int*)(b + o_action); gs.tile_prefix = (unsigned*)(b + o_tprefix); gs.tile_left = (unsigned*)(b + o_tleft); gs.tile_off = (unsigned*)(b + o_toff);
+    gs.part_action = (int*)(b + o_action); gs.tile_prefix = (unsigned*)(b + o_tprefix); gs.part_sync = (unsigned long long*)(b + o_psync);
     gs.lower = (float*)(b + o_lower); gs.upper = (float*)(b + o_upper);
     gs.depth = (int*)(b + o_depth); gs.open = b + o_open; gs.n_slots = (int*)(b + o_nslots); gs.lg_done = (int*)(b + o_lgdone);
-    gs.flags = b + o_flags; gs.n_leaves = (int*)(b + o_nleaves); gs.scales = (float*)(b + o_scales); gs.absmax = (unsigned*)(b + o_absmax);
+    gs.n_leaves = (int*)(b + o_nleaves); gs.scales = (float*)(b + o_scales); gs.absmax = (unsigned*)(b + o_absmax);
     tree_block_bytes = 64 + 9 * 4 * N + N;
     tree_block.alloc(tree_block_bytes);
     unsigned char* t = tree_block.p;
@@ -339,7 +339,7 @@
     float* fp = (float*)(ip + 5 * N);
     ta.split_cond = fp; ta.base_weight = fp + N; ta.loss_chg = fp + 2 * N; ta.sum_hess = fp + 3 * N;
     ta.default_left = (unsigned char*)(fp + 4 * N);
-    hist_configure();
+    hist_configure(); partition_configure();
     global_n = n;
     if (Comm::get().distributed()) {
       peer_reduce_setup({{hist_pool.p, hist_pool.n * sizeof(GH64)}, {state_block.p, state_block.n}}, engine_stream());
@@ -687,6 +687,9 @@
   const BinnedMatrix bm = dtrain->binned_view();
   const int num_sms = engine_num_sms();
   const unsigned max_tiles = (unsigned)((dtrain->n + kPartTile - 1) / kPartTile) + g.max_level_nodes + 1;
+  const bool gonly = root_mode != 0;
+  const float* gpair_g = reinterpret_cast<const float*>(g.gpair.p + (size_t)k * g.gp_stride);
+  float* g_buf0 = reinterpret_cast<float*>(g.gp0.p); float* g_buf1 = reinterpret_cast<float*>(g.gp1.p);
 
   launch_init_tree(g.gs, g.ta, (unsigned)dtrain->n, 0, g.max_level_nodes, s);
   if (root_mode == 2) { slot_from_cache_kernel<<<148, 256, 0, s>>>(g.hist_pool.p, g.root_h_cache.p, g.slot_stride); ++g_kernel_launches; CUDA_OK(cudaGetLastError()); }
@@ -747,13 +750,17 @@
     const bool carry_tail = bm.tw == 4;
     PartArgs pa{}; pa.gs = g.gs; pa.tree = g.ta; pa.bins_col = bm.bins_col; pa.n = bm.n;
     pa.ridx_cur = it == 0 ? nullptr : g.ridx0.p; pa.ridx_next = g.ridx1.p;
-    pa.gp_cur = it == 0 ? g.gpair.p + (size_t)k * g.gp_stride : g.gp0.p; pa.gp_next = g.gp1.p;
+    if (gonly) { pa.g_cur = it == 0 ? gpair_g : g_buf0; pa.g_stride = it == 0 ? 2 : 1; pa.g_next = g_buf1; }
+    else { pa.gp_cur = it == 0 ? g.gpair.p + (size_t)k * g.gp_stride : g.gp0.p; pa.gp_next = g.gp1.p; }
     pa.tl_cur = !carry_tail ? nullptr : (it == 0 ? reinterpret_cast<const unsigned*>(bm.bins_tail) : g.tl0.p); pa.tl_next = !carry_tail ? nullptr : g.tl1.p;
     pa.has_missing = bm.has_missing; pa.level = 0; pa.max_level_nodes = g.max_level_nodes;
-    launch_partition(pa, max_tiles, 1, s);
-    launch_lg_copy_back(pa, g.ridx0.p, g.gp0.p, g.tl0.p, max_tiles, s);
+    pa.rows_counter = profile_ ? prof_rows_.p + kProfPartRows : nullptr;
+    prof_begin(0, kProfPartition);
+    launch_partition(pa, max_tiles, num_sms, s);
+    prof_end();
+    launch_lg_copy_back(pa, g.ridx0.p, g.gp0.p, g_buf0, g.tl0.p, max_tiles, s);
     launch_zero_build_slots(g.gs, g.hist_pool.p, g.slot_stride, 1, s);
-    ha.ridx = g.ridx0.p; ha.gpair = g.gp0.p; ha.tail_pos = carry_tail ? g.tl0.p : nullptr; ha.accumulate_sum = 0;
+    ha.ridx = g.ridx0.p; ha.gpair = g.gp0.p; ha.g_pos = gonly ? g_buf0 : nullptr; ha.tail_pos = carry_tail ? g.tl0.p : nullptr; ha.accumulate_sum = 0;
     ha.rows_counter = profile_ ? prof_rows_.p + 1 : nullptr;
     prof_begin(1);
     launch_hist_build(ha, num_sms, s);
@@ -779,15 +786,18 @@
     PartArgs pa{}; pa.gs = g.gs; pa.tree = g.ta; pa.bins_col = bm.bins_col; pa.n = bm.n;
     pa.ridx_cur = L == 0 ? nullptr : ((L & 1) ? g.ridx0.p : g.ridx1.p);
     pa.ridx_next = (L & 1) ? g.ridx1.p : g.ridx0.p;
-    pa.gp_cur = L == 0 ? g.gpair.p + (size_t)k * g.gp_stride : ((L & 1) ? g.gp0.p : g.gp1.p);
-    pa.gp_next = (L & 1) ? g.gp1.p : g.gp0.p;
+    if (gonly) { pa.g_cur = L == 0 ? gpair_g : ((L & 1) ? g_buf0 : g_buf1); pa.g_stride = L == 0 ? 2 : 1; pa.g_next = (L & 1) ? g_buf1 : g_buf0; }
+    else { pa.gp_cur = L == 0 ? g.gpair.p + (size_t)k * g.gp_stride : ((L & 1) ? g.gp0.p : g.gp1.p); pa.gp_next = (L & 1) ? g.gp1.p : g.gp0.p; }
     const bool carry_tail = bm.tw == 4;
     pa.tl_cur = !carry_tail ? nullptr : (L == 0 ? reinterpret_cast<const unsigned*>(bm.bins_tail) : ((L & 1) ? g.tl0.p : g.tl1.p));
     pa.tl_next = !carry_tail ? nullptr : ((L & 1) ? g.tl1.p : g.tl0.p);
     pa.has_missing = bm.has_missing; pa.level = L; pa.max_level_nodes = g.max_level_nodes;
-    launch_partition(pa, max_tiles, 1 << L, s);
+    pa.rows_counter = profile_ ? prof_rows_.p + kProfPartRows + L : nullptr;
+    prof_begin(L, kProfPartition);
+    launch_partition(pa, max_tiles, num_sms, s);
+    prof_end();
     CUDA_OK(cudaMemsetAsync(g.hist_pool.p + (size_t)next_base * g.slot_stride, 0, (size_t)next_half * g.slot_stride * sizeof(GH64), s));
-    ha.ridx = pa.ridx_next; ha.gpair = pa.gp_next; ha.tail_pos = pa.tl_next; ha.accumulate_sum = 0;
+    ha.ridx = pa.ridx_next; ha.gpair = pa.gp_next; ha.g_pos = pa.g_next; ha.tail_pos = pa.tl_next; ha.accumulate_sum = 0;
     ha.rows_counter = profile_ ? prof_rows_.p + 1 : nullptr;
     prof_begin(L + 1);
     launch_hist_build(ha, num_sms, s);
@@ -1092,6 +1102,18 @@
     CUDA_OK(cudaGetLastError());
     ha.tail_pos = g.tl0.p;
   }
+  std::vector<float> g_only_pos;
+  if (mode & 8) {
+    B200_CHECK(row_ids != nullptr, "debug_build_root_hist: the G-only payload (mode 8) is a gathered-pass mode and needs row ids");
+    g_only_pos.resize((size_t)rows);
+    for (int64_t i = 0; i < rows; ++i) {
+      B200_CHECK(gpair_host[2 * i + 1] == 1.0f, "debug_build_root_hist: the G-only payload (mode 8) needs h == 1 for every row");
+      g_only_pos[(size_t)i] = gpair_host[2 * i];
+    }
+    float* gpos = reinterpret_cast<float*>(g.gp0.p);
+    CUDA_OK(cudaMemcpyAsync(gpos, g_only_pos.data(), sizeof(float) * rows, cudaMemcpyHostToDevice, s));
+    ha.g_pos = gpos;
+  }
   g.root_h_valid = false;
   cudaEvent_t e0, e1; CUDA_OK(cudaEventCreate(&e0)); CUDA_OK(cudaEventCreate(&e1));
   float total = 0.f;
@@ -1196,13 +1218,13 @@
 
 void Booster::set_profile(bool on) {
   profile_ = on;
-  if (on) { prof_rows_.alloc(2); prof_rows_.zero(engine_stream()); prof_launches_ = 0; }
+  if (on) { prof_rows_.alloc(kProfPartRows + kMaxDepth + 1); prof_rows_.zero(engine_stream()); prof_launches_ = 0; }
   for (auto& e : prof_events_) { cudaEventDestroy(e.a); cudaEventDestroy(e.b); }
   prof_events_.clear();
 }
-void Booster::prof_begin(int level) {
+void Booster::prof_begin(int level, int kind) {
   if (!profile_) return;
-  ProfEvent e; e.level = level;
+  ProfEvent e; e.level = level; e.kind = kind;
   CUDA_OK(cudaEventCreate(&e.a)); CUDA_OK(cudaEventCreate(&e.b));
   CUDA_OK(cudaEventRecord(e.a, engine_stream()));
   prof_events_.push_back(e);
@@ -1215,13 +1237,30 @@
   cudaStream_t s = engine_stream();
   Comm::get().sync_stream(s);
   double root_ms = 0, deep_ms = 0; long long root_n = 0, deep_n = 0;
-  for (auto& e : prof_events_) { float ms = 0; CUDA_OK(cudaEventElapsedTime(&ms, e.a, e.b)); if (e.level == 0) { root_ms += ms; ++root_n; } else { deep_ms += ms; ++deep_n; } }
-  unsigned long long rows[2] = {0, 0};
-  if (prof_rows_.p) CUDA_OK(cudaMemcpy(rows, prof_rows_.p, sizeof rows, cudaMemcpyDeviceToHost));
+  double part_ms[kMaxDepth + 1] = {}; long long part_n[kMaxDepth + 1] = {};
+  for (auto& e : prof_events_) {
+    float ms = 0; CUDA_OK(cudaEventElapsedTime(&ms, e.a, e.b));
+    if (e.kind == kProfPartition) { part_ms[e.level] += ms; ++part_n[e.level]; }
+    else if (e.level == 0) { root_ms += ms; ++root_n; } else { deep_ms += ms; ++deep_n; }
+  }
+  unsigned long long rows[kProfPartRows + kMaxDepth + 1] = {};
+  if (prof_rows_.p) CUDA_OK(cudaMemcpy(rows, prof_rows_.p, sizeof(unsigned long long) * std::min(prof_rows_.n, sizeof rows / sizeof rows[0]), cudaMemcpyDeviceToHost));
+  int levels = 0;
+  for (int l = 0; l <= kMaxDepth; ++l) if (part_n[l]) levels = l + 1;
+  double pms = 0; long long pn = 0; unsigned long long prows = 0;
+  std::string lv_ms, lv_n, lv_rows;
+  for (int l = 0; l < levels; ++l) {
+    pms += part_ms[l]; pn += part_n[l]; prows += rows[kProfPartRows + l];
+    char b[96];
+    snprintf(b, sizeof b, "%s%.6f", l ? "," : "", part_ms[l]); lv_ms += b;
+    snprintf(b, sizeof b, "%s%lld", l ? "," : "", part_n[l]); lv_n += b;
+    snprintf(b, sizeof b, "%s%llu", l ? "," : "", rows[kProfPartRows + l]); lv_rows += b;
+  }
   char buf[512];
-  snprintf(buf, sizeof buf, "{\"root_hist_ms\":%.6f,\"root_hist_launches\":%lld,\"root_hist_rows\":%llu,\"deep_hist_ms\":%.6f,\"deep_hist_launches\":%lld,\"deep_hist_rows\":%llu}",
-           root_ms, root_n, rows[0], deep_ms, deep_n, rows[1]);
-  return buf;
-}
-
-}
+  snprintf(buf, sizeof buf, "{\"root_hist_ms\":%.6f,\"root_hist_launches\":%lld,\"root_hist_rows\":%llu,\"deep_hist_ms\":%.6f,\"deep_hist_launches\":%lld,\"deep_hist_rows\":%llu,"
+           "\"part_ms\":%.6f,\"part_launches\":%lld,\"part_rows\":%llu,",
+           root_ms, root_n, rows[0], deep_ms, deep_n, rows[1], pms, pn, prows);
+  return std::string(buf) + "\"part_level_ms\":[" + lv_ms + "],\"part_level_launches\":[" + lv_n + "],\"part_level_rows\":[" + lv_rows + "]}";
+}
+
+}
diff --git a/sagemaker-xgboost-container_b200/csrc/booster.h b/sagemaker-xgboost-container_b200/csrc/booster.h
--- a/sagemaker-xgboost-container_b200/csrc/booster.h
+++ b/sagemaker-xgboost-container_b200/csrc/booster.h
@@ -124,8 +124,10 @@
   DevBuf<float> pred_margin_, pred_cls_; DevBuf<int> pred_leaf_;
   bool children_adjacent_ = true;
   bool profile_ = false;
-  struct ProfEvent { cudaEvent_t a, b; int level; };
+  enum ProfKind { kProfHist = 0, kProfPartition = 1 };
+  struct ProfEvent { cudaEvent_t a, b; int level; int kind; };
   std::vector<ProfEvent> prof_events_;
+  static constexpr int kProfPartRows = 2;
   DevBuf<unsigned long long> prof_rows_;
   long long prof_launches_ = 0;
 
@@ -138,7 +140,7 @@
   void append_device_tree(int class_id, size_t device_offset, int max_nodes, PendingTree pt);
   void grow_one_tree(DMatrix* dtrain, PredCache& cache, int k, int tree_index);
   void enqueue_tree(DMatrix* dtrain, float* margin, int k, const unsigned char* mask, DevNode* packed_out, int root_mode);
-  void prof_begin(int level);
+  void prof_begin(int level, int kind = kProfHist);
   void prof_end();
   JPtr model_to_json();
   void model_from_json(const JValue& doc);
diff --git a/sagemaker-xgboost-container_b200/csrc/engine.h b/sagemaker-xgboost-container_b200/csrc/engine.h
--- a/sagemaker-xgboost-container_b200/csrc/engine.h
+++ b/sagemaker-xgboost-container_b200/csrc/engine.h
@@ -103,8 +103,7 @@
   unsigned* build_prefix;
   int* part_action;
   unsigned* tile_prefix;
-  unsigned* tile_left; unsigned* tile_off;
-  unsigned char* flags;
+  unsigned long long* part_sync;
   int* n_nodes; int* n_leaves;
   int* depth; unsigned char* open; int* n_slots; int* lg_done;
   float* lower; float* upper;
diff --git a/sagemaker-xgboost-container_b200/csrc/hist.cu b/sagemaker-xgboost-container_b200/csrc/hist.cu
--- a/sagemaker-xgboost-container_b200/csrc/hist.cu
+++ b/sagemaker-xgboost-container_b200/csrc/hist.cu
@@ -416,7 +416,7 @@
 __host__ __device__ constexpr int gather_tail_replicas(int ng) { return ng >= 3 ? 4 : 8; }
 __host__ __device__ constexpr int gather_tail_bytes(int ng) { return ng >= 3 ? 32768 : 65536; }
 
-template <int NG, int TW, int NTHREADS>
+template <int NG, int TW, int NTHREADS, bool GONLY>
 __global__ void __launch_bounds__(NTHREADS, NG == 1 ? (TW ? 1 : 3) : 1) hist_gather_kernel(HistArgs a) {
   constexpr bool TAIL = TW != 0;
   constexpr int NWARPS = NTHREADS / 32;
@@ -444,6 +444,7 @@
   const int ng_here = min(min(a.ng_chunk, NG), a.ngroups - g0);
   const bool has_tail = TAIL && a.tw > 0 && blockIdx.y == gridDim.y - 1;
   const float sg = a.scales[0], sh = a.scales[1];
+  const unsigned hq_one = (unsigned)__float2int_rn(1.0f * sh);
   const unsigned smem_g = (unsigned)__cvta_generic_to_shared(smem);
   const bool aligned = a.ridx != nullptr && a.bins_gather != nullptr;
   const int64_t row_stride = aligned ? (int64_t)a.gather_stride : (int64_t)a.row_stride;
@@ -487,7 +488,8 @@
       if constexpr (TW == 8) s_.t1 = 0u;
       unsigned p = pa + st * SUP + lane;
       if (lane < SUP && st < nsuper && p < pb) {
-        s_.id = a.ridx ? __ldg(a.ridx + p) : p; s_.gh = ldg_nc_f2(a.gpair + p);
+        s_.id = a.ridx ? __ldg(a.ridx + p) : p;
+        if constexpr (GONLY) s_.gh.x = __uint_as_float(ldg_nc_u32(a.g_pos + p)); else s_.gh = ldg_nc_f2(a.gpair + p);
         if (TAIL && has_tail) {
           if constexpr (TW == 8) { const uint2 v = ldg_nc_v2(a.bins_tail + (int64_t)s_.id * 8); s_.t0 = v.x; s_.t1 = v.y; }
           else if (a.tail_pos) s_.t0 = ldg_nc_u32(a.tail_pos + p);
@@ -510,7 +512,7 @@
       StageT nn = load_ids(s + 2 * NWARPS);
       const bool active = s < nsuper;
       const int gq_l = __float2int_rn(cur.gh.x * sg);
-      const unsigned hq_l = (unsigned)__float2int_rn(cur.gh.y * sh);
+      const unsigned hq_l = GONLY ? (cur.id != 0xffffffffu ? hq_one : 0u) : (unsigned)__float2int_rn(cur.gh.y * sh);
       accG += gq_l; accH += hq_l;
 #pragma unroll
       for (int k = 0; k < U; ++k) {
@@ -606,7 +608,9 @@
 }
 
 template <int NG, int TW, int NT> static void set_gather_attr() {
-  CUDA_OK(cudaFuncSetAttribute(hist_gather_kernel<NG, TW, NT>, cudaFuncAttributeMaxDynamicSharedMemorySize, NG * 2 * kPlaneBytes + (TW ? gather_tail_bytes(NG) : 0)));
+  const int smem = NG * 2 * kPlaneBytes + (TW ? gather_tail_bytes(NG) : 0);
+  CUDA_OK(cudaFuncSetAttribute(hist_gather_kernel<NG, TW, NT, false>, cudaFuncAttributeMaxDynamicSharedMemorySize, smem));
+  CUDA_OK(cudaFuncSetAttribute(hist_gather_kernel<NG, TW, NT, true>, cudaFuncAttributeMaxDynamicSharedMemorySize, smem));
 }
 
 void hist_configure() {
@@ -620,12 +624,16 @@
   configured = true;
 }
 
+template <int NG, int NT, bool GONLY>
+static void launch_gather_t(const HistArgs& a, int gx, int nchunks, cudaStream_t stream) {
+  const int smem = NG * 2 * kPlaneBytes + (a.tw ? gather_tail_bytes(NG) : 0);
+  if (a.tw == 0) hist_gather_kernel<NG, 0, NT, GONLY><<<dim3(gx, nchunks), NT, smem, stream>>>(a);
+  else if (a.tw == 4) hist_gather_kernel<NG, 4, NT, GONLY><<<dim3(gx, nchunks), NT, smem, stream>>>(a);
+  else hist_gather_kernel<NG, 8, NT, GONLY><<<dim3(gx, nchunks), NT, smem, stream>>>(a);
+}
 template <int NG, int NT>
 static void launch_gather(const HistArgs& a, int gx, int nchunks, cudaStream_t stream) {
-  const int smem = NG * 2 * kPlaneBytes + (a.tw ? gather_tail_bytes(NG) : 0);
-  if (a.tw == 0) hist_gather_kernel<NG, 0, NT><<<dim3(gx, nchunks), NT, smem, stream>>>(a);
-  else if (a.tw == 4) hist_gather_kernel<NG, 4, NT><<<dim3(gx, nchunks), NT, smem, stream>>>(a);
-  else hist_gather_kernel<NG, 8, NT><<<dim3(gx, nchunks), NT, smem, stream>>>(a);
+  if (a.g_pos) launch_gather_t<NG, NT, true>(a, gx, nchunks, stream); else launch_gather_t<NG, NT, false>(a, gx, nchunks, stream);
 }
 
 void launch_hist_build(const HistArgs& a_in, int num_sms, cudaStream_t stream) {
@@ -658,7 +666,7 @@
     const int gx = (num_sms + nchunks - 1) / nchunks;
     if (ng == 2) launch_gather<2, 768>(a, gx, nchunks, stream); else launch_gather<3, 768>(a, gx, nchunks, stream);
   }
-  g_last_kernel = "hist_gather_kernel";
+  g_last_kernel = a.g_pos ? "hist_gather_kernel<GONLY>" : "hist_gather_kernel";
   ++g_kernel_launches;
   CUDA_OK(cudaGetLastError());
 }
diff --git a/sagemaker-xgboost-container_b200/csrc/tree.cu b/sagemaker-xgboost-container_b200/csrc/tree.cu
--- a/sagemaker-xgboost-container_b200/csrc/tree.cu
+++ b/sagemaker-xgboost-container_b200/csrc/tree.cu
@@ -1,5 +1,7 @@
 #include "engine.h"
 #include "tree.h"
+#include <algorithm>
+#include <type_traits>
 
 namespace b200 {
 
@@ -303,7 +305,8 @@
       t.split_cond[c] = a.p.eta * cw[s]; t.base_weight[c] = a.p.eta * cw[s]; t.loss_chg[c] = 0.f; t.sum_hess[c] = (float)chh[s];
     }
     gs.node_sum[Lc].g = GLq; gs.node_sum[Lc].h = HLq; gs.node_sum[Rc].g = GRq; gs.node_sum[Rc].h = HRq;
-    gs.seg_begin[Lc] = 0; gs.seg_count[Lc] = 0; gs.seg_begin[Rc] = 0; gs.seg_count[Rc] = 0;
+    const unsigned sb0 = gs.seg_begin[nid];
+    gs.seg_begin[Lc] = sb0; gs.seg_count[Lc] = 0; gs.seg_begin[Rc] = sb0; gs.seg_count[Rc] = 0;
     if (children_evaluated) {
       int* nxt = gs.level_nodes + (size_t)(L + 1) * a.max_level_nodes;
       nxt[2 * r] = Lc; nxt[2 * r + 1] = Rc;
@@ -400,7 +403,8 @@
     gs.depth[c] = d + 1; gs.open[c] = 0;
   }
   gs.node_sum[Lc].g = GLq; gs.node_sum[Lc].h = HLq; gs.node_sum[Rc].g = GRq; gs.node_sum[Rc].h = HRq;
-  gs.seg_begin[Lc] = 0; gs.seg_count[Lc] = 0; gs.seg_begin[Rc] = 0; gs.seg_count[Rc] = 0;
+  const unsigned sb0 = gs.seg_begin[nid];
+  gs.seg_begin[Lc] = sb0; gs.seg_count[Lc] = 0; gs.seg_begin[Rc] = sb0; gs.seg_count[Rc] = 0;
   *gs.n_nodes = n0 + 2;
   const int leaves = *gs.n_leaves + 1;
   *gs.n_leaves = leaves;
@@ -420,13 +424,14 @@
   } else { gs.level_count[1] = 0; *gs.build_count = 0; }
 }
 
-__global__ void __launch_bounds__(256) lg_copy_back_kernel(PartArgs a, unsigned* ridx_dst, float2* gp_dst, unsigned* tl_dst) {
+__global__ void __launch_bounds__(256) lg_copy_back_kernel(PartArgs a, unsigned* ridx_dst, float2* gp_dst, float* g_dst, unsigned* tl_dst) {
   const GrowState& gs = a.gs;
   if (gs.level_count[0] <= 0 || !gs.part_action[0]) return;
   const int nid = gs.level_nodes[0];
   const unsigned b = gs.seg_begin[nid], c = gs.seg_count[nid];
   for (unsigned p = b + blockIdx.x * blockDim.x + threadIdx.x; p < b + c; p += gridDim.x * blockDim.x) {
-    ridx_dst[p] = a.ridx_next[p]; gp_dst[p] = a.gp_next[p];
+    ridx_dst[p] = a.ridx_next[p];
+    if (a.g_next) g_dst[p] = a.g_next[p]; else gp_dst[p] = a.gp_next[p];
     if (a.tl_next) tl_dst[p] = a.tl_next[p];
   }
 }
@@ -454,39 +459,135 @@
   return lo;
 }
 
-__global__ void __launch_bounds__(256) part_count_kernel(PartArgs a) {
+constexpr int kPartThreads = 256, kPartSteps = kPartTile / kPartThreads, kPartWarps = kPartThreads / 32;
+constexpr unsigned kStatusAggregate = 1u, kStatusInclusive = 2u;
+
+__device__ __forceinline__ void publish_status(unsigned long long* w, unsigned flag, unsigned lefts) {
+  *reinterpret_cast<volatile unsigned long long*>(w) = ((unsigned long long)flag << 32) | lefts;
+}
+
+__device__ __forceinline__ unsigned lookback_lefts(const unsigned long long* status, unsigned tile, unsigned first, unsigned* s_red, unsigned* s_stop) {
+  unsigned excl = 0;
+  for (long long j = (long long)tile - 1 - threadIdx.x;; j -= kPartThreads) {
+    unsigned long long w = (unsigned long long)kStatusInclusive << 32;
+    if (j >= (long long)first) { do { w = *reinterpret_cast<const volatile unsigned long long*>(status + j); } while ((w >> 32) == 0); }
+    if (threadIdx.x == 0) *s_stop = kPartThreads;
+    __syncthreads();
+    if ((unsigned)(w >> 32) == kStatusInclusive) atomicMin(s_stop, threadIdx.x);
+    __syncthreads();
+    const unsigned stop = *s_stop;
+    unsigned v = threadIdx.x <= stop ? (unsigned)w : 0u;
+#pragma unroll
+    for (int o = 16; o > 0; o >>= 1) v += __shfl_xor_sync(0xffffffffu, v, o);
+    if ((threadIdx.x & 31) == 0) s_red[threadIdx.x >> 5] = v;
+    __syncthreads();
+#pragma unroll
+    for (int k = 0; k < kPartWarps; ++k) excl += s_red[k];
+    __syncthreads();
+    if (stop < kPartThreads) return excl;
+  }
+}
+
+template <bool GONLY>
+__global__ void __launch_bounds__(kPartThreads, 4) partition_kernel(PartArgs a) {
+  typedef typename std::conditional<GONLY, float, float2>::type Pay;
   const GrowState& gs = a.gs;
+  __shared__ unsigned s_rid[kPartTile];
+  __shared__ Pay s_gp[kPartTile];
+  __shared__ unsigned s_tl[kPartTile];
+  __shared__ unsigned s_pre[kPartSteps * kPartWarps];
+  __shared__ unsigned s_tile, s_tile_left, s_stop, s_red[kPartWarps], s_tmp[33];
+  __shared__ bool s_last;
+  unsigned long long* status = a.gs.part_sync + 2;
   const int cnt = gs.level_count[a.level];
-  if (cnt <= 0) return;
-  const unsigned tile = blockIdx.x;
-  if (tile >= gs.tile_prefix[cnt]) return;
-  const int i = find_node_of_tile(gs.tile_prefix, cnt, tile);
-  if (!gs.part_action[i]) return;
-  const int nid = gs.level_nodes[(size_t)a.level * a.max_level_nodes + i];
-  const unsigned lt = tile - gs.tile_prefix[i];
-  const unsigned b = gs.seg_begin[nid], c = gs.seg_count[nid];
-  const unsigned p0 = b + lt * kPartTile, p1 = (b + c < p0 + kPartTile) ? b + c : p0 + kPartTile;
-  const int f = a.tree.split_index[nid];
-  const int sb = a.tree.split_bin[nid], dl = a.tree.default_left[nid];
-  const uint8_t* col = a.bins_col + (int64_t)f * a.n;
-  unsigned nleft = 0;
-  const unsigned pt = p0 + threadIdx.x * 8;
-#pragma unroll
-  for (int j = 0; j < 8; ++j) {
-    unsigned p = pt + j;
-    if (p < p1) {
-      unsigned r = a.ridx_cur ? a.ridx_cur[p] : p;
-      int byte = col[r];
-      bool left = (a.has_missing && byte == kMissingBin) ? (dl != 0) : (byte <= sb);
-      gs.flags[p] = left ? 1 : 0; nleft += left ? 1u : 0u;
-    }
-  }
-  __shared__ unsigned s_cnt[8];
-#pragma unroll
-  for (int o = 16; o > 0; o >>= 1) nleft += __shfl_xor_sync(0xffffffffu, nleft, o);
-  if ((threadIdx.x & 31) == 0) s_cnt[threadIdx.x >> 5] = nleft;
-  __syncthreads();
-  if (threadIdx.x == 0) { unsigned tsum = 0; for (int w = 0; w < 8; ++w) tsum += s_cnt[w]; gs.tile_left[tile] = tsum; }
+  const unsigned T = cnt > 0 ? gs.tile_prefix[cnt] : 0u;
+  const bool has_tl = a.tl_cur != nullptr;
+  const int lane = threadIdx.x & 31, warp = threadIdx.x >> 5;
+  const unsigned lt_mask = (1u << lane) - 1u;
+  for (;;) {
+    if (threadIdx.x == 0) s_tile = (unsigned)atomicAdd(&a.gs.part_sync[0], 1ull);
+    __syncthreads();
+    const unsigned tile = s_tile;
+    if (tile >= T) break;
+    const int i = find_node_of_tile(gs.tile_prefix, cnt, tile);
+    if (gs.part_action[i]) {
+      const int nid = gs.level_nodes[(size_t)a.level * a.max_level_nodes + i];
+      const unsigned first = gs.tile_prefix[i], lt = tile - first;
+      const unsigned b = gs.seg_begin[nid], c = gs.seg_count[nid];
+      const unsigned p0 = b + lt * kPartTile, nrows = min(kPartTile, c - lt * kPartTile);
+      const int f = a.tree.split_index[nid], sb = a.tree.split_bin[nid], dl = a.tree.default_left[nid];
+      const uint8_t* col = a.bins_col + (int64_t)f * a.n;
+      unsigned rows[kPartSteps], tl[kPartSteps], bal[kPartSteps]; Pay gp[kPartSteps];
+#pragma unroll
+      for (int j = 0; j < kPartSteps; ++j) {
+        const unsigned k = j * kPartThreads + threadIdx.x, p = p0 + k;
+        const bool v = k < nrows;
+        rows[j] = v ? (a.ridx_cur ? a.ridx_cur[p] : p) : 0u;
+        if constexpr (GONLY) gp[j] = v ? a.g_cur[(size_t)p * a.g_stride] : 0.f;
+        else gp[j] = v ? a.gp_cur[p] : make_float2(0.f, 0.f);
+        tl[j] = (v && has_tl) ? a.tl_cur[p] : 0u;
+      }
+#pragma unroll
+      for (int j = 0; j < kPartSteps; ++j) {
+        const bool v = j * kPartThreads + threadIdx.x < nrows;
+        const int byte = v ? col[rows[j]] : 0;
+        const bool left = v && ((a.has_missing && byte == kMissingBin) ? (dl != 0) : (byte <= sb));
+        bal[j] = __ballot_sync(0xffffffffu, left);
+        if (lane == 0) s_pre[j * kPartWarps + warp] = __popc(bal[j]);
+      }
+      __syncthreads();
+      if (warp == 0) {
+        const unsigned x0 = s_pre[2 * lane], x1 = s_pre[2 * lane + 1];
+        unsigned x = x0 + x1;
+#pragma unroll
+        for (int o = 1; o < 32; o <<= 1) { const unsigned y = __shfl_up_sync(0xffffffffu, x, o); if (lane >= o) x += y; }
+        const unsigned ex = x - x0 - x1, tile_left = __shfl_sync(0xffffffffu, x, 31);
+        s_pre[2 * lane] = ex; s_pre[2 * lane + 1] = ex + x0;
+        if (lane == 0) { s_tile_left = tile_left; publish_status(status + tile, lt == 0 ? kStatusInclusive : kStatusAggregate, tile_left); }
+      }
+      __syncthreads();
+      const unsigned tile_left = s_tile_left;
+#pragma unroll
+      for (int j = 0; j < kPartSteps; ++j) {
+        const unsigned k = j * kPartThreads + threadIdx.x;
+        if (k < nrows) {
+          const unsigned lb = s_pre[j * kPartWarps + warp] + __popc(bal[j] & lt_mask);
+          const unsigned slot = ((bal[j] >> lane) & 1u) ? lb : nrows - 1u - (k - lb);
+          s_rid[slot] = rows[j]; s_gp[slot] = gp[j]; if (has_tl) s_tl[slot] = tl[j];
+        }
+      }
+      const unsigned excl = lt == 0 ? 0u : lookback_lefts(status, tile, first, s_red, &s_stop);
+      if (threadIdx.x == 0) {
+        if (lt != 0) publish_status(status + tile, kStatusInclusive, excl + tile_left);
+        if (tile + 1 == gs.tile_prefix[i + 1]) {
+          const unsigned nl = excl + tile_left;
+          const int Lc = a.tree.left[nid], Rc = a.tree.right[nid];
+          gs.seg_begin[Lc] = b; gs.seg_count[Lc] = nl; gs.seg_begin[Rc] = b + nl; gs.seg_count[Rc] = c - nl;
+        }
+        if (a.rows_counter) atomicAdd(a.rows_counter, (unsigned long long)nrows);
+      }
+      __syncthreads();
+      const unsigned dl0 = b + excl;
+      const unsigned dr0 = b + c - (lt * kPartTile - excl) - (nrows - tile_left);
+      for (unsigned k = threadIdx.x; k < nrows; k += kPartThreads) {
+        const unsigned dest = k < tile_left ? dl0 + k : dr0 + (k - tile_left);
+        a.ridx_next[dest] = s_rid[k];
+        if constexpr (GONLY) a.g_next[dest] = s_gp[k]; else a.gp_next[dest] = s_gp[k];
+        if (has_tl) a.tl_next[dest] = s_tl[k];
+      }
+    }
+    __syncthreads();
+  }
+  if (threadIdx.x == 0) { __threadfence(); s_last = atomicAdd(&a.gs.part_sync[1], 1ull) == gridDim.x - 1; }
+  __syncthreads();
+  if (!s_last) return;
+  __threadfence();
+  const int nb = *gs.build_count;
+  if (nb <= 0) { if (threadIdx.x == 0) gs.build_prefix[0] = 0; return; }
+  for (int k = threadIdx.x; k < nb; k += blockDim.x) gs.build_prefix[k] = __ldcg(gs.seg_count + gs.build_nid[k]);
+  __syncthreads();
+  const unsigned total = block_exclusive_scan(gs.build_prefix, gs.build_prefix, nb, s_tmp);
+  if (threadIdx.x == 0) gs.build_prefix[nb] = total;
 }
 
 struct PackedNode { unsigned short feat_dl; unsigned short bin_plus1; unsigned short left, right; };
@@ -541,87 +642,6 @@
   for (int j = 0; j < 4; ++j) { const int64_t r = base + j * 256; if (r < n) margin[r * K + k] += packed ? s_leaf[nid[j]] : t.split_cond[nid[j]]; }
 }
 
-__global__ void __launch_bounds__(1024) part_scan_kernel(PartArgs a) {
-  __shared__ unsigned s_tmp[33];
-  const GrowState& gs = a.gs;
-  const int cnt = gs.level_count[a.level];
-  const int i = blockIdx.x;
-  if (i >= cnt || !gs.part_action[i]) return;
-  const int nid = gs.level_nodes[(size_t)a.level * a.max_level_nodes + i];
-  const unsigned t0 = gs.tile_prefix[i], t1 = gs.tile_prefix[i + 1];
-  const unsigned nl = block_exclusive_scan(gs.tile_left + t0, gs.tile_off + t0, (int)(t1 - t0), s_tmp);
-  if (threadIdx.x == 0) {
-    const unsigned b = gs.seg_begin[nid], c = gs.seg_count[nid];
-    const int Lc = a.tree.left[nid], Rc = a.tree.right[nid];
-    gs.seg_begin[Lc] = b; gs.seg_count[Lc] = nl; gs.seg_begin[Rc] = b + nl; gs.seg_count[Rc] = c - nl;
-  }
-}
-
-__global__ void __launch_bounds__(256) part_scatter_kernel(PartArgs a) {
-  const GrowState& gs = a.gs;
-  const int cnt = gs.level_count[a.level];
-  if (cnt <= 0) return;
-  const unsigned tile = blockIdx.x;
-  if (tile >= gs.tile_prefix[cnt]) return;
-  const int i = find_node_of_tile(gs.tile_prefix, cnt, tile);
-  if (!gs.part_action[i]) return;
-  const int nid = gs.level_nodes[(size_t)a.level * a.max_level_nodes + i];
-  const unsigned lt = tile - gs.tile_prefix[i];
-  const unsigned b = gs.seg_begin[nid], c = gs.seg_count[nid];
-  const unsigned p0 = b + lt * kPartTile, p1 = (b + c < p0 + kPartTile) ? b + c : p0 + kPartTile;
-  const unsigned nrows = p1 - p0;
-  const unsigned nl = gs.seg_count[a.tree.left[nid]];
-  const unsigned toff = gs.tile_off[tile];
-  const unsigned pt = p0 + threadIdx.x * 8;
-  __shared__ unsigned s_rid[kPartTile];
-  __shared__ float2 s_gp[kPartTile];
-  __shared__ unsigned s_tl[kPartTile];
-  __shared__ unsigned s_w[8];
-  const bool has_tl = a.tl_cur != nullptr;
-  unsigned rows[8]; float2 gp[8]; unsigned tl[8]; unsigned char fl[8]; unsigned mine = 0;
-#pragma unroll
-  for (int j = 0; j < 8; ++j) {
-    unsigned p = pt + j;
-    if (p < p1) { rows[j] = a.ridx_cur ? a.ridx_cur[p] : p; gp[j] = a.gp_cur[p]; tl[j] = has_tl ? a.tl_cur[p] : 0u; fl[j] = gs.flags[p]; mine += fl[j]; }
-    else { rows[j] = 0; gp[j] = make_float2(0.f, 0.f); tl[j] = 0u; fl[j] = 2; }
-  }
-  const int lane = threadIdx.x & 31, warp = threadIdx.x >> 5;
-  unsigned x = mine;
-#pragma unroll
-  for (int o = 1; o < 32; o <<= 1) { unsigned y = __shfl_up_sync(0xffffffffu, x, o); if (lane >= o) x += y; }
-  if (lane == 31) s_w[warp] = x;
-  __syncthreads();
-  unsigned woff = 0, tile_left = 0;
-  for (int w = 0; w < 8; ++w) { if (w < warp) woff += s_w[w]; tile_left += s_w[w]; }
-  unsigned lbefore = woff + x - mine;
-#pragma unroll
-  for (int j = 0; j < 8; ++j) {
-    if (fl[j] == 2) continue;
-    unsigned jj = threadIdx.x * 8 + j;
-    unsigned slot = fl[j] ? lbefore++ : tile_left + (jj - lbefore);
-    s_rid[slot] = rows[j]; s_gp[slot] = gp[j]; if (has_tl) s_tl[slot] = tl[j];
-  }
-  __syncthreads();
-  const unsigned dl = b + toff, dr = b + nl + (lt * kPartTile - toff);
-  for (unsigned k = threadIdx.x; k < nrows; k += blockDim.x) {
-    unsigned dest = k < tile_left ? dl + k : dr + (k - tile_left);
-    a.ridx_next[dest] = s_rid[k];
-    a.gp_next[dest] = s_gp[k];
-    if (has_tl) a.tl_next[dest] = s_tl[k];
-  }
-}
-
-__global__ void __launch_bounds__(256) build_prefix_kernel(GrowState gs) {
-  __shared__ unsigned s_tmp[33];
-  const int nb = *gs.build_count;
-  if (nb <= 0) { if (threadIdx.x == 0) gs.build_prefix[0] = 0; return; }
-  unsigned* tmp = gs.tile_left;
-  for (int i = threadIdx.x; i < nb; i += blockDim.x) tmp[i] = gs.seg_count[gs.build_nid[i]];
-  __syncthreads();
-  unsigned total = block_exclusive_scan(tmp, gs.build_prefix, nb, s_tmp);
-  if (threadIdx.x == 0) gs.build_prefix[nb] = total;
-}
-
 __global__ void __launch_bounds__(256) subtract_kernel(GrowState gs, GH64* pool, size_t stride) {
   const int r = blockIdx.x;
   if (r >= *gs.build_count) return;
@@ -642,8 +662,8 @@
   dim3 grid(max_nodes_level, a.ngroups + (a.tw > 0 ? 1 : 0)); eval_kernel<<<grid, 32 * kEvalSegs, 0, s>>>(a); ++g_kernel_launches; CUDA_OK(cudaGetLastError());
 }
 void launch_apply_lossguide(const ApplyArgs& a, int iter, cudaStream_t s) { apply_lossguide_kernel<<<1, 256, 0, s>>>(a, iter); ++g_kernel_launches; CUDA_OK(cudaGetLastError()); }
-void launch_lg_copy_back(const PartArgs& a, unsigned* ridx_dst, float2* gp_dst, unsigned* tl_dst, unsigned max_tiles, cudaStream_t s) {
-  lg_copy_back_kernel<<<max_tiles < 1184u ? max_tiles : 1184u, 256, 0, s>>>(a, ridx_dst, gp_dst, tl_dst); ++g_kernel_launches; CUDA_OK(cudaGetLastError());
+void launch_lg_copy_back(const PartArgs& a, unsigned* ridx_dst, float2* gp_dst, float* g_dst, unsigned* tl_dst, unsigned max_tiles, cudaStream_t s) {
+  lg_copy_back_kernel<<<max_tiles < 1184u ? max_tiles : 1184u, 256, 0, s>>>(a, ridx_dst, gp_dst, g_dst, tl_dst); ++g_kernel_launches; CUDA_OK(cudaGetLastError());
 }
 void launch_zero_build_slots(const GrowState& gs, GH64* pool, size_t slot_entries, int max_build, cudaStream_t s) {
   dim3 grid(max_build, (unsigned)((slot_entries + 1023) / 1024)); zero_build_slots_kernel<<<grid, 256, 0, s>>>(gs, pool, slot_entries); ++g_kernel_launches; CUDA_OK(cudaGetLastError());
@@ -652,11 +672,20 @@
   lg_stage_kernel<<<(unsigned)((slot_entries + 1023) / 1024), 256, 0, s>>>(gs, pool, slot_entries, to_stage); ++g_kernel_launches; CUDA_OK(cudaGetLastError());
 }
 void launch_apply(const ApplyArgs& a, cudaStream_t s) { apply_kernel<<<1, 256, 0, s>>>(a); ++g_kernel_launches; CUDA_OK(cudaGetLastError()); }
-void launch_partition(const PartArgs& a, unsigned max_tiles, int max_nodes_level, cudaStream_t s) {
-  part_count_kernel<<<max_tiles, 256, 0, s>>>(a); ++g_kernel_launches; CUDA_OK(cudaGetLastError());
-  part_scan_kernel<<<max_nodes_level, 1024, 0, s>>>(a); ++g_kernel_launches; CUDA_OK(cudaGetLastError());
-  part_scatter_kernel<<<max_tiles, 256, 0, s>>>(a); ++g_kernel_launches; CUDA_OK(cudaGetLastError());
-  build_prefix_kernel<<<1, 256, 0, s>>>(a.gs); ++g_kernel_launches; CUDA_OK(cudaGetLastError());
+static int g_part_ctas_per_sm[2] = {0, 0};
+void partition_configure() {
+  if (g_part_ctas_per_sm[0]) return;
+  CUDA_OK(cudaOccupancyMaxActiveBlocksPerMultiprocessor(&g_part_ctas_per_sm[0], partition_kernel<false>, kPartThreads, 0));
+  CUDA_OK(cudaOccupancyMaxActiveBlocksPerMultiprocessor(&g_part_ctas_per_sm[1], partition_kernel<true>, kPartThreads, 0));
+  for (int& c : g_part_ctas_per_sm) c = std::max(c, 1);
+}
+void launch_partition(const PartArgs& a, unsigned max_tiles, int num_sms, cudaStream_t s) {
+  const bool gonly = a.g_next != nullptr;
+  B200_CHECK(g_part_ctas_per_sm[gonly] > 0, "partition_configure() must run before the first partition launch");
+  const unsigned grid = std::min<unsigned>(max_tiles, (unsigned)(num_sms * g_part_ctas_per_sm[gonly]));
+  CUDA_OK(cudaMemsetAsync(a.gs.part_sync, 0, (2 + (size_t)max_tiles) * sizeof(unsigned long long), s));
+  if (gonly) partition_kernel<true><<<grid, kPartThreads, 0, s>>>(a); else partition_kernel<false><<<grid, kPartThreads, 0, s>>>(a);
+  ++g_kernel_launches; CUDA_OK(cudaGetLastError());
 }
 void launch_update_margin(const TreeArrays& t, const int* n_nodes, const uint8_t* bins_col, int64_t n, int has_missing, float* margin, int K, int k, cudaStream_t s) {
   if (n == 0) return;
diff --git a/sagemaker-xgboost-container_b200/csrc/tree.h b/sagemaker-xgboost-container_b200/csrc/tree.h
--- a/sagemaker-xgboost-container_b200/csrc/tree.h
+++ b/sagemaker-xgboost-container_b200/csrc/tree.h
@@ -28,8 +28,10 @@
 struct PartArgs {
   GrowState gs; TreeArrays tree; const uint8_t* bins_col; int64_t n; const unsigned* ridx_cur; unsigned* ridx_next;
   const float2* gp_cur; float2* gp_next;
+  const float* g_cur; float* g_next; int g_stride;
   const unsigned* tl_cur; unsigned* tl_next;
   int has_missing, level, max_level_nodes;
+  unsigned long long* rows_counter;
 };
 
 struct HistArgs {
@@ -42,6 +44,7 @@
   int gather_stride;
   int tw;
   const float2* gpair;
+  const float* g_pos;
   const unsigned* ridx;
   const int* build_count;
   const int* build_nid;
@@ -62,7 +65,7 @@
 
 constexpr int kLgRootSlot = 0, kLgStageSlot = 1, kLgFirstFreeSlot = 2;
 void launch_apply_lossguide(const ApplyArgs& a, int iter, cudaStream_t s);
-void launch_lg_copy_back(const PartArgs& a, unsigned* ridx_dst, float2* gp_dst, unsigned* tl_dst, unsigned max_tiles, cudaStream_t s);
+void launch_lg_copy_back(const PartArgs& a, unsigned* ridx_dst, float2* gp_dst, float* g_dst, unsigned* tl_dst, unsigned max_tiles, cudaStream_t s);
 void launch_zero_build_slots(const GrowState& gs, GH64* pool, size_t slot_entries, int max_build, cudaStream_t s);
 void launch_lg_stage(const GrowState& gs, GH64* pool, size_t slot_entries, int to_stage, cudaStream_t s);
 void launch_hist_build(const HistArgs& a, int num_sms, cudaStream_t stream);
@@ -72,7 +75,8 @@
 void launch_scales(const GrowState& gs, int grad_bits, cudaStream_t s);
 void launch_eval(const EvalArgs& a, int max_nodes_level, cudaStream_t s);
 void launch_apply(const ApplyArgs& a, cudaStream_t s);
-void launch_partition(const PartArgs& a, unsigned max_tiles, int max_nodes_level, cudaStream_t s);
+void partition_configure();
+void launch_partition(const PartArgs& a, unsigned max_tiles, int num_sms, cudaStream_t s);
 void launch_update_margin(const TreeArrays& t, const int* n_nodes, const uint8_t* bins_col, int64_t n, int has_missing, float* margin, int K, int k, cudaStream_t s);
 void launch_subtract(const GrowState& gs, GH64* pool, size_t slot_entries, int max_build, cudaStream_t s);
 
```

Measured after the change: 109.6 (median of 6 runs). 0.963x the previous value.
